# James51332/OceanSimulation

Hardware: AMD Instinct MI355X
Metric: height-field points/sec (N² iFFT) at 1/2/4/8 MI355X; % HBM roofline (higher is better)
Workload: dtype f32

## Files before the change

include/oceanfft.h:

```cpp
#ifndef OCEANFFT_H
#define OCEANFFT_H

#include <stddef.h>
#include <stdint.h>

#ifdef __cplusplus
extern "C" {
#endif

#define OCEAN_OK 0
#define OCEAN_ERR_INVALID 1
#define OCEAN_ERR_HIP 2
#define OCEAN_ERR_NO_DEVICE 3
#define OCEAN_ERR_OOM 4

#define OCEAN_MAX_CASCADES 64

typedef struct ocean_settings
{
  int32_t seed[2];
  float U_10;
  float theta_0;
  float F;
  float g;
  float swell;
  float h;
  float displacement;
  float time;
  float planeSize;
  float scale;
  float spread;
  int32_t boundWavelength;
  float wavelengthMin;
  float wavelengthMax;
} ocean_settings;

typedef struct ocean_fft ocean_fft;
typedef struct ocean_generator ocean_generator;

const char* ocean_last_error(void);
const char* ocean_version(void);
void ocean_default_settings(ocean_settings* s);
int ocean_device_count(void);

int ocean_fft_create(ocean_fft** out, size_t texture_size, void* hip_stream);
int ocean_fft_destroy(ocean_fft* fft);
size_t ocean_fft_texture_resolution(const ocean_fft* fft);
int ocean_fft_encode_ifft(ocean_fft* fft, float* image);
int ocean_fft_encode_ifft_batch(ocean_fft* fft, float* images, int n_images);
int ocean_fft_synchronize(ocean_fft* fft);
int ocean_fft_device_cus(const ocean_fft* fft);
int ocean_fft_set_cu_budget(ocean_fft* fft, int cus);

int ocean_generator_create(ocean_generator** out, ocean_fft* fft, int cascades);
int ocean_generator_destroy(ocean_generator* gen);
int ocean_generator_cascades(const ocean_generator* gen);
ocean_settings* ocean_generator_settings(ocean_generator* gen, int cascade);
int ocean_generator_calculate(ocean_generator* gen, float timestep, int update_spectrum);
int ocean_generator_generate_spectrum(ocean_generator* gen);
float* ocean_generator_height_map(ocean_generator* gen, int cascade);
float* ocean_generator_displacement_map(ocean_generator* gen, int cascade);
float* ocean_generator_jacobian_map(ocean_generator* gen, int cascade);
float* ocean_generator_initial_spectrum(ocean_generator* gen, int cascade);
int ocean_generator_spectrum_block(const ocean_generator* gen);

int ocean_generator_set_half_spectrum(ocean_generator* gen, int enable);
int ocean_generator_set_four_step(ocean_generator* gen, int enable);
int ocean_generator_set_h0_memo(ocean_generator* gen, int enable);
int ocean_generator_set_frame_overlap(ocean_generator* gen, int enable);
int ocean_generator_frame_bytes(const ocean_generator* gen, double per_point[2]);

int ocean_generator_create_slab(ocean_generator** out, ocean_fft* fft, int rank, int ranks);
size_t ocean_generator_exchange_bytes(const ocean_generator* gen);
int ocean_generator_slab_columns(ocean_generator* gen, float timestep, int update_spectrum, float* send);
int ocean_generator_slab_rows(ocean_generator* gen, const float* recv);
int ocean_generator_slab_info(const ocean_generator* gen, int* rank, int* ranks, int* row0, int* rows);
int ocean_slab_layout(size_t texture_size, int rank, int ranks, int half, int64_t out[6]);

#define OCEAN_COMM_ID_BYTES 128
typedef struct ocean_comm ocean_comm;
int ocean_comm_unique_id(unsigned char id[OCEAN_COMM_ID_BYTES]);
int ocean_comm_create(ocean_comm** out, const unsigned char id[OCEAN_COMM_ID_BYTES], int nranks, int rank);
int ocean_comm_wrap(ocean_comm** out, void* nccl_comm, int nranks, int rank);
int ocean_comm_destroy(ocean_comm* comm);
int ocean_comm_all_to_all(ocean_comm* comm, const void* send, void* recv, size_t bytes, void* hip_stream);
int ocean_generator_slab_frame(ocean_generator* gen, ocean_comm* comm, float timestep, int update_spectrum);
int ocean_generator_slab_frame_pipelined(ocean_generator* gen, ocean_comm* comm, float timestep, int update_spectrum);
int ocean_generator_slab_flush(ocean_generator* gen);

#define OCEAN_ERR_TIMEOUT 5
#define OCEAN_PEER_HANDLE_BYTES 256
typedef struct ocean_peers ocean_peers;
int ocean_peers_create(ocean_peers** out, ocean_generator* gen);
int ocean_peers_destroy(ocean_peers* peers);
int ocean_peers_handle(const ocean_peers* peers, unsigned char handle[OCEAN_PEER_HANDLE_BYTES]);
int ocean_peers_connect(ocean_peers* peers, const unsigned char* handles);
int ocean_peers_connect_local(ocean_peers* const* all, int ranks);
int ocean_peers_set_timeout(ocean_peers* peers, int ms);
int ocean_peers_set_put_cus(ocean_peers* peers, int cus);
int ocean_peers_set_streams(ocean_peers* peers, void* column_stream, void* put_stream, void* row_stream);
int ocean_peers_set_row_cus(ocean_peers* peers, int cus);
int ocean_peers_set_put_cu_mask(ocean_peers* peers, int cus_per_xcd);
int ocean_generator_slab_frame_put(ocean_generator* gen, ocean_peers* peers, float timestep, int update_spectrum);
int ocean_generator_slab_frame_put_pipelined(ocean_generator* gen, ocean_peers* peers, float timestep,
                                             int update_spectrum);
int ocean_peers_flush(ocean_peers* peers);
int ocean_generator_slab_put_columns(ocean_generator* gen, ocean_peers* peers, float timestep, int update_spectrum);
int ocean_generator_slab_put_rows(ocean_generator* gen, ocean_peers* peers);
int ocean_peers_synchronize(ocean_peers* peers);

int ocean_peers_debug_slot(const ocean_peers* peers, int slot, void** ptr, size_t* bytes);

int ocean_frame_plan(size_t texture_size, int cascades, int32_t out[8]);

int ocean_generator_set_profiling(ocean_generator* gen, int enable);
int ocean_generator_kernel_times(ocean_generator* gen, double ms_total[3], int64_t launches[3]);
int ocean_generator_kernel_times4(ocean_generator* gen, double ms_total[4], int64_t launches[4]);

int ocean_debug_hash(const uint32_t* xy, int count, uint32_t* raw, float* uv, void* hip_stream);
int ocean_debug_copy(void* dst, const void* src, size_t bytes, int workgroups, void* hip_stream);
int ocean_debug_fft_work_limit(ocean_fft* fft, size_t bytes);

int ocean_surface_sample(ocean_generator* const* gens, const int* cascades, int count, const float* xz,
                         int64_t points, float* out);
int ocean_surface_sample_plane(ocean_generator* const* gens, const int* cascades, int count, const float camera[5],
                               int res, float* out);
int ocean_surface_query(ocean_generator* const* gens, const int* cascades, int count, const float* xz,
                        int64_t points, int iterations, float tolerance, float* out);

int ocean_generator_mip_levels(const ocean_generator* gen);
int ocean_generator_build_mips(ocean_generator* gen);
float* ocean_generator_height_mip(ocean_generator* gen, int cascade, int level);
float* ocean_generator_displacement_mip(ocean_generator* gen, int cascade, int level);
float* ocean_generator_jacobian_mip(ocean_generator* gen, int cascade, int level);
int ocean_surface_sample_lod(ocean_generator* const* gens, const int* cascades, int count, const float* xzf,
                             int64_t points, float* out);
int ocean_surface_sample_plane_lod(ocean_generator* const* gens, const int* cascades, int count,
                                   const float camera[5], int res, float* out);

int ocean_generator_calculate_rates(ocean_generator* gen);
float* ocean_generator_height_rate_map(ocean_generator* gen, int cascade);
float* ocean_generator_displacement_rate_map(ocean_generator* gen, int cascade);
int ocean_surface_velocity(ocean_generator* const* gens, const int* cascades, int count, const float* xz,
                           int64_t points, float* out);

int ocean_generator_set_depth_layers(ocean_generator* gen, const float* depths, int layers);
int ocean_generator_depth_layers(const ocean_generator* gen, float out[8]);
int ocean_generator_calculate_kinematics(ocean_generator* gen);
float* ocean_generator_kinematics_map(ocean_generator* gen, int cascade, int layer, int image);
int ocean_water_kinematics(ocean_generator* const* gens, const int* cascades, int count, const float* xyz,
                           int64_t points, int iterations, float tolerance, float* out);

int ocean_generator_build_bounds(ocean_generator* gen);
int ocean_generator_bounds(ocean_generator* gen, int cascade, float out[18]);
const float* ocean_generator_bounds_device(ocean_generator* gen);
int ocean_surface_raycast(ocean_generator* const* gens, const int* cascades, int count, const float* rays,
                          int64_t n_rays, float step, int max_steps, int refine, int iterations, float tolerance,
                          float slope, float pad, float* out);

typedef struct ocean_camera
{
  float position[3];
  float right[3], up[3], forward[3];
  float tan_half_fov_y, near_plane, far_plane;
  float lod_scale;
} ocean_camera;
typedef struct ocean_shading
{
  float wave_color[3], scatter_color[3], sky_color[3], light_color[3], light_direction[3];
  float sun_view_angle, sun_falloff_angle, fog_begin, fog_density;
} ocean_shading;
typedef struct ocean_march
{
  float step;
  int max_steps, refine, iterations;
  float tolerance, slope, pad;
} ocean_march;
void ocean_default_camera(ocean_camera* camera);
void ocean_default_shading(ocean_shading* shading);
void ocean_default_march(ocean_march* march);
int ocean_camera_rays(const ocean_camera* camera, int width, int height, float* rays, void* hip_stream);
int ocean_camera_render(ocean_generator* const* gens, const int* cascades, int count, const ocean_camera* camera,
                        const ocean_shading* shading, const ocean_march* march, int width, int height, float* image,
                        float* aux, uint8_t* image8);

typedef struct ocean_camera_layers
{
  float foam_color[3];
  float foam_lo, foam_hi;
  float foam_opacity;
  float spray_color[3];
  float spray_radius;
  int32_t spray_max_half;
  float spray_opacity;
} ocean_camera_layers;
void ocean_default_camera_layers(ocean_camera_layers* layers);
size_t ocean_camera_layers_scratch_bytes(int width, int height);
int ocean_camera_render_layers(ocean_generator* const* gens, const int* cascades, int count,
                               const ocean_camera* camera, const ocean_shading* shading, const ocean_march* march,
                               const ocean_camera_layers* layers, int width, int height, const float* records,
                               const int64_t* count_device, int64_t max_records, void* scratch, float* image,
                               float* aux, float* aux2, uint8_t* image8);

typedef struct ocean_hulls ocean_hulls;
int ocean_hulls_create(ocean_hulls** out, ocean_fft* fft, const float* points, int64_t n_points,
                       const int32_t* ranges, int bodies);
int ocean_hulls_destroy(ocean_hulls* hulls);
int ocean_hulls_bodies(const ocean_hulls* hulls);
int64_t ocean_hulls_instance_points(const ocean_hulls* hulls);
int ocean_hulls_loads(ocean_hulls* hulls, ocean_generator* const* gens, const int* cascades, int count,
                      const float* poses, float rho_g, int iterations, float tolerance, int water_velocity,
                      float* loads, float* point_out);

int ocean_hulls_set_bodies(ocean_hulls* hulls, const float* props);

typedef struct ocean_hull_step_settings {
  float dt; int32_t substeps;
  float gravity[3];
  float rho_g; int32_t iterations; float tolerance; int32_t water_velocity;
} ocean_hull_step_settings;
void ocean_default_hull_step_settings(ocean_hull_step_settings* settings);

int ocean_hulls_step(ocean_hulls* hulls, ocean_generator* const* gens, const int* cascades, int count,
                     const ocean_hull_step_settings* settings, float* poses, const float* wrench_ext,
                     float* loads, float* point_out);

int ocean_debug_hulls_packing(int enable);

typedef struct ocean_foam_settings {
  float bias;
  float gain;
  float decay;
  float level;
} ocean_foam_settings;
void ocean_default_foam_settings(ocean_foam_settings* out);
ocean_foam_settings* ocean_generator_foam_settings(ocean_generator* gen, int cascade);
int ocean_generator_advance_foam(ocean_generator* gen, float dt);
int ocean_generator_reset_foam(ocean_generator* gen);
float* ocean_generator_foam_map(ocean_generator* gen, int cascade);
int ocean_generator_foam_counts(ocean_generator* gen, int cascade, int64_t out[3]);
const int64_t* ocean_generator_foam_counts_device(ocean_generator* gen);
int ocean_surface_sample_foam(ocean_generator* const* gens, const int* cascades, int count, const float* xz,
                              int64_t points, float* out);
int ocean_surface_sample_plane_foam(ocean_generator* const* gens, const int* cascades, int count,
                                    const float camera[5], int res, float* out);

typedef struct ocean_foam_deposit_settings {
  float amount;
  float per_speed;
} ocean_foam_deposit_settings;
void ocean_default_foam_deposit_settings(ocean_foam_deposit_settings* out);
int ocean_foam_deposit(ocean_generator* const* gens, const int* cascades, int count,
                       const ocean_foam_deposit_settings* settings, const float* records,
                       const int64_t* count_device, int64_t max_records);
int ocean_foam_deposit_counts(ocean_generator* gen0, int64_t out[50]);
const int64_t* ocean_foam_deposit_counts_device(ocean_generator* gen0);
int ocean_debug_foam_deposit_merge(int enable);

typedef struct ocean_spray_settings {
  float threshold;
  float rate;
  uint32_t seed;
} ocean_spray_settings;
void ocean_default_spray_settings(ocean_spray_settings* out);
typedef struct ocean_spray ocean_spray;
int ocean_spray_create(ocean_spray** out, ocean_fft* fft);
int ocean_spray_destroy(ocean_spray* spray);
int ocean_spray_emit(ocean_spray* spray, ocean_generator* const* gens, const int* cascades, int count,
                     const ocean_spray_settings* settings, const int32_t* tiles, float dt, uint32_t step,
                     int velocity, int64_t capacity, float* out);
int ocean_spray_counts(ocean_spray* spray, int64_t out[18]);
const int64_t* ocean_spray_counts_device(ocean_spray* spray);

typedef struct ocean_particle_settings {
  float gravity;
  float drag;
  float wind[3];
  float lifetime;
  float gain;
  float lift;
  int32_t iterations;
  float tolerance;
} ocean_particle_settings;
void ocean_default_particle_settings(ocean_particle_settings* out);
typedef struct ocean_particles ocean_particles;
int ocean_particles_create(ocean_particles** out, ocean_fft* fft, int64_t capacity);
int ocean_particles_destroy(ocean_particles* pool);
int ocean_particles_step(ocean_particles* pool, ocean_generator* const* gens, const int* cascades, int count,
                         const ocean_particle_settings* settings, float dt, const float* emit_records,
                         const int64_t* emit_counts_device, int64_t landed_capacity, float* landed_out);
int ocean_particles_load(ocean_particles* pool, const float* device_records, int64_t count);
int ocean_particles_clear(ocean_particles* pool);
const float* ocean_particles_records(ocean_particles* pool);
int ocean_particles_counts(ocean_particles* pool, int64_t out[8]);
const int64_t* ocean_particles_counts_device(ocean_particles* pool);

#ifdef __cplusplus
}
#endif

#endif
```

oceansimulation_amd/capi.py:

```python
from __future__ import annotations

import ctypes
import os

_HERE = os.path.dirname(os.path.abspath(__file__))
LIB_PATH = os.path.join(_HERE, "liboceanfft.so")

OCEAN_OK = 0
OCEAN_ERR_INVALID = 1
OCEAN_ERR_HIP = 2
OCEAN_ERR_NO_DEVICE = 3
OCEAN_ERR_OOM = 4
OCEAN_ERR_TIMEOUT = 5
OCEAN_MAX_CASCADES = 64
OCEAN_COMM_ID_BYTES = 128
OCEAN_PEER_HANDLE_BYTES = 256


class OceanSettings(ctypes.Structure):

    _fields_ = [
        ("seed", ctypes.c_int32 * 2),
        ("U_10", ctypes.c_float),
        ("theta_0", ctypes.c_float),
        ("F", ctypes.c_float),
        ("g", ctypes.c_float),
        ("swell", ctypes.c_float),
        ("h", ctypes.c_float),
        ("displacement", ctypes.c_float),
        ("time", ctypes.c_float),
        ("planeSize", ctypes.c_float),
        ("scale", ctypes.c_float),
        ("spread", ctypes.c_float),
        ("boundWavelength", ctypes.c_int32),
        ("wavelengthMin", ctypes.c_float),
        ("wavelengthMax", ctypes.c_float),
    ]


assert ctypes.sizeof(OceanSettings) == 64


class OceanFoamSettings(ctypes.Structure):

    _fields_ = [
        ("bias", ctypes.c_float),
        ("gain", ctypes.c_float),
        ("decay", ctypes.c_float),
        ("level", ctypes.c_float),
    ]


assert ctypes.sizeof(OceanFoamSettings) == 16


class OceanFoamDepositSettings(ctypes.Structure):

    _fields_ = [
        ("amount", ctypes.c_float),
        ("per_speed", ctypes.c_float),
    ]


assert ctypes.sizeof(OceanFoamDepositSettings) == 8


class OceanSpraySettings(ctypes.Structure):

    _fields_ = [
        ("threshold", ctypes.c_float),
        ("rate", ctypes.c_float),
        ("seed", ctypes.c_uint32),
    ]


assert ctypes.sizeof(OceanSpraySettings) == 12


class OceanParticleSettings(ctypes.Structure):

    _fields_ = [
        ("gravity", ctypes.c_float),
        ("drag", ctypes.c_float),
        ("wind", ctypes.c_float * 3),
        ("lifetime", ctypes.c_float),
        ("gain", ctypes.c_float),
        ("lift", ctypes.c_float),
        ("iterations", ctypes.c_int32),
        ("tolerance", ctypes.c_float),
    ]


assert ctypes.sizeof(OceanParticleSettings) == 40


class OceanHullStepSettings(ctypes.Structure):

    _fields_ = [
        ("dt", ctypes.c_float),
        ("substeps", ctypes.c_int32),
        ("gravity", ctypes.c_float * 3),
        ("rho_g", ctypes.c_float),
        ("iterations", ctypes.c_int32),
        ("tolerance", ctypes.c_float),
        ("water_velocity", ctypes.c_int32),
    ]


assert ctypes.sizeof(OceanHullStepSettings) == 36


class OceanCamera(ctypes.Structure):

    _fields_ = [
        ("position", ctypes.c_float * 3),
        ("right", ctypes.c_float * 3),
        ("up", ctypes.c_float * 3),
        ("forward", ctypes.c_float * 3),
        ("tan_half_fov_y", ctypes.c_float),
        ("near_plane", ctypes.c_float),
        ("far_plane", ctypes.c_float),
        ("lod_scale", ctypes.c_float),
    ]


class OceanShading(ctypes.Structure):

    _fields_ = [
        ("wave_color", ctypes.c_float * 3),
        ("scatter_color", ctypes.c_float * 3),
        ("sky_color", ctypes.c_float * 3),
        ("light_color", ctypes.c_float * 3),
        ("light_direction", ctypes.c_float * 3),
        ("sun_view_angle", ctypes.c_float),
        ("sun_falloff_angle", ctypes.c_float),
        ("fog_begin", ctypes.c_float),
        ("fog_density", ctypes.c_float),
    ]


class OceanMarch(ctypes.Structure):

    _fields_ = [
        ("step", ctypes.c_float),
        ("max_steps", ctypes.c_int),
        ("refine", ctypes.c_int),
        ("iterations", ctypes.c_int),
        ("tolerance", ctypes.c_float),
        ("slope", ctypes.c_float),
        ("pad", ctypes.c_float),
    ]


assert ctypes.sizeof(OceanCamera) == 64 and ctypes.sizeof(OceanShading) == 76 and ctypes.sizeof(OceanMarch) == 28


class OceanCameraLayers(ctypes.Structure):

    _fields_ = [
        ("foam_color", ctypes.c_float * 3),
        ("foam_lo", ctypes.c_float),
        ("foam_hi", ctypes.c_float),
        ("foam_opacity", ctypes.c_float),
        ("spray_color", ctypes.c_float * 3),
        ("spray_radius", ctypes.c_float),
        ("spray_max_half", ctypes.c_int32),
        ("spray_opacity", ctypes.c_float),
    ]


assert ctypes.sizeof(OceanCameraLayers) == 48

_vp = ctypes.c_void_p
_i = ctypes.c_int
_f = ctypes.c_float
_sz = ctypes.c_size_t
_fp = ctypes.POINTER(ctypes.c_float)
_sp = ctypes.POINTER(OceanSettings)
_fsp = ctypes.POINTER(OceanFoamSettings)

SIGNATURES = {
    "ocean_last_error": (ctypes.c_char_p, []),
    "ocean_version": (ctypes.c_char_p, []),
    "ocean_default_settings": (None, [_sp]),
    "ocean_device_count": (_i, []),
    "ocean_fft_create": (_i, [ctypes.POINTER(_vp), _sz, _vp]),
    "ocean_fft_destroy": (_i, [_vp]),
    "ocean_fft_texture_resolution": (_sz, [_vp]),
    "ocean_fft_encode_ifft": (_i, [_vp, _vp]),
    "ocean_fft_encode_ifft_batch": (_i, [_vp, _vp, _i]),
    "ocean_fft_synchronize": (_i, [_vp]),
    "ocean_fft_device_cus": (_i, [_vp]),
    "ocean_fft_set_cu_budget": (_i, [_vp, _i]),
    "ocean_generator_create": (_i, [ctypes.POINTER(_vp), _vp, _i]),
    "ocean_generator_destroy": (_i, [_vp]),
    "ocean_generator_cascades": (_i, [_vp]),
    "ocean_generator_settings": (_sp, [_vp, _i]),
    "ocean_generator_calculate": (_i, [_vp, _f, _i]),
    "ocean_generator_generate_spectrum": (_i, [_vp]),
    "ocean_generator_height_map": (_vp, [_vp, _i]),
    "ocean_generator_displacement_map": (_vp, [_vp, _i]),
    "ocean_generator_jacobian_map": (_vp, [_vp, _i]),
    "ocean_generator_initial_spectrum": (_vp, [_vp, _i]),
    "ocean_generator_spectrum_block": (_i, [_vp]),
    "ocean_generator_create_slab": (_i, [ctypes.POINTER(_vp), _vp, _i, _i]),
    "ocean_generator_exchange_bytes": (_sz, [_vp]),
    "ocean_generator_slab_columns": (_i, [_vp, _f, _i, _vp]),
    "ocean_generator_slab_rows": (_i, [_vp, _vp]),
    "ocean_generator_slab_info": (_i, [_vp, ctypes.POINTER(_i), ctypes.POINTER(_i), ctypes.POINTER(_i), ctypes.POINTER(_i)]),
    "ocean_generator_set_profiling": (_i, [_vp, _i]),
    "ocean_generator_kernel_times": (_i, [_vp, ctypes.POINTER(ctypes.c_double), ctypes.POINTER(ctypes.c_int64)]),
    "ocean_debug_hash": (_i, [_vp, _i, _vp, _vp, _vp]),
    "ocean_debug_copy": (_i, [_vp, _vp, _sz, _i, _vp]),
    "ocean_debug_fft_work_limit": (_i, [_vp, _sz]),
    "ocean_surface_sample": (_i, [_vp, _vp, _i, _vp, ctypes.c_int64, _vp]),
    "ocean_surface_sample_plane": (_i, [_vp, _vp, _i, _vp, _i, _vp]),
    "ocean_surface_query": (_i, [_vp, _vp, _i, _vp, ctypes.c_int64, _i, ctypes.c_float, _vp]),
    "ocean_generator_mip_levels": (_i, [_vp]),
    "ocean_generator_build_mips": (_i, [_vp]),
    "ocean_generator_height_mip": (_vp, [_vp, _i, _i]),
    "ocean_generator_displacement_mip": (_vp, [_vp, _i, _i]),
    "ocean_generator_jacobian_mip": (_vp, [_vp, _i, _i]),
    "ocean_surface_sample_lod": (_i, [_vp, _vp, _i, _vp, ctypes.c_int64, _vp]),
    "ocean_surface_sample_plane_lod": (_i, [_vp, _vp, _i, _vp, _i, _vp]),
    "ocean_generator_calculate_rates": (_i, [_vp]),
    "ocean_generator_height_rate_map": (_vp, [_vp, _i]),
    "ocean_generator_displacement_rate_map": (_vp, [_vp, _i]),
    "ocean_surface_velocity": (_i, [_vp, _vp, _i, _vp, ctypes.c_int64, _vp]),
    "ocean_generator_set_depth_layers": (_i, [_vp, _fp, _i]),
    "ocean_generator_depth_layers": (_i, [_vp, _fp]),
    "ocean_generator_calculate_kinematics": (_i, [_vp]),
    "ocean_generator_kinematics_map": (_vp, [_vp, _i, _i, _i]),
    "ocean_water_kinematics": (_i, [_vp, _vp, _i, _vp, ctypes.c_int64, _i, ctypes.c_float, _vp]),
    "ocean_generator_build_bounds": (_i, [_vp]),
    "ocean_generator_bounds": (_i, [_vp, _i, _fp]),
    "ocean_generator_bounds_device": (_vp, [_vp]),
    "ocean_surface_raycast": (_i, [_vp, _vp, _i, _vp, ctypes.c_int64, _f, _i, _i, _i, _f, _f, _f, _vp]),
    "ocean_default_camera": (None, [ctypes.POINTER(OceanCamera)]),
    "ocean_default_shading": (None, [ctypes.POINTER(OceanShading)]),
    "ocean_default_march": (None, [ctypes.POINTER(OceanMarch)]),
    "ocean_camera_rays": (_i, [ctypes.POINTER(OceanCamera), _i, _i, _vp, _vp]),
    "ocean_camera_render": (_i, [_vp, _vp, _i, ctypes.POINTER(OceanCamera), ctypes.POINTER(OceanShading),
                                 ctypes.POINTER(OceanMarch), _i, _i, _vp, _vp, _vp]),
    "ocean_default_camera_layers": (None, [ctypes.POINTER(OceanCameraLayers)]),
    "ocean_camera_layers_scratch_bytes": (_sz, [_i, _i]),
    "ocean_camera_render_layers": (_i, [_vp, _vp, _i, ctypes.POINTER(OceanCamera), ctypes.POINTER(OceanShading),
                                        ctypes.POINTER(OceanMarch), ctypes.POINTER(OceanCameraLayers), _i, _i, _vp, _vp,
                                        ctypes.c_int64, _vp, _vp, _vp, _vp, _vp]),
    "ocean_default_foam_settings": (None, [_fsp]),
    "ocean_generator_foam_settings": (_fsp, [_vp, _i]),
    "ocean_generator_advance_foam": (_i, [_vp, _f]),
    "ocean_generator_reset_foam": (_i, [_vp]),
    "ocean_generator_foam_map": (_vp, [_vp, _i]),
    "ocean_generator_foam_counts": (_i, [_vp, _i, ctypes.POINTER(ctypes.c_int64)]),
    "ocean_generator_foam_counts_device": (_vp, [_vp]),
    "ocean_surface_sample_foam": (_i, [_vp, _vp, _i, _vp, ctypes.c_int64, _vp]),
    "ocean_surface_sample_plane_foam": (_i, [_vp, _vp, _i, _vp, _i, _vp]),
    "ocean_default_foam_deposit_settings": (None, [ctypes.POINTER(OceanFoamDepositSettings)]),
    "ocean_foam_deposit": (_i, [_vp, _vp, _i, ctypes.POINTER(OceanFoamDepositSettings), _vp, _vp, ctypes.c_int64]),
    "ocean_foam_deposit_counts": (_i, [_vp, ctypes.POINTER(ctypes.c_int64)]),
    "ocean_foam_deposit_counts_device": (_vp, [_vp]),
    "ocean_debug_foam_deposit_merge": (_i, [_i]),
    "ocean_hulls_create":(_i, [ctypes.POINTER(_vp), _vp, _vp, ctypes.c_int64, _vp, _i]),
    "ocean_hulls_destroy": (_i, [_vp]),
    "ocean_hulls_bodies": (_i, [_vp]),
    "ocean_hulls_instance_points": (ctypes.c_int64, [_vp]),
    "ocean_debug_hulls_packing": (_i, [_i]),
    "ocean_hulls_loads": (_i, [_vp, _vp, _vp, _i, _vp, _f, _i, _f, _i, _vp, _vp]),
    "ocean_hulls_set_bodies": (_i, [_vp, _vp]),
    "ocean_default_hull_step_settings": (None, [ctypes.POINTER(OceanHullStepSettings)]),
    "ocean_hulls_step": (_i, [_vp, _vp, _vp, _i, ctypes.POINTER(OceanHullStepSettings), _vp, _vp, _vp, _vp]),
    "ocean_default_spray_settings": (None, [ctypes.POINTER(OceanSpraySettings)]),
    "ocean_spray_create": (_i, [ctypes.POINTER(_vp), _vp]),
    "ocean_spray_destroy": (_i, [_vp]),
    "ocean_spray_emit": (_i, [_vp, _vp, _vp, _i, ctypes.POINTER(OceanSpraySettings), _vp, _f, ctypes.c_uint32, _i,
                              ctypes.c_int64, _vp]),
    "ocean_spray_counts": (_i, [_vp, ctypes.POINTER(ctypes.c_int64)]),
    "ocean_spray_counts_device": (_vp, [_vp]),
    "ocean_default_particle_settings": (None, [ctypes.POINTER(OceanParticleSettings)]),
    "ocean_particles_create": (_i, [ctypes.POINTER(_vp), _vp, ctypes.c_int64]),
    "ocean_particles_destroy": (_i, [_vp]),
    "ocean_particles_step": (_i, [_vp, _vp, _vp, _i, ctypes.POINTER(OceanParticleSettings), _f, _vp, _vp,
                                  ctypes.c_int64, _vp]),
    "ocean_particles_load": (_i, [_vp, _vp, ctypes.c_int64]),
    "ocean_particles_clear": (_i, [_vp]),
    "ocean_particles_records": (_vp, [_vp]),
    "ocean_particles_counts": (_i, [_vp, ctypes.POINTER(ctypes.c_int64)]),
    "ocean_particles_counts_device": (_vp, [_vp]),
    "ocean_generator_set_half_spectrum": (_i, [_vp, _i]),
    "ocean_generator_set_four_step": (_i, [_vp, _i]),
    "ocean_generator_set_h0_memo": (_i, [_vp, _i]),
    "ocean_generator_set_frame_overlap": (_i, [_vp, _i]),
    "ocean_generator_frame_bytes": (_i, [_vp, _vp]),
    "ocean_slab_layout": (_i, [_sz, _i, _i, _i, ctypes.POINTER(ctypes.c_int64)]),
    "ocean_comm_unique_id": (_i, [_vp]),
    "ocean_comm_create": (_i, [ctypes.POINTER(_vp), _vp, _i, _i]),
    "ocean_comm_wrap": (_i, [ctypes.POINTER(_vp), _vp, _i, _i]),
    "ocean_comm_destroy": (_i, [_vp]),
    "ocean_comm_all_to_all": (_i, [_vp, _vp, _vp, _sz, _vp]),
    "ocean_generator_slab_frame": (_i, [_vp, _vp, _f, _i]),
    "ocean_generator_slab_frame_pipelined": (_i, [_vp, _vp, _f, _i]),
    "ocean_generator_slab_flush": (_i, [_vp]),
    "ocean_peers_create": (_i, [ctypes.POINTER(_vp), _vp]),
    "ocean_peers_destroy": (_i, [_vp]),
    "ocean_peers_handle": (_i, [_vp, _vp]),
    "ocean_peers_connect": (_i, [_vp, _vp]),
    "ocean_peers_connect_local": (_i, [ctypes.POINTER(_vp), _i]),
    "ocean_peers_set_timeout": (_i, [_vp, _i]),
    "ocean_peers_set_put_cus": (_i, [_vp, _i]),
    "ocean_peers_set_streams": (_i, [_vp, _vp, _vp, _vp]),
    "ocean_peers_set_row_cus": (_i, [_vp, _i]),
    "ocean_peers_set_put_cu_mask": (_i, [_vp, _i]),
    "ocean_generator_kernel_times4": (_i, [_vp, ctypes.POINTER(ctypes.c_double), ctypes.POINTER(ctypes.c_int64)]),
    "ocean_generator_slab_frame_put": (_i, [_vp, _vp, _f, _i]),
    "ocean_generator_slab_frame_put_pipelined": (_i, [_vp, _vp, _f, _i]),
    "ocean_peers_flush": (_i, [_vp]),
    "ocean_frame_plan": (_i, [_sz, _i, ctypes.POINTER(ctypes.c_int32)]),
    "ocean_peers_debug_slot": (_i, [_vp, _i, ctypes.POINTER(ctypes.c_void_p), ctypes.POINTER(_sz)]),
    "ocean_generator_slab_put_columns": (_i, [_vp, _vp, _f, _i]),
    "ocean_generator_slab_put_rows": (_i, [_vp, _vp]),
    "ocean_peers_synchronize": (_i, [_vp]),
}

_lib = None


class OceanError(RuntimeError):
    def __init__(self, code: int, where: str):
        msg = lib().ocean_last_error().decode(errors="replace")
        super().__init__(f"{where} failed with status {code}: {msg}")
        self.code = code


def lib():
    global _lib
    if _lib is None:
        if not os.path.exists(LIB_PATH):
            raise ImportError(f"{LIB_PATH} is missing — run `make` (or __graft_entry__.build()) first; "
                              "there is no CPU fallback for the ocean hot path")
        L = ctypes.CDLL(LIB_PATH)
        for name, (res, args) in SIGNATURES.items():
            fn = getattr(L, name)
            fn.restype = res
            fn.argtypes = args
        _lib = L
    return _lib


def check(code: int, where: str) -> None:
    if code != OCEAN_OK:
        raise OceanError(code, where)
```

oceansimulation_amd/csrc/device/k_half_cols.h:

```cpp
#pragma once

#include <hip/hip_runtime.h>

#include <cstdint>

#include "ocean_internal.h"
#include "launch_common.h"
#include "device/evolve.h"
#include "device/fft.h"
#include "device/grid.h"
#include "device/memory.h"
#include "device/spectrum.h"

namespace oceanfft
{


template <int LOGN>
struct HalfCfg
{
  static constexpr int N = 1 << LOGN;
  static constexpr int B = ColFirstCfg<LOGN>::B;
  static constexpr int STRIPS = N / (2 * B) + 1;
  static constexpr bool SUPPORTED = B == 4 && ColFirstCfg<LOGN>::SPW == 1;
  static constexpr bool SLAB_SUPPORTED = ColFirstCfg<LOGN>::SPW == 1;
};

constexpr int kHalfRG = 2, kHalfRGC = 4;
constexpr int kHalfRG2 = 4, kHalfRGC2 = 8;
constexpr int kHalfHL = 1, kHalfHK = 4, kHalfHKSeed = 2;
template <int LOGN, int RG, int FB = 4>
__device__ __forceinline__ int half_group_offset(int y, int strip, int b = 0)
{
  constexpr int N = HalfCfg<LOGN>::N, FS = HalfCfg<LOGN>::STRIPS * HalfCfg<LOGN>::B / FB;
  return RG == 1 ? (strip * N + y) * FB + b : (((y / RG) * FS + strip) * RG + (y % RG)) * FB + b;
}


template <int LOGN_, bool SEED_>
struct ColsWhole
{
  static constexpr int LOGN = LOGN_, LA = SEED_ ? 0 : kStream;
  static constexpr bool SLAB = false, SEED = SEED_, PUT = false, NYQ = true;
  static constexpr int RG = kHalfRG, RGC = kHalfRGC, FB = 4;
  static constexpr int CPI = ColFirstCfg<LOGN_>::B, HB = ColFirstCfg<LOGN_>::B;
  static constexpr int HL = kHalfHL, HK = SEED_ ? kHalfHKSeed : LOGN_ == 12 ? kHalfHK : 2;
};

template <int LOGN_, bool SEED_, int HB_>
struct ColsHalfStrip
{
  static constexpr int LOGN = LOGN_, LA = SEED_ ? 0 : kStream;
  static constexpr bool SLAB = false, SEED = SEED_, PUT = false, NYQ = true;
  static constexpr int RG = kHalfRG2, RGC = kHalfRGC2, FB = 2;
  static constexpr int CPI = 2, HB = HB_;
  static constexpr int HL = kHalfHL, HK = SEED_ ? kHalfHKSeed : LOGN_ == 12 ? kHalfHK : 2;
};

template <int LOGN_, bool PUT_>
struct ColsSlab
{
  static constexpr int LOGN = LOGN_, LA = kStream;
  static constexpr bool SLAB = true, SEED = false, PUT = PUT_, NYQ = false;
  static constexpr int RG = 1, RGC = 1, FB = 4;
  static constexpr int CPI = ColFirstCfg<LOGN_>::B, HB = ColFirstCfg<LOGN_>::B;
  static constexpr int HL = kHalfHL, HK = LOGN_ == 13 ? 1 : kHalfHK - 1;
};

template <typename Sh>
struct ColsLaunch
{
  using S = FftShape<Sh::LOGN>;
  static constexpr int WG = S::T * Sh::CPI;
  static constexpr int LDS = ((S::TW_ENTRIES * 8 + 15) / 16) * 16 + Sh::CPI * S::PADDED * 8 + Sh::HL * WG * 16;
  static constexpr int items(int cascades, int nstrips) { return cascades * nstrips * (ColFirstCfg<Sh::LOGN>::B / Sh::CPI); }
  static constexpr int max_grid(int hs_blocks) { return Sh::SLAB ? hs_blocks : hs_blocks * (1024 / WG); }
};

template <typename Sh>
__global__ __launch_bounds__(ColsLaunch<Sh>::WG, Sh::CPI < ColFirstCfg<Sh::LOGN>::B ? 4 : 1) void k_cols_half(
    FrameParams fp, const float4* __restrict__ h0, float4* __restrict__ gab, float4* __restrict__ gde,
    float2* __restrict__ gc, const float2* __restrict__ tw_glob, float2* __restrict__ hs, HalfSlab hsl,
    unsigned char* __restrict__ send, int h0_full, const SpectrumConsts* __restrict__ seed)
{
  constexpr int LOGN = Sh::LOGN, LA = Sh::LA, RG = Sh::RG, RGC = Sh::RGC, CPI = Sh::CPI, HL = Sh::HL, HK = Sh::HK,
                FB = Sh::FB, HB = Sh::HB;
  constexpr bool SLAB = Sh::SLAB, SEED = Sh::SEED, PUT = Sh::PUT, NYQ = Sh::NYQ;
  using S = FftShape<LOGN>;
  using K = ColFirstCfg<LOGN>;
  using HC = HalfCfg<LOGN>;
  constexpr int N = S::N, T = S::T, B = K::B, STRIPS = HC::STRIPS, WG = T * CPI, HALVES = B / CPI;
  static_assert(SLAB ? HC::SLAB_SUPPORTED : HC::SUPPORTED, "half-spectrum path: one strip per item (B = 4 unless SLAB)");
  static_assert(CPI * HALVES == B && HALVES <= 2 && (HALVES == 1 || !SLAB), "whole or half strips");
  static_assert(HL >= 0 && HK >= 0 && HL + HK <= 8, "H pairs outside the scratch");
  static_assert(FB == 4 || (FB == CPI && HALVES == 2 && !SLAB && RG > 1 && RGC > 1), "FB: half-strip fields");
  static_assert(!PUT || SLAB, "PUT: the strip-dealt slab stores");
  static_assert(HB == B || (HB == CPI && HALVES == 2 && !SLAB), "HB: half strips over 2-column h0 strips");
  static_assert(!NYQ || !SLAB, "NYQ: whole grids (send is the spec output)");
  constexpr int XB = CPI * S::PADDED * 8;
  extern __shared__ __attribute__((aligned(16))) unsigned char smem[];
  float2* tw = reinterpret_cast<float2*>(smem);
  void* xch = smem + ((S::TW_ENTRIES * 8 + 15) / 16) * 16;
  float4* hlds = reinterpret_cast<float4*>(static_cast<unsigned char*>(xch) + XB);
  load_twiddles<LOGN>(tw, tw_glob);

  const int nstrips = SLAB ? hsl.nstrips : STRIPS;
  const int total = fp.cascades * nstrips * HALVES;
  const float dim = (float)N;
  for (int item = HALVES > 1 ? xcd_pair_slot(blockIdx.x, gridDim.x) : (int)blockIdx.x; item < total; item += gridDim.x)
  {
    const int hh = HALVES > 1 ? item % HALVES : 0, si = HALVES > 1 ? item / HALVES : item;
    const int c = si / nstrips, s = si - c * nstrips;
    const int sg = SLAB ? hsl.strip0 + s : s;
    if (HALVES > 1 && sg == STRIPS - 1 && hh != 0)
      continue;
    const int b = opaque((int)threadIdx.x) % CPI + hh * CPI;
    const int xb = sg == STRIPS - 1 ? 0 : N / (2 * B) + sg;
    const CascadeFrame f = fp.c[c];
    const float4* src = HB != B                  ? h0 + ((size_t)c * (N / HB) + xb * (B / HB) + hh) * N * HB
                        : (!SLAB || h0_full) ? h0 + ((size_t)c * (N / B) + xb) * N * B
                                             : h0 + ((size_t)c * nstrips + s) * N * B;
    const int fs = FB == 4 ? s : 2 * s + hh;
    const size_t gbase = RG == 1 ? ((size_t)c * STRIPS + s) * N * B
                                 : (size_t)c * STRIPS * N * B + half_group_offset<LOGN, RG, FB>(0, fs);
    const size_t cgbase = RGC == 1 ? ((size_t)c * STRIPS + s) * N * B
                                   : (size_t)c * STRIPS * N * B + half_group_offset<LOGN, RGC, FB>(0, fs);
    const int bf = FB == 4 ? b : b - hh * CPI;
    const int x = xb * B + b;
    float4 hk[HK > 0 ? HK : 1];
    auto run_round = [&](int round) __attribute__((always_inline)) {
      const int i = (opaque((int)threadIdx.x) / CPI) % T;
      const int voff = (i * B + b) * 16;
      CPair v[16];
      auto pack = [&](int m, float2 H, const KVec& q) __attribute__((always_inline)) {
        if (round == 0)
          v[m] = CPair{f2v{H.x, q.kz * H.x}, f2v{H.y, q.kz * H.y}};
        else if (round == 1)
        {
          const float e = q.kz * q.dirz;
          v[m] = CPair{f2v{q.dirz * H.x, e * H.x}, f2v{q.dirz * H.y, e * H.y}};
        }
        else
          v[m] = CPair{f2v{q.inv * H.x, 0.0f}, f2v{q.inv * H.y, 0.0f}};
      };
      if (SEED && round == 0)
      {
        float2* hsb = hs + (size_t)blockIdx.x * 16 * WG;
        const int hoff = opaque((int)threadIdx.x) * 8;
        const SpectrumConsts q = seed[c];
#pragma unroll 1
        for (int m = 0; m < 16; m++)
        {
          const int y = i + ((m + 8) & 15) * T;
          const float2 H = evolve(seed_texel(q, x, y, dim), make_kvec(x, y, dim, f.dk).k, f);
          if ((m >> 1) < HL)
            reinterpret_cast<float2*>(hlds)[((m >> 1) * WG + threadIdx.x) * 2 + (m & 1)] = H;
          else
            st2s<0>(hsb, hoff * 2 + (m & 1) * 8, (m >> 1) * WG * 16, H);
        }
        __threadfence_block();
#pragma unroll
        for (int m = 0; m < 16; m += 2)
        {
          const int y = i + ((m + 8) & 15) * T, p = m >> 1;
          const float4 pp = p < HL ? hlds[p * WG + threadIdx.x] : ld4s<kStream>(hsb, hoff * 2, p * WG * 16);
          if (p >= HL && p < HL + HK)
            hk[p < HL + HK && p >= HL ? p - HL : 0] = pp;
          pack(m, make_float2(pp.x, pp.y), make_kvec(x, y, dim, f.dk));
          pack(m + 1, make_float2(pp.z, pp.w), make_kvec(x, y + T, dim, f.dk));
        }
      }
      else if (round == 0)
      {
        float2* hsb = hs + (size_t)blockIdx.x * 16 * WG;
        const int hoff = opaque((int)threadIdx.x) * 8;
        float4 a[16];
        float2 hprev = make_float2(0.0f, 0.0f);
        const int loff = HB == B ? voff : (i * HB + (b - hh * CPI)) * 16;
#pragma unroll
        for (int m = 0; m < 16; m++)
          a[m] = ld4s<LA>(src, loff, ((m + 8) & 15) * T * HB * 16);
#pragma unroll
        for (int m = 0; m < 16; m++)
        {
          const int y = i + ((m + 8) & 15) * T;
          const KVec q = make_kvec(x, y, dim, f.dk);
          const float2 H = evolve(a[m], q.k, f);
          const int p = m >> 1;
          if ((m & 1) && p < HL)
            hlds[p * WG + threadIdx.x] = make_float4(hprev.x, hprev.y, H.x, H.y);
          else if ((m & 1) && p < HL + HK)
            hk[p - HL] = make_float4(hprev.x, hprev.y, H.x, H.y);
          else if (m & 1)
            st4s<0>(hsb, hoff * 2, p * WG * 16, make_float4(hprev.x, hprev.y, H.x, H.y));
          else
            hprev = H;
          pack(m, H, q);
        }
      }
      else
      {
        const float2* hsb = hs + (size_t)blockIdx.x * 16 * WG;
        const int hoff = opaque((int)threadIdx.x) * 8;
#pragma unroll
        for (int m = 0; m < 16; m += 2)
        {
          const int y = i + ((m + 8) & 15) * T, pi = m >> 1;
          const float4 p = pi < HL        ? hlds[pi * WG + threadIdx.x]
                           : pi < HL + HK ? hk[pi < HL + HK ? pi - HL : 0]
                                          : ld4s<kStream>(hsb, hoff * 2, pi * WG * 16);
          pack(m, make_float2(p.x, p.y), make_kvec(x, y, dim, f.dk));
          pack(m + 1, make_float2(p.z, p.w), make_kvec(x, y + T, dim, f.dk));
        }
      }
      const int reg = HALVES > 1 ? opaque((int)threadIdx.x) % CPI : b;
      fft_run<LOGN, CPI, true>(v, i, reg, xch, tw);
      const int vo = (i * B + b) * 16;
#pragma unroll
      for (int m = 0; m < 16; m++)
      {
        if constexpr (SLAB)
        {
          const size_t part = (size_t)fp.cascades * hsl.S * hsl.w * B;
          const int q = (m * T) / hsl.w, yl0 = (m * T) % hsl.w;
          const size_t el = (((size_t)c * hsl.S + s) * hsl.w + yl0) * B;
          unsigned char* blk =
              PUT ? reinterpret_cast<unsigned char*>(sopaque((size_t)reinterpret_cast<const uint64_t*>(send)[q]))
                  : send + sopaque((size_t)q * (part * 40 + (size_t)fp.cascades * 2 * N * 16));
          if (round == 0)
            st4<kStream>(blk + el * 16, vo, pair_raw(v[m]));
          else if (round == 1)
            st4<kStream>(blk + part * 16 + el * 16, vo, pair_raw(v[m]));
          else
            st2<kStream>(blk + part * 32 + el * 8, (i * B + b) * 8, make_float2(v[m].re.x, v[m].im.x));
        }
        else if constexpr (RG == 1 && RGC == 1)
        {
          if (round == 0)
            st4s<kStream>(gab + gbase, vo, m * T * B * 16, pair_raw(v[m]));
          else if (round == 1)
            st4s<kStream>(gde + gbase, vo, m * T * B * 16, pair_raw(v[m]));
          else
            st2s<kStream>(gc + gbase, (i * B + b) * 8, m * T * B * 8, make_float2(v[m].re.x, v[m].im.x));
        }
        else if (round == 0)
          st4s<kStream>(gab + gbase, half_group_offset<LOGN, RG, FB>(i, 0, bf) * 16, half_group_offset<LOGN, RG, FB>(m * T, 0) * 16,
                        pair_raw(v[m]));
        else if (round == 1)
          st4s<kStream>(gde + gbase, half_group_offset<LOGN, RG, FB>(i, 0, bf) * 16, half_group_offset<LOGN, RG, FB>(m * T, 0) * 16,
                        pair_raw(v[m]));
        else
          st2s<kStream>(gc + cgbase, half_group_offset<LOGN, RGC, FB>(i, 0, bf) * 8, half_group_offset<LOGN, RGC, FB>(m * T, 0) * 8,
                        make_float2(v[m].re.x, v[m].im.x));
      }
    };
#pragma unroll
    for (int round = 0; round < 3; round++)
      run_round(round);
  }
  if constexpr (NYQ)
    if ((HALVES > 1 ? xcd_pair_slot(blockIdx.x, gridDim.x) : (int)blockIdx.x) == (int)gridDim.x - 1)
      for (int idx = threadIdx.x; idx < fp.cascades * N; idx += WG)
        half_nyquist_texel(fp, N, HB, h0, reinterpret_cast<float4*>(send), nullptr, 1, 0, seed, nullptr, 0, idx);
}

template <typename Sh>
hipError_t launch_cols_half(const FrameParams& fp, int nstrips, const float4* h0, float4* gab, float4* gde, float2* gc,
                            const float2* tw, float2* hs, int hs_blocks, const HalfSlab& hsl, unsigned char* send,
                            int h0_full, const SpectrumConsts* seed, hipStream_t stream, int cus)
{
  using G = ColsLaunch<Sh>;
  auto kern = k_cols_half<Sh>;
  int grid = persistent_grid(kern, G::WG, G::LDS, G::items(fp.cascades, nstrips), cus);
  if (grid > G::max_grid(hs_blocks))
    grid = G::max_grid(hs_blocks);
  if (grid < 1)
    return hipErrorInvalidValue;
  hipLaunchKernelGGL(kern, dim3(grid), dim3(G::WG), G::LDS, stream, fp, h0, gab, gde, gc, tw, hs, hsl, send, h0_full, seed);
  return hipGetLastError();
}

}
```

oceansimulation_amd/csrc/device/k_half_rows.h:

```cpp
#pragma once

#include <hip/hip_runtime.h>

#include <cstdint>

#include "ocean_internal.h"
#include "device/evolve.h"
#include "device/fft.h"
#include "device/grid.h"
#include "device/memory.h"
#include "device/spectrum.h"
#include "device/k_half_cols.h"

namespace oceanfft
{

template <int LOGN, int LA, bool RM, int RG = 1, int RGC = 1, int FB = 4>
__global__ __launch_bounds__(FftShape<LOGN>::T * 2) void k_rows_half(
    FrameParams fp, const float4* __restrict__ gab, const float4* __restrict__ gde, const float2* __restrict__ gc,
    const float4* __restrict__ spec, float4* __restrict__ maps, float* __restrict__ jac, FoamParams foam,
    const float2* __restrict__ tw_glob, int rows, RowSrc rs)
{
  using S = FftShape<LOGN>;
  using K = ColFirstCfg<LOGN>;
  using HC = HalfCfg<LOGN>;
  constexpr int N = S::N, T = S::T, B = K::B, RPW = 2, STRIPS = HC::STRIPS, WG = T * RPW;
  static_assert(WG <= 1024, "two rows per workgroup: N <= 8192");
  static_assert(WG * 8 * 16 <= lds_row_slots<LOGN>(RPW) * 8, "mirror exchange fits the transform's LDS");
  extern __shared__ __attribute__((aligned(16))) unsigned char smem[];
  float2* tw = reinterpret_cast<float2*>(smem);
  void* xch = smem + ((S::TW_ENTRIES * 8 + 15) / 16) * 16;
  CPair* mir = reinterpret_cast<CPair*>(xch);
  load_twiddles<LOGN>(tw, tw_glob);

  const int blocks = (RM ? rows : N) / RPW;
  const int b0 = threadIdx.x % B, r0 = (threadIdx.x / B) % RPW, ihi0 = threadIdx.x / (B * RPW);
  constexpr int CI = T >= 128 ? 2 : 0;
  const int i20 = CI ? (threadIdx.x / RPW) % T : threadIdx.x % T, r20 = CI ? threadIdx.x % RPW : threadIdx.x / T;
  const int total = fp.cascades * blocks;
  const float dim = (float)N;
  for (int item = xcd_pair_slot(blockIdx.x, gridDim.x); item < total; item += gridDim.x)
  {
    const int c = item / blocks, y0 = (item - c * blocks) * RPW;
    float2 ckeep[8];
    float2 cnyq;
#pragma unroll
    for (int img = 0; img < 2; img++)
    {
    const int cimg = c * 2 + img;
    const int b = opaque(b0), ihi = opaque(ihi0), r = opaque(r0);
    const int i = ihi * B + b;
    const float dk = fp.c[c].dk;
    const size_t base = RM ? ((size_t)c * rows + y0) * rs.lp : (size_t)c * STRIPS * N * B;
    const int y = y0 + r;
    const float sgy = (y & 1) ? -1.0f : 1.0f;
    const float4* sp = spec + (size_t)cimg * N;
    const int tid = opaque((int)threadIdx.x);
    CPair v[16];
#pragma unroll
    for (int m = 0; m < 8; m++)
    {
      const int u = m * T + i;
      const int src = RM ? __builtin_amdgcn_readfirstlane(u >> (31 - __builtin_clz(rs.cpr))) : 0;
      const int off = RM ? r * rs.lp + (u & (rs.cpr - 1)) : half_group_offset<LOGN, RG, FB>(y, u / FB, u % FB);
      const int offc = RM ? off : half_group_offset<LOGN, RGC, FB>(y, u / FB, u % FB);
      const float4* fab = RM ? reinterpret_cast<const float4*>(rs.ab + src * rs.src_stride) + base : gab + base;
      const float4* fde = RM ? reinterpret_cast<const float4*>(rs.de + src * rs.src_stride) + base : gde + base;
      const float2* fc = RM ? reinterpret_cast<const float2*>(rs.c + src * rs.src_stride) + base : gc + base;
      const float kx = (float)u * dk;
      const float4 s4 = ld4<0>(sp, (N / 2 - u) * 16);
      CPair own, neg;
      if (img == 0)
      {
        const CPair p = raw_pair(ld4<LA>(fab, off * 16));
        const float2 cc = ld2<LA>(fc, offc * 8);
        ckeep[m] = cc;
        const float Ar = p.re.x, Ai = p.im.x, Br = p.re.y, Bi = p.im.y, Cr = cc.x, Ci = cc.y;
        own = CPair{f2v{(1.0f - kx) * Ar, -Bi - kx * Cr}, f2v{(1.0f - kx) * Ai, Br - kx * Ci}};
        neg = CPair{f2v{(1.0f + kx) * Ar + sgy * s4.x, -Bi + kx * Cr + sgy * s4.z},
                    f2v{-(1.0f + kx) * Ai + sgy * s4.y, -Br - kx * Ci + sgy * s4.w}};
      }
      else
      {
        const CPair q = raw_pair(ld4<LA>(fde, off * 16));
        const float2 cc = ckeep[m];
        const float Cr = cc.x, Ci = cc.y, Dr = q.re.x, Di = q.im.x, Er = q.re.y, Ei = q.im.y;
        const float kx2 = kx * kx;
        own = CPair{f2v{-(Di - kx2 * Ci), -Er + kx * Di}, f2v{Dr - kx2 * Cr, -Ei - kx * Dr}};
        neg = CPair{f2v{-(Di + kx2 * Ci) + sgy * s4.x, -Er - kx * Di + sgy * s4.z},
                    f2v{-Dr - kx2 * Cr + sgy * s4.y, Ei - kx * Dr + sgy * s4.w}};
      }
      v[m] = own;
      mir[m * WG + tid] = neg;
    }
    __syncthreads();
    const int tp = i == 0 ? tid : tid + (((T - i) / B - ihi) * B * RPW) + ((T - i) % B - b);
#pragma unroll
    for (int m = 8; m < 16; m++)
    {
      if (i == 0 && m == 8)
      {
        const int off = RM ? r * rs.lp + rs.cpr : half_group_offset<LOGN, RG, FB>(y, N / 2 / FB);
        const int offc = RM ? off : half_group_offset<LOGN, RGC, FB>(y, N / 2 / FB);
        const size_t ns = RM ? (size_t)rs.nyq_src * rs.src_stride : 0;
        const float4* fab = RM ? reinterpret_cast<const float4*>(rs.ab + ns) + base : gab + base;
        const float4* fde = RM ? reinterpret_cast<const float4*>(rs.de + ns) + base : gde + base;
        const float2* fc = RM ? reinterpret_cast<const float2*>(rs.c + ns) + base : gc + base;
        const float kx = -(dim / 2.0f) * dk;
        float2 cc;
        if (img == 1)
          cc = cnyq;
        else
          cc = ld2<LA>(fc, offc * 8);
        if (img == 0)
          cnyq = cc;
        if (img == 0)
        {
          const CPair p = raw_pair(ld4<LA>(fab, off * 16));
          v[m] = CPair{f2v{(1.0f - kx) * p.re.x, -p.im.y - kx * cc.x},
                       f2v{(1.0f - kx) * p.im.x, p.re.y - kx * cc.y}};
        }
        else
        {
          const CPair q = raw_pair(ld4<LA>(fde, off * 16));
          const float kx2 = kx * kx;
          v[m] = CPair{f2v{-(q.im.x - kx2 * cc.y), -q.re.y + kx * q.im.x},
                       f2v{q.re.x - kx2 * cc.x, -q.im.y - kx * q.re.x}};
        }
      }
      else
        v[m] = mir[(i == 0 ? 16 - m : 15 - m) * WG + tp];
    }
    __syncthreads();
    const int i2 = opaque(i20), r2 = opaque(r20);
    fft_run<LOGN, CI, true>(v, i, r, i2, r2, xch, tw);
    float4* dst = maps + ((size_t)cimg * (RM ? rows : N) + y0) * N;
    const int woff = ((r2 << LOGN) + i2) * 16;
#pragma unroll
    for (int m = 0; m < 16; m++)
      st4<kStream>(dst + m * T, woff, from_pair(v[m]));
    if (img & 1)
    {
      const float lam = foam.displacement[c];
      float* jb = jac + ((size_t)c * (RM ? rows : N) + y0) * N;
      const int joff = ((r2 << LOGN) + i2) * 4;
#pragma unroll
      for (int m = 0; m < 16; m++)
        st1<kStream>(jb + m * T, joff,
                (1.0f + lam * v[m].im.x) * (1.0f + lam * v[m].re.y) - lam * lam * v[m].im.y * v[m].im.y);
    }
    }
  }
}

}
```

oceansimulation_amd/csrc/device/k_rows_hp.h:

```cpp
#pragma once

#include <hip/hip_runtime.h>

#include <cstdint>

#include "ocean_internal.h"
#include "device/fft.h"
#include "device/grid.h"
#include "device/k_half_cols.h"
#include "device/lane_xchg.h"
#include "device/memory.h"

namespace oceanfft
{

struct HpCfg
{
  static constexpr int LOGN = 12, RS = 264;
  static constexpr int TW = ((FftShape<LOGN>::TW_ENTRIES * 8 + 15) / 16) * 16;
  static constexpr int LDS = TW + 16 * RS * 8;
};

__device__ __forceinline__ int hp_swz(int n1) { return ((n1 >> 1) & 7) ^ (((n1 >> 1) & 1) << 2); }
__device__ __forceinline__ int hp_slot(int n1, int j) { return n1 * HpCfg::RS + (j ^ hp_swz(n1)); }

template <int RG, int RGC, bool RM = false, int FB = 4, int GRP = 4, int EARLY = 0, int MINB = 4>
__global__ __launch_bounds__(256, MINB) void k_rows_hp(FrameParams fp, const float4* __restrict__ gab,
                                                 const float4* __restrict__ gde, const float2* __restrict__ gc,
                                                 const float4* __restrict__ spec, float4* __restrict__ maps,
                                                 float* __restrict__ jac, FoamParams foam,
                                                 const float2* __restrict__ tw_glob, int rows, RowSrc rs)
{
  constexpr int LOGN = HpCfg::LOGN, RS = HpCfg::RS;
  using S = FftShape<LOGN>;
  using HC = HalfCfg<LOGN>;
  constexpr int N = S::N, T = S::T, B = 4, STRIPS = HC::STRIPS;
  static_assert(T == 256, "one 4-wave row per workgroup");
  extern __shared__ __attribute__((aligned(16))) unsigned char smem[];
  float2* tw = reinterpret_cast<float2*>(smem);
  float2* xs = reinterpret_cast<float2*>(smem + HpCfg::TW);
  load_twiddles<LOGN>(tw, tw_glob);

  const int nrows = RM ? rows : N;
  const int total = fp.cascades * nrows;
  const float dim = (float)N;
  constexpr int LA = RM ? kStream : 0;
  const int lcpr = RM ? 31 - __builtin_clz(rs.cpr) : 0, cmask = RM ? rs.cpr - 1 : 0;
  const int wave0 = __builtin_amdgcn_readfirstlane((int)threadIdx.x & ~63);
  static_assert(EARLY == 0 || (EARLY == 1 && !RM), "EARLY: whole-grid layouts");
  float4 fpre[EARLY > 0 ? 8 : 1];
  auto issue = [&](int item, float4* f) __attribute__((always_inline)) {
    const int c = item / nrows, y = item - c * nrows;
    const size_t base = (size_t)c * STRIPS * N * B;
    const int i = opaque((int)threadIdx.x);
#pragma unroll
    for (int m = 0; m < 8; m++)
    {
      const int u = m * T + i;
      f[m] = ld4<LA>(gde + base, half_group_offset<LOGN, RG, FB>(y, u / FB, u % FB) * 16);
    }
  };
  for (int item = RM ? (int)blockIdx.x : xcd_group_slot<GRP>(blockIdx.x, gridDim.x); item < total; item += gridDim.x)
  {
    const int c = item / nrows, y = item - c * nrows;
    const float dk = fp.c[c].dk;
    const size_t base = RM ? ((size_t)c * rows + y) * rs.lp : (size_t)c * STRIPS * N * B;
    const float sgy = (y & 1) ? -1.0f : 1.0f;
    float2 ckeep[8], cnyq;
#pragma unroll
    for (int img = 0; img < 2; img++)
    {
      const int cimg = c * 2 + img;
      const float4* sp = spec + (size_t)cimg * N;
      const int tid = opaque((int)threadIdx.x), i = tid;
      CPair v[16];
#pragma unroll
      for (int m = 0; m < 8; m++)
      {
        const int u = m * T + i;
        const int src = RM ? (m * T + sopaque(wave0)) >> lcpr : 0;
        const int off = RM ? (u & cmask) : half_group_offset<LOGN, RG, FB>(y, u / FB, u % FB);
        const int offc = RM ? off : half_group_offset<LOGN, RGC, FB>(y, u / FB, u % FB);
        const float4* fab = RM ? reinterpret_cast<const float4*>(rs.ab + (size_t)src * rs.src_stride) : gab;
        const float4* fde = RM ? reinterpret_cast<const float4*>(rs.de + (size_t)src * rs.src_stride) : gde;
        const float2* fc = RM ? reinterpret_cast<const float2*>(rs.c + (size_t)src * rs.src_stride) : gc;
        const float kx = (float)u * dk;
        const float4 s4 = ld4<0>(sp, (N / 2 - u) * 16);
        if (img == 0)
        {
          const CPair p = raw_pair(ld4<LA>(fab + base, off * 16));
          const float2 cc = ld2<0>(fc + base, offc * 8);
          if constexpr (!RM)
            ckeep[m] = cc;
          const float Ar = p.re.x, Ai = p.im.x, Br = p.re.y, Bi = p.im.y, Cr = cc.x, Ci = cc.y;
          v[m] = CPair{f2v{(1.0f - kx) * Ar, -Bi - kx * Cr}, f2v{(1.0f - kx) * Ai, Br - kx * Ci}};
          v[m + 8] = CPair{f2v{(1.0f + kx) * Ar + sgy * s4.x, -Bi + kx * Cr + sgy * s4.z},
                           f2v{-(1.0f + kx) * Ai + sgy * s4.y, -Br - kx * Ci + sgy * s4.w}};
        }
        else
        {
          const CPair q = raw_pair(EARLY > 0 ? fpre[m] : ld4<LA>(fde + base, off * 16));
          float2 cc;
          if constexpr (RM)
            cc = ld2<0>(fc + base, offc * 8);
          else
            cc = ckeep[m];
          const float Cr = cc.x, Ci = cc.y, Dr = q.re.x, Di = q.im.x, Er = q.re.y, Ei = q.im.y;
          const float kx2 = kx * kx;
          v[m] = CPair{f2v{-(Di - kx2 * Ci), -Er + kx * Di}, f2v{Dr - kx2 * Cr, -Ei - kx * Dr}};
          v[m + 8] = CPair{f2v{-(Di + kx2 * Ci) + sgy * s4.x, -Er - kx * Di + sgy * s4.z},
                           f2v{-Dr - kx2 * Cr + sgy * s4.y, Ei - kx * Dr + sgy * s4.w}};
        }
      }
      if (i == 0)
      {
        const int off = RM ? rs.cpr : half_group_offset<LOGN, RG, FB>(y, N / 2 / FB);
        const int offc = RM ? off : half_group_offset<LOGN, RGC, FB>(y, N / 2 / FB);
        const size_t ns = RM ? (size_t)rs.nyq_src * rs.src_stride : 0;
        const float4* fab = RM ? reinterpret_cast<const float4*>(rs.ab + ns) : gab;
        const float4* fde = RM ? reinterpret_cast<const float4*>(rs.de + ns) : gde;
        const float2* fc = RM ? reinterpret_cast<const float2*>(rs.c + ns) : gc;
        const float kx = -(dim / 2.0f) * dk;
        if (RM || img == 0)
          cnyq = ld2<0>(fc + base, offc * 8);
        const float2 cc = cnyq;
        if (img == 0)
        {
          const CPair p = raw_pair(ld4<LA>(fab + base, off * 16));
          v[8] = CPair{f2v{(1.0f - kx) * p.re.x, -p.im.y - kx * cc.x}, f2v{(1.0f - kx) * p.im.x, p.re.y - kx * cc.y}};
        }
        else
        {
          const CPair q = raw_pair(ld4<LA>(fde + base, off * 16));
          const float kx2 = kx * kx;
          v[8] = CPair{f2v{-(q.im.x - kx2 * cc.y), -q.re.y + kx * q.im.x}, f2v{q.re.x - kx2 * cc.x, -q.im.y - kx * q.re.x}};
        }
      }
      const int w = tid >> 6, l = tid & 63, s = l & 3, p = l >> 2;
      const int n1r = 4 * w + s;
      const int rd = n1r * RS + (p ^ hp_swz(n1r));
      const int wo = hp_slot(i & 15, i >> 4);
      const int nm = N - i;
      const int wm = hp_slot(nm & 15, nm >> 4);
      const int wm0 = i == 0 ? hp_slot(0, (N / 2) >> 4) : wm;
      __syncthreads();
#pragma unroll
      for (int h = 0; h < 2; h++)
      {
        if (h)
          __syncthreads();
#pragma unroll
        for (int m = 0; m < 8; m++)
        {
          xs[wo + 16 * m] = half_of(v[m], h);
          xs[(m == 0 ? wm0 : wm) - 16 * m] = half_of(v[m + 8], h);
        }
        __syncthreads();
#pragma unroll
        for (int m = 0; m < 16; m++)
          set_half(v[m], h, xs[rd + 16 * m]);
      }
      idft16(v);
      apply_stage_twiddles<LOGN>(v, 16 * p, tw);
      transpose_reg_lanes_2_5(v);
      idft16(v);
      const float2 base_w = twiddle<LOGN>(n1r * p, tw);
#pragma unroll
      for (int m = 0; m < 16; m++)
        v[m] = cmul(v[m], base_w);
      apply_stage_twiddles<LOGN>(v, 16 * n1r, tw);
#pragma unroll
      for (int h = 0; h < 2; h++)
      {
        if (h)
          __syncthreads();
#pragma unroll
        for (int m = 0; m < 16; m++)
          xs[rd + 16 * m] = half_of(v[m], h);
        __syncthreads();
#pragma unroll
        for (int n1 = 0; n1 < 16; n1++)
          set_half(v[n1], h, xs[n1 * RS + (tid ^ hp_swz(n1))]);
      }
      idft16(v);
      if constexpr (EARLY > 0)
        if (img == 0)
          issue(item, fpre);
      float4* dst = maps + ((size_t)cimg * nrows + y) * N;
#pragma unroll
      for (int m = 0; m < 16; m++)
        st4<kStream>(dst + m * T, tid * 16, from_pair(v[m]));
      if (img == 1)
      {
        const float lam = foam.displacement[c];
        float* jb = jac + ((size_t)c * nrows + y) * N;
#pragma unroll
        for (int m = 0; m < 16; m++)
          st1<kStream>(jb + m * T, tid * 4,
                       (1.0f + lam * v[m].im.x) * (1.0f + lam * v[m].re.y) - lam * lam * v[m].im.y * v[m].im.y);
      }
    }
  }
}

}
```

oceansimulation_amd/csrc/launch_half.hip:

```cpp
#include <hip/hip_runtime.h>

#include <cstdint>

#include "oceanfft.h"
#include "ocean_internal.h"
#include "launch_common.h"
#include "device/grid.h"
#include "device/k_half_cols.h"
#include "device/k_half_rows.h"
#include "device/k_rows_hp.h"
#include "device/spectrum.h"

namespace oceanfft
{

bool half_spectrum_supported(int logn) { return logn >= 10 && logn <= 12; }

constexpr bool half_strip_launch(int logn, int cascades) { return (logn == 12 || logn == 11) && cascades <= 2; }

template <int LOGN, typename V>
hipError_t select_half_cols(int cascades, bool seed, int h0_blk, V&& visit)
{
  constexpr int B = ColFirstCfg<LOGN>::B;
  if constexpr (LOGN == 12 || LOGN == 11)
    if (half_strip_launch(LOGN, cascades))
    {
      if (h0_blk != 0 && h0_blk != 2 && h0_blk != B)
        return hipErrorInvalidValue;
      if (seed)
        return visit(ColsHalfStrip<LOGN, true, B>{});
      return h0_blk == B ? visit(ColsHalfStrip<LOGN, false, B>{}) : visit(ColsHalfStrip<LOGN, false, 2>{});
    }
  if (h0_blk != 0 && h0_blk != B)
    return hipErrorInvalidValue;
  return seed ? visit(ColsWhole<LOGN, true>{}) : visit(ColsWhole<LOGN, false>{});
}

template <int FB_, int RG_, int RGC_, int GRP_, int EARLY_, int MINB_>
struct RowsHp
{
  static constexpr bool HP = true;
  static constexpr int FB = FB_, RG = RG_, RGC = RGC_, GRP = GRP_, EARLY = EARLY_, MINB = MINB_;
};
template <int FB_, int RG_, int RGC_>
struct RowsHalf
{
  static constexpr bool HP = false;
  static constexpr int FB = FB_, RG = RG_, RGC = RGC_;
};

template <int LOGN, typename V>
hipError_t select_half_rows(int cascades, V&& visit)
{
  const bool hs = half_strip_launch(LOGN, cascades);
  if constexpr (LOGN == 12)
    return hs ? visit(RowsHp<2, kHalfRG2, kHalfRGC2, kHalfRGC2, 0, 4>{}) : visit(RowsHp<4, kHalfRG, kHalfRGC, 4, 1, 3>{});
  else if constexpr (LOGN == 11)
    return hs ? visit(RowsHalf<2, kHalfRG2, kHalfRGC2>{}) : visit(RowsHalf<4, kHalfRG, kHalfRGC>{});
  else
    return visit(RowsHalf<4, kHalfRG, kHalfRGC>{});
}

int half_h0_block(int logn, int cascades)
{
  int hb = spectrum_block(logn);
  (void)with_logn(logn, [&](auto L) -> hipError_t {
    constexpr int LOGN = decltype(L)::value;
    if constexpr (HalfCfg<LOGN>::SUPPORTED)
      return select_half_cols<LOGN>(cascades, false, 0, [&](auto sh) {
        hb = decltype(sh)::HB;
        return hipSuccess;
      });
    else
      return hipSuccess;
  });
  return hb;
}

size_t half_field_texels(int logn)
{
  const size_t n = (size_t)1 << logn;
  return (n / 8 + 1) * n * 4;
}

size_t half_hs_bytes(int logn, int blocks)
{
  return half_slab_supported(logn) ? (size_t)blocks * 16 * 1024 * sizeof(float2) : 0;
}

hipError_t launch_half_columns(int logn, const FrameParams& fp, const float4* h0, float4* gab, float4* gcd, float2* ge,
                               float4* spec, const float2* tw, hipStream_t stream, int cus, float2* hs, int hs_blocks,
                               const void* seed_consts, int h0_blk)
{
  if (!hs)
    return hipErrorInvalidValue;
  const SpectrumConsts* seed = static_cast<const SpectrumConsts*>(seed_consts);
  return with_logn(logn, [&](auto L) -> hipError_t {
    constexpr int LOGN = decltype(L)::value;
    if constexpr (!HalfCfg<LOGN>::SUPPORTED)
      return hipErrorInvalidValue;
    else
      return select_half_cols<LOGN>(fp.cascades, seed != nullptr, h0_blk > 0 ? h0_blk : ColFirstCfg<LOGN>::B, [&](auto sh) {
        return launch_cols_half<decltype(sh)>(fp, HalfCfg<LOGN>::STRIPS, h0, gab, gcd, ge, tw, hs, hs_blocks, HalfSlab{},
                                              reinterpret_cast<unsigned char*>(spec), 1, seed, stream, cus);
      });
  });
}

hipError_t launch_half_rows(int logn, const FrameParams& fp, const float4* gab, const float4* gcd, const float2* ge,
                            const float4* rcorr, float4* maps, float* jac, const FoamParams& foam, const float2* tw,
                            hipStream_t stream, int cus)
{
  return with_logn(logn, [&](auto L) -> hipError_t {
    constexpr int LOGN = decltype(L)::value;
    if constexpr (!HalfCfg<LOGN>::SUPPORTED)
      return hipErrorInvalidValue;
    else
      return select_half_rows<LOGN>(fp.cascades, [&](auto sh) {
        using R = decltype(sh);
        using S = FftShape<LOGN>;
        if constexpr (R::HP)
        {
          auto kern = k_rows_hp<R::RG, R::RGC, false, R::FB, R::GRP, R::EARLY, R::MINB>;
          const int grid = persistent_grid(kern, 256, HpCfg::LDS, fp.cascades * S::N, cus);
          hipLaunchKernelGGL(kern, dim3(grid), dim3(256), HpCfg::LDS, stream, fp, gab, gcd, ge, rcorr, maps, jac, foam, tw, 0,
                             RowSrc{});
        }
        else
        {
          auto kern = k_rows_half<LOGN, 0, false, R::RG, R::RGC, R::FB>;
          const int lds = ((S::TW_ENTRIES * 8 + 15) / 16) * 16 + lds_row_slots<LOGN>(2) * 8;
          const int grid = persistent_grid(kern, S::T * 2, lds, fp.cascades * (S::N / 2), cus);
          hipLaunchKernelGGL(kern, dim3(grid), dim3(S::T * 2), lds, stream, fp, gab, gcd, ge, rcorr, maps, jac, foam, tw, S::N,
                             RowSrc{});
        }
        return hipGetLastError();
      });
  });
}

}

extern "C" int ocean_frame_plan(size_t texture_size, int cascades, int32_t out[8])
{
  using namespace oceanfft;
  int logn = 0;
  while (logn < 15 && ((size_t)1 << logn) < texture_size)
    logn++;
  if (!out || ((size_t)1 << logn) != texture_size || !half_spectrum_supported(logn) || cascades < 1 ||
      cascades > kMaxCascades)
    return OCEAN_ERR_INVALID;
  const hipError_t e = with_logn(logn, [&](auto L) -> hipError_t {
    constexpr int LOGN = decltype(L)::value;
    if constexpr (!HalfCfg<LOGN>::SUPPORTED)
      return hipErrorInvalidValue;
    else
    {
      const hipError_t ec = select_half_cols<LOGN>(cascades, false, 0, [&](auto sh) {
        using C = decltype(sh);
        out[0] = C::FB, out[1] = C::RG, out[2] = C::RGC, out[3] = C::HB;
        return hipSuccess;
      });
      const hipError_t er = select_half_rows<LOGN>(cascades, [&](auto sh) {
        using R = decltype(sh);
        out[4] = R::FB, out[5] = R::RG, out[6] = R::RGC;
        return hipSuccess;
      });
      return ec != hipSuccess ? ec : er;
    }
  });
  if (e != hipSuccess)
    return OCEAN_ERR_INVALID;
  out[7] = half_h0_block(logn, cascades);
  return OCEAN_OK;
}
```

oceansimulation_amd/csrc/ocean_capi.cpp:

```cpp
#include "oceanfft.h"

#include <hip/hip_runtime.h>

#include <algorithm>
#include <cmath>
#include <cstdio>
#include <cstring>
#include <string>
#include <vector>

#include "ocean_capi_internal.h"
#include "ocean_internal.h"

static_assert(sizeof(ocean_settings) == sizeof(OceanSettings), "settings layout");

namespace
{
int log2_exact(size_t n)
{
  int l = 0;
  while (((size_t)1 << l) < n)
    l++;
  return ((size_t)1 << l) == n ? l : -1;
}

std::vector<float2> twiddle_tables(int logn, size_t& tw2_at, size_t& twm_at)
{
  std::vector<float2> tab;
  const double two_pi = 6.283185307179586476925286766559;
  auto append_table = [&](int lg) {
    const int lb = lg / 2, tb = 1 << lb, ta = 1 << (lg - lb);
    const double len = (double)(1 << lg);
    for (int e2 = 0; e2 < tb; e2++)
    {
      double a = two_pi * e2 / len;
      tab.push_back(make_float2((float)std::cos(a), (float)std::sin(a)));
    }
    for (int e2 = 0; e2 < ta; e2++)
    {
      double a = two_pi * ((double)e2 * tb) / len;
      tab.push_back(make_float2((float)std::cos(a), (float)std::sin(a)));
    }
  };
  append_table(logn);
  tw2_at = tab.size();
  if (fourstep_table(logn))
    append_table(logn - 4);
  twm_at = tab.size();
  if (ifft_pre_supported(logn))
    append_table(12);
  return tab;
}

void grow_work(ocean_fft* fft, size_t texels, int images)
{
  float4* w = nullptr;
  if (texels * sizeof(float4) > fft->work_limit)
    return;
  if (hipMalloc(&w, texels * sizeof(float4)) != hipSuccess)
  {
    (void)hipGetLastError();
    return;
  }
  if (fft->work)
    (void)hipFree(fft->work);
  fft->work = w;
  fft->work_images = images;
  fft->work_texels = texels;
}
}

constexpr int kFourStepSlab = 2048;

extern "C" {

const char* ocean_last_error(void) { return g_err.c_str(); }

const char* ocean_version(void) { return "oceanfft 0.1 (gfx950)"; }

void ocean_default_settings(ocean_settings* s)
{
  std::memset(s, 0, sizeof(*s));
  s->seed[0] = 12342;
  s->seed[1] = 8934;
  s->U_10 = 40.0f;
  s->theta_0 = 25.0f;
  s->F = 800000.0f;
  s->g = 9.8f;
  s->swell = 0.5f;
  s->h = 100.0f;
  s->displacement = 0.4f;
  s->time = 0.0f;
  s->planeSize = 40.0f;
  s->scale = 1.0f;
  s->spread = 0.2f;
  s->boundWavelength = 0;
  s->wavelengthMin = 0.0f;
  s->wavelengthMax = 0.0f;
}

int ocean_device_count(void)
{
  int n = 0;
  if (hipGetDeviceCount(&n) != hipSuccess)
    return 0;
  return n;
}

int ocean_fft_create(ocean_fft** out, size_t texture_size, void* hip_stream)
{
  if (!out)
    return fail(OCEAN_ERR_INVALID, "ocean_fft_create: out is null");
  *out = nullptr;
  int logn = log2_exact(texture_size);
  if (logn < 4 || logn > 14)
    return fail(OCEAN_ERR_INVALID, "ocean_fft_create: texture_size must be a power of two in [16, 16384], got " +
                                       std::to_string(texture_size));
  int ndev = 0;
  if (hipGetDeviceCount(&ndev) != hipSuccess || ndev == 0)
    return fail(OCEAN_ERR_NO_DEVICE, "ocean_fft_create: no HIP device visible");

  auto* f = new ocean_fft();
  f->n = (int)texture_size;
  f->logn = logn;
  f->stream = (hipStream_t)hip_stream;
  hipError_t e = hipGetDevice(&f->device);
  if (e == hipSuccess)
    e = hipDeviceGetAttribute(&f->device_cus, hipDeviceAttributeMultiprocessorCount, f->device);
  f->cus = f->device_cus;
  if (e != hipSuccess)
  {
    delete f;
    return hip_fail(e, "ocean_fft_create: device query");
  }

  size_t tw2_at = 0, twm_at = 0;
  const std::vector<float2> tab = twiddle_tables(logn, tw2_at, twm_at);
  e = hipMalloc(&f->twiddles, tab.size() * sizeof(float2));
  if (e == hipSuccess)
    e = hipMemcpy(f->twiddles, tab.data(), tab.size() * sizeof(float2), hipMemcpyHostToDevice);
  if (e != hipSuccess)
  {
    if (f->twiddles)
      (void)hipFree(f->twiddles);
    delete f;
    return hip_fail(e, "ocean_fft_create: twiddle table");
  }
  if (fourstep_table(logn))
    f->tw2 = f->twiddles + tw2_at;
  if (ifft_pre_supported(logn))
    f->twm = f->twiddles + twm_at;
  *out = f;
  return OCEAN_OK;
}

int ocean_fft_destroy(ocean_fft* fft)
{
  if (!fft)
    return OCEAN_OK;
  if (fft->twiddles)
    (void)hipFree(fft->twiddles);
  if (fft->work)
    (void)hipFree(fft->work);
  if (fft->surf_atlas)
    (void)hipFree(fft->surf_atlas);
  delete fft;
  return OCEAN_OK;
}

size_t ocean_fft_texture_resolution(const ocean_fft* fft) { return fft ? (size_t)fft->n : 0; }

int ocean_fft_device_cus(const ocean_fft* fft) { return fft ? fft->device_cus : 0; }

int ocean_fft_set_cu_budget(ocean_fft* fft, int cus)
{
  if (!fft)
    return fail(OCEAN_ERR_INVALID, "ocean_fft_set_cu_budget: null plan");
  if (cus < 0 || cus > fft->device_cus)
    return fail(OCEAN_ERR_INVALID, "ocean_fft_set_cu_budget: budget outside [0, device CUs]");
  fft->cus = cus == 0 ? fft->device_cus : cus;
  return OCEAN_OK;
}

int ocean_debug_fft_work_limit(ocean_fft* fft, size_t bytes)
{
  if (!fft)
    return fail(OCEAN_ERR_INVALID, "ocean_debug_fft_work_limit: null plan");
  fft->work_limit = bytes;
  if (fft->work && fft->work_texels * sizeof(float4) > bytes)
  {
    HIP_TRY(hipStreamSynchronize(fft->stream), "hipStreamSynchronize");
    (void)hipFree(fft->work);
    fft->work = nullptr;
    fft->work_images = 0;
    fft->work_texels = 0;
  }
  return OCEAN_OK;
}

int ocean_fft_encode_ifft_batch(ocean_fft* fft, float* images, int n_images)
{
  if (!fft || !images || n_images < 1)
    return fail(OCEAN_ERR_INVALID, "ocean_fft_encode_ifft_batch: null plan/image or n_images < 1");
  auto* img = reinterpret_cast<float4*>(images);
  const bool pre = fft->logn == 13 && fft->twm != nullptr;
  if (ifft_colfirst_supported(fft->logn) || pre)
  {
    const int chunk = std::max(1, (int)(((size_t)2 << 30) / ((size_t)fft->n * fft->n * sizeof(float4))));
    const int want = n_images < chunk ? n_images : chunk;
    if (fft->work_images < want)
      grow_work(fft, (size_t)want * fft->n * fft->n, want);
    if (fft->work)
    {
      for (int first = 0; first < n_images; first += fft->work_images)
      {
        const int count = n_images - first < fft->work_images ? n_images - first : fft->work_images;
        float4* first_img = img + (size_t)first * fft->n * fft->n;
        if (pre)
          HIP_TRY(launch_ifft_pre(fft->logn, count, first_img, fft->work, fft->twiddles, fft->twm, fft->stream, fft->cus),
                  "pre-stage EncodeIFFT");
        else
          HIP_TRY(launch_ifft_colfirst(fft->logn, count, first_img, fft->work, fft->twiddles, fft->stream, fft->cus),
                  "column-first EncodeIFFT");
      }
      return OCEAN_OK;
    }
  }
  if (ifft_fourstep_supported(fft->logn) && fft->logn == 14)
  {
    const size_t want = ifft_fourstep_work_texels(fft->logn, kFourStepSlab);
    if (fft->work_texels < want)
      grow_work(fft, want, 0);
    if (fft->work_texels >= want)
    {
      HIP_TRY(launch_ifft_fourstep(fft->logn, n_images, img, fft->work, kFourStepSlab, fft->twiddles, fft->tw2,
                                   fft->stream, fft->cus),
              "four-step EncodeIFFT");
      return OCEAN_OK;
    }
  }
  HIP_TRY(launch_rows_ifft(fft->logn, n_images, img, fft->twiddles, fft->stream, fft->cus), "row pass");
  HIP_TRY(launch_cols(fft->logn, n_images, img, fft->twiddles, fft->stream, fft->cus), "column pass");
  return OCEAN_OK;
}

int ocean_fft_encode_ifft(ocean_fft* fft, float* image) { return ocean_fft_encode_ifft_batch(fft, image, 1); }

int ocean_fft_synchronize(ocean_fft* fft)
{
  if (!fft)
    return fail(OCEAN_ERR_INVALID, "ocean_fft_synchronize: null plan");
  HIP_TRY(hipStreamSynchronize(fft->stream), "hipStreamSynchronize");
  return OCEAN_OK;
}

}

namespace
{
hipEvent_t take_event(ocean_generator* g)
{
  if (!g->pool.empty())
  {
    hipEvent_t e = g->pool.back();
    g->pool.pop_back();
    return e;
  }
  hipEvent_t e = nullptr;
  (void)hipEventCreate(&e);
  return e;
}

template <typename F>
hipError_t timed(ocean_generator* g, int kind, F&& launch, hipStream_t stream = nullptr)
{
  if (!g->profiling)
    return launch();
  if (!stream)
    stream = g->fft->stream;
  EventPair p{kind, take_event(g), take_event(g)};
  hipError_t e = hipEventRecord(p.a, stream);
  if (e != hipSuccess)
    return e;
  e = launch();
  if (e != hipSuccess)
    return e;
  e = hipEventRecord(p.b, stream);
  g->pending.push_back(p);
  return e;
}

hipError_t half_fields(ocean_generator* g, int slot)
{
  const size_t t = half_field_texels(g->fft->logn) * g->cascades;
  HalfFields& f = g->fields[slot];
  hipError_t e = alloc_if_null(f.gab, t * sizeof(float4));
  e = alloc_if_null(f.gde, t * sizeof(float4), e);
  e = alloc_if_null(f.gc, t * sizeof(float2), e);
  return alloc_if_null(f.spec, (size_t)g->cascades * 2 * g->fft->n * sizeof(float4), e);
}

hipError_t half_buffers(ocean_generator* g)
{
  return alloc_if_null(g->hs, half_hs_bytes(g->fft->logn, g->fft->device_cus), half_fields(g, 0));
}

HalfSlab half_slab_geom(int logn, int rank, int ranks)
{
  const int strips = half_strips(logn);
  HalfSlab h{};
  h.S = (strips + ranks - 1) / ranks;
  h.strip0 = rank * h.S;
  h.nstrips = std::max(0, std::min(h.S, strips - h.strip0));
  h.w = (1 << logn) / ranks;
  return h;
}

int h0_block(const ocean_generator* g)
{
  switch (frame_path(g))
  {
    case FramePath::FourStep:
      return gen4_h0_block();
    case FramePath::HalfBlocked:
      return half_h0_block(g->fft->logn, g->cascades);
    default:
      return spectrum_block(g->fft->logn);
  }
}

size_t h0_texels(const ocean_generator* g)
{
  const size_t full = (size_t)g->fft->n * g->geom.w;
  if (g->ranks == 1)
    return full;
  const size_t strips = (size_t)g->hsl.nstrips * spectrum_block(g->fft->logn) * g->fft->n;
  size_t t = std::max(full, strips);
  if (gen4_supported(g->fft->logn))
    t = std::max(t, g->g4.h0_cstride);
  return t;
}

hipError_t full_buffers(ocean_generator* g)
{
  const size_t slab = (size_t)g->fft->n * g->geom.w * g->cascades;
  hipError_t e = alloc_if_null(g->inter, slab * 2 * sizeof(float4));
  return rows_need_transpose(g->fft->logn) ? alloc_if_null(g->scratch, slab * 2 * sizeof(float4), e) : e;
}

hipError_t path_buffers(ocean_generator* g)
{
  switch (frame_path(g))
  {
    case FramePath::Full:
      return full_buffers(g);
    case FramePath::HalfBlocked:
      return half_buffers(g);
    default:
      return hslab_buffers(g);
  }
}
}

size_t hslab_xbuf_bytes(const ocean_generator* g)
{
  if (frame_path(g) == FramePath::FourStep)
    return (size_t)g->ranks * g->g4.blk_bytes;
  return (size_t)g->ranks * half_slab_block_bytes(g->fft->logn, g->cascades, g->hsl);
}

hipError_t hslab_buffers(ocean_generator* g)
{
  const int logn = g->fft->logn, C = g->cascades;
  hipError_t e = hipSuccess;
  if (frame_path(g) == FramePath::FourStep)
    e = alloc_if_null(g->parts, gen4_parts_bytes(logn, C, g->g4));
  else
  {
    const size_t rt = half_slab_row_texels(logn, C, g->hsl.w);
    e = alloc_if_null(g->rm_ab, rt * sizeof(float4));
    e = alloc_if_null(g->rm_de, rt * sizeof(float4), e);
    e = alloc_if_null(g->rm_c, rt * sizeof(float2), e);
    e = alloc_if_null(g->hs, half_hs_bytes(logn, g->fft->device_cus), e);
  }
  const size_t xb = hslab_xbuf_bytes(g);
  if (e == hipSuccess && g->xbuf_bytes < xb)
  {
    if (g->xbuf)
      (void)hipFree(g->xbuf);
    g->xbuf = nullptr;
    g->xbuf_bytes = 0;
    e = hipMalloc(&g->xbuf, xb);
    if (e == hipSuccess)
      g->xbuf_bytes = xb;
  }
  if (g->ranks > 1)
    e = alloc_if_null(g->h0row, (size_t)C * g->fft->n * sizeof(float4), e);
  return e;
}

namespace
{
int generator_alloc(ocean_generator** out, ocean_fft* fft, int cascades, int rank, int ranks, bool is_slab)
{
  auto* g = new ocean_generator();
  g->fft = fft;
  g->cascades = cascades;
  g->rank = rank;
  g->ranks = ranks;
  g->geom.w = fft->n / ranks;
  g->geom.x0 = rank * g->geom.w;
  g->settings.resize(cascades);
  for (auto& s : g->settings)
    ocean_default_settings(&s);
  g->foam_settings.resize(cascades);
  for (auto& s : g->foam_settings)
    ocean_default_foam_settings(&s);
  const size_t slab = (size_t)fft->n * g->geom.w;
  g->slab = is_slab;
  g->half_kind = half_kind_of(fft->logn, is_slab);
  g->half_on = g->half_kind != HalfKind::None;
  g->hsl = half_slab_geom(fft->logn, rank, ranks);
  if (gen4_supported(fft->logn))
  {
    g->g4 = gen4_geom(fft->logn, cascades, rank, ranks, ranks == 1);
    g->g4.h0_cstride = h0_texels(g);
  }
  if (is_slab && cascades != 1)
  {
    delete g;
    return fail(OCEAN_ERR_INVALID, "generator allocation: a slab generator holds exactly one cascade");
  }
  const size_t h0_bytes = h0_texels(g) * cascades * sizeof(float4);
  hipError_t e = alloc_if_null(g->h0, h0_bytes);
  if (e == hipSuccess)
    e = path_buffers(g);
  e = alloc_if_null(g->maps, slab * cascades * 2 * sizeof(float4), e);
  e = alloc_if_null(g->jac, slab * cascades * sizeof(float), e);
  if (e == hipSuccess)
    e = hipMemsetAsync(g->h0, 0, h0_bytes, fft->stream);
  if (e == hipSuccess)
    e = hipMemsetAsync(g->maps, 0, slab * cascades * 2 * sizeof(float4), fft->stream);
  if (e == hipSuccess)
    e = hipMemsetAsync(g->jac, 0, slab * cascades * sizeof(float), fft->stream);
  if (e != hipSuccess)
  {
    ocean_generator_destroy(g);
    return alloc_fail(e, "generator allocation");
  }
  *out = g;
  return OCEAN_OK;
}

int wait_h0_readers(ocean_generator* g)
{
  if (g->cols_ev_valid)
    HIP_TRY(hipStreamWaitEvent(g->fft->stream, g->h0r_ev, 0), "h0 write: wait for the last column pass");
  return OCEAN_OK;
}

struct H0Piece
{
  size_t at;
  int x0, cols, block;
};

struct H0Pieces
{
  H0Piece piece[2];
  int count = 0;
  bool row0 = false;
};

H0Pieces h0_pieces(const ocean_generator* g)
{
  const int n = g->fft->n;
  const FramePath path = frame_path(g);
  H0Pieces p;
  if (g->ranks > 1 && path == FramePath::FourStep)
  {
    const Gen4Geom& q = g->g4;
    const int B = gen4_h0_block();
    p.piece[p.count++] = {q.h0_reg, n / 2 + q.u0, q.cols, B};
    if (q.nyq)
      p.piece[p.count++] = {q.h0_nyq, 0, B, B};
    p.row0 = true;
  }
  else if (g->ranks > 1 && path == FramePath::StripDealt)
  {
    const int B = spectrum_block(g->fft->logn), strips = half_strips(g->fft->logn);
    const HalfSlab& h = g->hsl;
    const int nreg = std::max(0, std::min(h.nstrips, strips - 1 - h.strip0));
    if (nreg > 0)
      p.piece[p.count++] = {0, n / 2 + h.strip0 * B, nreg * B, 0};
    if (nreg < h.nstrips)
      p.piece[p.count++] = {(size_t)nreg * n * B, 0, B, 0};
    p.row0 = true;
  }
  else
    p.piece[p.count++] = {0, g->geom.x0, g->geom.w, h0_block(g)};
  return p;
}

int generate_spectrum_with(ocean_generator* g, const std::vector<ocean_settings>& settings)
{
  TRY(wait_h0_readers(g));
  g->h0_dirty = true;
  g->h0_stale = false;
  g->h0_block = h0_block(g);
  g->h0_settings = settings;
  g->seeded = settings;
  ocean_fft* f = g->fft;
  const H0Pieces pieces = h0_pieces(g);
  for (int c = 0; c < g->cascades; c++)
  {
    OceanSettings s;
    std::memcpy(&s, &settings[c], sizeof(s));
    float4* base = g->h0 + h0_texels(g) * c;
    HIP_TRY(timed(g, 0, [&] {
              hipError_t e = hipSuccess;
              for (int i = 0; i < pieces.count && e == hipSuccess; i++)
              {
                const H0Piece& p = pieces.piece[i];
                e = launch_generate_spectrum(s, f->n, base + p.at, f->stream, f->cus, p.x0, p.cols, p.block);
              }
              if (e == hipSuccess && pieces.row0)
                e = launch_generate_spectrum_row(s, f->n, g->h0row + (size_t)c * f->n, f->stream);
              return e;
            }),
            "generateSpectrum");
  }
  return OCEAN_OK;
}

bool same_h0_inputs(const std::vector<ocean_settings>& a, const std::vector<ocean_settings>& b)
{
  if (a.size() != b.size())
    return false;
  for (size_t i = 0; i < a.size(); i++)
  {
    ocean_settings x = a[i], y = b[i];
    x.time = y.time = 0.0f;
    if (std::memcmp(&x, &y, sizeof(x)) != 0)
      return false;
  }
  return true;
}

int fused_reseed(ocean_generator* g, const void*& seed)
{
  ocean_fft* f = g->fft;
  std::vector<unsigned char> host((size_t)g->cascades * seed_consts_bytes());
  for (int c = 0; c < g->cascades; c++)
  {
    OceanSettings os;
    std::memcpy(&os, &g->settings[c], sizeof(os));
    seed_consts(os, f->n, host.data() + (size_t)c * seed_consts_bytes());
  }
  if (!g->seedc)
    HIP_TRY(hipMalloc(&g->seedc, (size_t)kMaxCascades * seed_consts_bytes()), "seed constants");
  if (host != g->seedc_host)
  {
    TRY(wait_h0_readers(g));
    HIP_TRY(hipMemcpyAsync(g->seedc, host.data(), host.size(), hipMemcpyHostToDevice, f->stream), "seed constants");
    g->seedc_host.swap(host);
  }
  seed = g->seedc;
  g->h0_dirty = true;
  g->h0_stale = true;
  g->seed_settings = g->settings;
  g->seeded = g->settings;
  return OCEAN_OK;
}

int seed_h0(ocean_generator* g, int update_spectrum, const void*& seed)
{
  if (update_spectrum && !g->update_spectrum && g->memo_h0 && same_h0_inputs(g->settings, g->seeded))
    update_spectrum = 0;
  if (g->update_spectrum || update_spectrum)
  {
    const bool fused = update_spectrum && !g->update_spectrum && frame_path(g) == FramePath::HalfBlocked && g->hs;
    g->update_spectrum = false;
    return fused ? fused_reseed(g, seed) : ocean_generator_generate_spectrum(g);
  }
  TRY(materialise_h0(g));
  if (g->h0_block != h0_block(g))
    TRY(generate_spectrum_with(g, g->h0_settings));
  return OCEAN_OK;
}

FrameParams frame_params(const ocean_generator* g)
{
  FrameParams fp{};
  fp.cascades = g->cascades;
  for (int c = 0; c < g->cascades; c++)
  {
    const ocean_settings& s = g->settings[c];
    fp.c[c].dk = 2.0f * 3.14159265358f / s.planeSize;
    fp.c[c].time = s.time;
    fp.c[c].g = s.g;
    fp.c[c].h = s.h;
  }
  return fp;
}

int half_slab_columns(ocean_generator* g, const FrameParams& fp, float4* out, const Gen4Put* put,
                      hipStream_t col_stream)
{
  ocean_fft* f = g->fft;
  const hipError_t eb = hslab_buffers(g);
  if (eb != hipSuccess)
    return alloc_fail(eb, "column pass buffers");
  hipStream_t cs = col_stream ? col_stream : f->stream;
  if (g->cols_ev_valid)
    HIP_TRY(hipStreamWaitEvent(cs, g->cols_ev, 0), "column pass: after the last column pass");
  if (cs != f->stream && g->h0_dirty)
  {
    if (!g->put_h0)
      HIP_TRY(hipEventCreateWithFlags(&g->put_h0, hipEventDisableTiming), "column pass: event");
    HIP_TRY(hipEventRecord(g->put_h0, f->stream), "column pass: stream event");
    HIP_TRY(hipStreamWaitEvent(cs, g->put_h0, 0), "column pass: stream order");
    g->h0_dirty = false;
  }
  Gen4Put timed_put = put ? *put : Gen4Put{};
  EventPair pp{3, nullptr, nullptr};
  if (put && g->profiling)
  {
    pp.a = take_event(g);
    pp.b = take_event(g);
    timed_put.start = pp.a;
  }
  if (frame_path(g) == FramePath::FourStep)
    HIP_TRY(timed(g, 1, [&] {
              return launch_gen4_columns(f->logn, fp, g->g4, g->h0, g->ranks > 1 ? g->h0row : nullptr,
                                         put && put->parts ? put->parts : g->parts, out ? (void*)out : (void*)g->xbuf,
                                         f->twiddles, f->tw2, cs, f->cus, put ? &timed_put : nullptr);
            }, cs),
            "column pass (half spectrum, four-step)");
  else
    HIP_TRY(timed(g, 1, [&] {
              return launch_half_slab_columns(f->logn, fp, g->hsl, g->ranks, g->h0, g->ranks == 1, g->h0row,
                                              out ? (void*)out : (void*)g->xbuf, f->twiddles, cs, f->cus, g->hs,
                                              f->device_cus, put ? &timed_put : nullptr);
            }, cs),
            "column pass (half spectrum, strip-dealt)");
  if (pp.a)
  {
    HIP_TRY(hipEventRecord(pp.b, put && put->stream ? put->stream : cs), "column pass: put event");
    g->pending.push_back(pp);
  }
  for (hipEvent_t* ev : {&g->cols_ev, &g->h0r_ev})
    if (!*ev)
      HIP_TRY(hipEventCreateWithFlags(ev, hipEventDisableTiming), "column pass: event");
  HIP_TRY(hipEventRecord(g->cols_ev, cs), "column pass: end event");
  HIP_TRY(hipEventRecord(g->h0r_ev, put && put->stream ? put->stream : cs), "column pass: end event");
  g->cols_ev_valid = true;
  return OCEAN_OK;
}

int overlapped_columns(ocean_generator* g, const FrameParams& fp, const void* seed)
{
  ocean_fft* f = g->fft;
  const int s = g->oslot;
  if (g->h0_dirty)
  {
    HIP_TRY(hipEventRecord(g->oh0, f->stream), "overlap: h0 event");
    HIP_TRY(hipStreamWaitEvent(g->side, g->oh0, 0), "overlap: h0 wait");
    g->h0_dirty = false;
  }
  if (g->orows_valid[s])
    HIP_TRY(hipStreamWaitEvent(g->side, g->orows[s], 0), "overlap: slot wait");
  const HalfFields& fl = g->fields[s];
  HIP_TRY(timed(g, 1, [&] {
            return launch_half_columns(f->logn, fp, g->h0, fl.gab, fl.gde, fl.gc, fl.spec, f->twiddles, g->side, f->cus,
                                       g->hs, f->device_cus, seed, g->h0_block);
          }, g->side),
          "column pass (half spectrum, overlapped)");
  HIP_TRY(hipEventRecord(g->ocols[s], g->side), "overlap: column event");
  return OCEAN_OK;
}

float4* own_exchange(const ocean_generator* g) { return half_slab_path(g) ? nullptr : g->inter; }

int land_frames_in_flight(ocean_generator* g)
{
  if (peers_pending(g->peers))
    TRY(ocean_peers_flush(g->peers));
  return ocean_generator_slab_flush(g);
}
}

int generator_columns(ocean_generator* g, float timestep, int update_spectrum, float4* out, const Gen4Put* put,
                      hipStream_t col_stream)
{
  ocean_fft* f = g->fft;
  g->rates_fresh = false;
  g->kin_fresh = false;
  for (auto& s : g->settings)
    s.time += timestep;
  const void* seed = nullptr;
  TRY(seed_h0(g, update_spectrum, seed));
  const FrameParams fp = frame_params(g);
  if (put && !half_slab_path(g))
    return fail(OCEAN_ERR_INVALID, "column pass: the one-sided exchange needs a half-spectrum slab path (N >= 1024)");
  switch (frame_path(g))
  {
    case FramePath::FourStep:
    case FramePath::StripDealt:
      TRY(half_slab_columns(g, fp, out, put, col_stream));
      break;
    case FramePath::HalfBlocked:
      if (g->overlap)
        TRY(overlapped_columns(g, fp, seed));
      else
        HIP_TRY(timed(g, 1, [&] {
                  const HalfFields& fl = g->fields[0];
                  return launch_half_columns(f->logn, fp, g->h0, fl.gab, fl.gde, fl.gc, fl.spec, f->twiddles, f->stream,
                                             f->cus, g->hs, f->device_cus, seed, g->h0_block);
                }),
                "column pass (half spectrum)");
      break;
    case FramePath::Full:
      HIP_TRY(timed(g, 1, [&] {
                return launch_cols_evolve(f->logn, fp, g->geom, g->h0, out, f->twiddles, f->stream, f->cus,
                                          default_keep(f->logn));
              }),
              "column pass");
      break;
  }
  g->frame = fp;
  return OCEAN_OK;
}

FrameState current_frame(const ocean_generator* g)
{
  FrameState fs{g->frame, FoamParams{}};
  for (int c = 0; c < g->cascades; c++)
    fs.foam.displacement[c] = g->settings[c].displacement;
  return fs;
}

int generator_rows(ocean_generator* g, const float4* in, const FrameState& fs, hipStream_t row_stream, int row_cus)
{
  ocean_fft* f = g->fft;
  g->mips_fresh = false;
  g->bounds_fresh = false;
  const int rcus = row_cus > 0 && row_cus < f->cus ? row_cus : f->cus;
  if (row_stream && !half_slab_path(g))
    return fail(OCEAN_ERR_INVALID, "row pass: a row stream needs a half-spectrum slab path");
  hipStream_t rs = row_stream ? row_stream : f->stream;
  switch (frame_path(g))
  {
    case FramePath::FourStep:
      HIP_TRY(timed(g, 2, [&] {
                return launch_gen4_rows(f->logn, fs.frame, g->g4, in ? (const void*)in : (const void*)g->xbuf, g->maps,
                                        g->jac, fs.foam, f->twiddles, f->tw2, rs, rcus);
              }, rs),
              "row pass (half spectrum, four-step)");
      break;
    case FramePath::StripDealt:
      HIP_TRY(timed(g, 2, [&] {
                return launch_half_slab_rows(f->logn, fs.frame, g->hsl, in ? (const void*)in : (const void*)g->xbuf,
                                             g->rm_ab, g->rm_de, g->rm_c, g->maps, g->jac, fs.foam, f->twiddles,
                                             f->tw2, rs, rcus);
              }, rs),
              "row pass (half spectrum, strip-dealt)");
      break;
    case FramePath::HalfBlocked:
    {
      const int s = g->overlap ? g->oslot : 0;
      const HalfFields& fl = g->fields[s];
      if (g->overlap)
        HIP_TRY(hipStreamWaitEvent(f->stream, g->ocols[s], 0), "overlap: column wait");
      HIP_TRY(timed(g, 2, [&] {
                return launch_half_rows(f->logn, fs.frame, fl.gab, fl.gde, fl.gc, fl.spec, g->maps, g->jac, fs.foam,
                                        f->twiddles, f->stream, f->cus);
              }),
              g->overlap ? "row pass (half spectrum, overlapped)" : "row pass (half spectrum)");
      if (g->overlap)
      {
        HIP_TRY(hipEventRecord(g->orows[s], f->stream), "overlap: row event");
        g->orows_valid[s] = true;
        g->oslot = s ^ 1;
      }
      break;
    }
    case FramePath::Full:
      HIP_TRY(timed(g, 2, [&] {
                return launch_rows_final(f->logn, g->cascades, g->geom, in, g->scratch, g->maps, g->jac, fs.foam,
                                         f->twiddles, f->stream, f->cus);
              }),
              "row pass");
      break;
  }
  return OCEAN_OK;
}

int materialise_h0(ocean_generator* g)
{
  return g->h0_stale ? generate_spectrum_with(g, g->seed_settings) : OCEAN_OK;
}

extern "C" {

int ocean_generator_create(ocean_generator** out, ocean_fft* fft, int cascades)
{
  if (!out || !fft)
    return fail(OCEAN_ERR_INVALID, "ocean_generator_create: null argument");
  *out = nullptr;
  if (cascades < 1 || cascades > OCEAN_MAX_CASCADES)
    return fail(OCEAN_ERR_INVALID, "ocean_generator_create: cascades must be in [1, 64]");
  return generator_alloc(out, fft, cascades, 0, 1, false);
}

int ocean_generator_create_slab(ocean_generator** out, ocean_fft* fft, int rank, int ranks)
{
  if (!out || !fft)
    return fail(OCEAN_ERR_INVALID, "ocean_generator_create_slab: null argument");
  *out = nullptr;
  const int blk = spectrum_block(fft->logn);
  if (ranks < 1 || ranks > 16 || (ranks & (ranks - 1)) != 0 || rank < 0 || rank >= ranks)
    return fail(OCEAN_ERR_INVALID, "ocean_generator_create_slab: ranks must be a power of two in [1, 16], 0 <= rank < ranks");
  const int w = fft->n / ranks;
  if (w % blk != 0 || w < fft->n / 16 || w < slab_min_width(fft->logn))
    return fail(OCEAN_ERR_INVALID, "ocean_generator_create_slab: N / ranks = " + std::to_string(w) +
                                       " is below this size's minimum slab width " +
                                       std::to_string(slab_min_width(fft->logn)));
  return generator_alloc(out, fft, 1, rank, ranks, true);
}

int ocean_generator_destroy(ocean_generator* g)
{
  if (!g)
    return OCEAN_OK;
  if (g->comm_stream)
    (void)hipStreamSynchronize(g->comm_stream);
  if (g->peers)
    peers_detach(g->peers);
  if (g->fft)
    (void)hipStreamSynchronize(g->fft->stream);
  if (g->side)
    (void)hipStreamSynchronize(g->side);
  for (hipStream_t st : {g->comm_stream, g->side})
    if (st)
      (void)hipStreamDestroy(st);
  for (auto& p : g->pending)
    for (hipEvent_t ev : {p.a, p.b})
      g->pool.push_back(ev);
  for (hipEvent_t ev : g->pool)
    (void)hipEventDestroy(ev);
  for (hipEvent_t ev : {g->cols_done[0], g->cols_done[1], g->xchg_done[0], g->xchg_done[1], g->rows_done[0],
                        g->rows_done[1], g->put_h0, g->cols_ev, g->h0r_ev, g->ocols[0], g->ocols[1], g->orows[0],
                        g->orows[1], g->oh0})
    if (ev)
      (void)hipEventDestroy(ev);
  const HalfFields &f0 = g->fields[0], &f1 = g->fields[1];
  for (void* p : {(void*)g->h0, (void*)g->inter, (void*)g->scratch, (void*)g->maps, (void*)g->jac, (void*)g->xsend[0],
                  (void*)g->xsend[1], (void*)g->xrecv[0], (void*)g->xrecv[1], (void*)f0.gab, (void*)f0.gde, (void*)f0.gc,
                  (void*)f0.spec, (void*)f1.gab, (void*)f1.gde, (void*)f1.gc, (void*)f1.spec, (void*)g->hs,
                  (void*)g->h0row, g->seedc, (void*)g->rm_ab, (void*)g->rm_de, (void*)g->rm_c, (void*)g->parts,
                  (void*)g->xbuf, (void*)g->mips, (void*)g->rates, (void*)g->kin, (void*)g->bounds, (void*)g->foam, g->foam_counts,
                  (void*)g->deposit_acc, g->deposit_counts})
    if (p)
      (void)hipFree(p);
  delete g;
  return OCEAN_OK;
}

int ocean_generator_cascades(const ocean_generator* g) { return g ? g->cascades : 0; }

ocean_settings* ocean_generator_settings(ocean_generator* g, int c)
{
  if (!g || c < 0 || c >= g->cascades)
  {
    fail(OCEAN_ERR_INVALID, "ocean_generator_settings: cascade out of range");
    return nullptr;
  }
  return &g->settings[c];
}

int ocean_generator_generate_spectrum(ocean_generator* g)
{
  if (!g)
    return fail(OCEAN_ERR_INVALID, "ocean_generator_generate_spectrum: null generator");
  return generate_spectrum_with(g, g->settings);
}

int ocean_generator_set_half_spectrum(ocean_generator* g, int enable)
{
  if (!g)
    return fail(OCEAN_ERR_INVALID, "ocean_generator_set_half_spectrum: null generator");
  TRY(land_frames_in_flight(g));
  if (!enable && g->overlap)
    TRY(ocean_generator_set_frame_overlap(g, 0));
  if (enable && g->half_kind == HalfKind::None)
    return fail(OCEAN_ERR_INVALID, "ocean_generator_set_half_spectrum: N = 1024 .. 16384 only");
  const bool was_on = g->half_on, was_slab_path = half_slab_path(g);
  g->half_on = enable != 0;
  const hipError_t e = path_buffers(g);
  if (e != hipSuccess)
  {
    g->half_on = was_on;
    return alloc_fail(e, "ocean_generator_set_half_spectrum");
  }
  if ((was_slab_path && g->ranks > 1) != (half_slab_path(g) && g->ranks > 1))
    g->update_spectrum = true;
  return OCEAN_OK;
}

int ocean_generator_set_frame_overlap(ocean_generator* g, int enable)
{
  if (!g)
    return fail(OCEAN_ERR_INVALID, "ocean_generator_set_frame_overlap: null generator");
  if (enable && frame_path(g) != FramePath::HalfBlocked)
    return fail(OCEAN_ERR_INVALID, "ocean_generator_set_frame_overlap: whole grids of N = 1024 .. 4096 on the "
                                   "half-spectrum path only");
  ocean_fft* f = g->fft;
  if (enable && !g->overlap)
  {
    hipError_t e = hipSuccess;
    if (!g->side)
      e = hipStreamCreateWithFlags(&g->side, hipStreamNonBlocking);
    for (hipEvent_t* ev : {&g->ocols[0], &g->ocols[1], &g->orows[0], &g->orows[1], &g->oh0})
      if (e == hipSuccess && !*ev)
        e = hipEventCreateWithFlags(ev, hipEventDisableTiming);
    if (e == hipSuccess)
      e = half_fields(g, 1);
    if (e == hipSuccess)
      e = hipEventRecord(g->oh0, f->stream);
    if (e == hipSuccess)
      e = hipStreamWaitEvent(g->side, g->oh0, 0);
    if (e != hipSuccess)
      return alloc_fail(e, "ocean_generator_set_frame_overlap");
    g->orows_valid[0] = g->orows_valid[1] = false;
    g->oslot = 0;
    g->h0_dirty = false;
    g->overlap = true;
  }
  else if (!enable && g->overlap)
  {
    for (int s = 0; s < 2; s++)
      if (g->orows_valid[s])
        HIP_TRY(hipStreamWaitEvent(f->stream, g->orows[s], 0), "ocean_generator_set_frame_overlap");
    HIP_TRY(hipEventRecord(g->oh0, g->side), "ocean_generator_set_frame_overlap");
    HIP_TRY(hipStreamWaitEvent(f->stream, g->oh0, 0), "ocean_generator_set_frame_overlap");
    g->overlap = false;
  }
  return OCEAN_OK;
}

int ocean_generator_set_h0_memo(ocean_generator* g, int enable)
{
  if (!g)
    return fail(OCEAN_ERR_INVALID, "ocean_generator_set_h0_memo: null generator");
  g->memo_h0 = enable != 0;
  return OCEAN_OK;
}

int ocean_generator_set_four_step(ocean_generator* g, int enable)
{
  if (!g)
    return fail(OCEAN_ERR_INVALID, "ocean_generator_set_four_step: null generator");
  TRY(land_frames_in_flight(g));
  g->four_step = enable != 0;
  if (half_slab_path(g))
  {
    const hipError_t e = hslab_buffers(g);
    if (e != hipSuccess)
      return alloc_fail(e, "ocean_generator_set_four_step");
  }
  return OCEAN_OK;
}

int ocean_generator_frame_bytes(const ocean_generator* g, double per_point[2])
{
  if (!g || !per_point)
    return fail(OCEAN_ERR_INVALID, "ocean_generator_frame_bytes: null argument");
  const double n = g->fft->n;
  switch (const FramePath path = frame_path(g))
  {
    case FramePath::FourStep:
    {
      const double kept = (n / 2 + 1) / n;
      per_point[0] = (16.0 + 40.0 + 80.0) * kept;
      per_point[1] = 40.0 * kept + 36.0;
      break;
    }
    case FramePath::HalfBlocked:
    case FramePath::StripDealt:
    {
      const double kept = (n / 2 + spectrum_block(g->fft->logn)) / n;
      per_point[0] = 16.0 * kept + 40.0 * kept;
      per_point[1] = 40.0 * kept + 36.0 + (path == FramePath::StripDealt ? 80.0 * kept : 0.0);
      break;
    }
    case FramePath::Full:
      per_point[0] = 48.0;
      per_point[1] = 68.0 + (rows_need_transpose(g->fft->logn) ? 64.0 : 0.0);
      break;
  }
  return OCEAN_OK;
}

int ocean_generator_calculate(ocean_generator* g, float timestep, int update_spectrum)
{
  if (!g)
    return fail(OCEAN_ERR_INVALID, "ocean_generator_calculate: null generator");
  if (g->ranks != 1)
    return fail(OCEAN_ERR_INVALID, "ocean_generator_calculate: slab generators step with "
                                   "ocean_generator_slab_columns / exchange / ocean_generator_slab_rows");
  float4* buf = own_exchange(g);
  TRY(generator_columns(g, timestep, update_spectrum, buf));
  return generator_rows(g, buf, current_frame(g));
}

size_t ocean_generator_exchange_bytes(const ocean_generator* g)
{
  if (!g)
    return 0;
  if (half_slab_path(g))
    return hslab_xbuf_bytes(g);
  return (size_t)g->cascades * 2 * g->fft->n * g->geom.w * sizeof(float4);
}

int ocean_generator_slab_columns(ocean_generator* g, float timestep, int update_spectrum, float* send)
{
  if (!g)
    return fail(OCEAN_ERR_INVALID, "ocean_generator_slab_columns: null generator");
  return generator_columns(g, timestep, update_spectrum, send ? reinterpret_cast<float4*>(send) : own_exchange(g));
}

int ocean_generator_slab_rows(ocean_generator* g, const float* recv)
{
  if (!g)
    return fail(OCEAN_ERR_INVALID, "ocean_generator_slab_rows: null generator");
  return generator_rows(g, recv ? reinterpret_cast<const float4*>(recv) : own_exchange(g), current_frame(g));
}

int ocean_slab_layout(size_t texture_size, int rank, int ranks, int half, int64_t out[6])
{
  int logn = 0;
  while (logn < 15 && ((size_t)1 << logn) < texture_size)
    logn++;
  if (!out || ((size_t)1 << logn) != texture_size || logn < 4 || logn > 14 || ranks < 1 || ranks > 16 ||
      (ranks & (ranks - 1)) != 0 || rank < 0 || rank >= ranks)
    return fail(OCEAN_ERR_INVALID, "ocean_slab_layout: N a power of two in [16, 16384], ranks a power of two <= 16");
  if (half && !half_slab_supported(logn))
    return fail(OCEAN_ERR_INVALID, "ocean_slab_layout: the half-spectrum path needs N >= 1024");
  if (half == 2 && !gen4_supported(logn))
    return fail(OCEAN_ERR_INVALID, "ocean_slab_layout: the four-step path needs N = 8192 or 16384");
  const int n = 1 << logn, w = n / ranks;
  if (half == 2)
  {
    const Gen4Geom q = gen4_geom(logn, 1, rank, ranks, ranks == 1);
    const int64_t v[6] = {q.u0, q.cols, q.nyq, q.w, (int64_t)q.blk_bytes, (int64_t)q.blk_bytes * ranks};
    std::memcpy(out, v, sizeof(v));
  }
  else if (half)
  {
    const HalfSlab h = half_slab_geom(logn, rank, ranks);
    const int64_t blk = (int64_t)half_slab_block_bytes(logn, 1, h);
    const int64_t v[6] = {h.strip0, h.nstrips, h.S, h.w, blk, blk * ranks};
    std::memcpy(out, v, sizeof(v));
  }
  else
  {
    const int64_t blk = (int64_t)2 * w * w * sizeof(float4);
    const int64_t v[6] = {(int64_t)rank * w, w, 0, w, blk, blk * ranks};
    std::memcpy(out, v, sizeof(v));
  }
  return OCEAN_OK;
}

int ocean_generator_slab_info(const ocean_generator* g, int* rank, int* ranks, int* row0, int* rows)
{
  if (!g)
    return fail(OCEAN_ERR_INVALID, "ocean_generator_slab_info: null generator");
  if (rank)
    *rank = g->rank;
  if (ranks)
    *ranks = g->ranks;
  if (row0)
    *row0 = g->rank * g->geom.w;
  if (rows)
    *rows = g->geom.w;
  return OCEAN_OK;
}

float* ocean_generator_initial_spectrum(ocean_generator* g, int c)
{
  if (!g || c < 0 || c >= g->cascades)
    return nullptr;
  if (materialise_h0(g) != OCEAN_OK)
    return nullptr;
  g->seeded.clear();
  g->h0_dirty = true;
  return reinterpret_cast<float*>(g->h0 + h0_texels(g) * c);
}

int ocean_generator_spectrum_block(const ocean_generator* g)
{
  return g ? (g->h0_block > 0 ? g->h0_block : h0_block(g)) : 0;
}

int ocean_generator_set_profiling(ocean_generator* g, int enable)
{
  if (!g)
    return fail(OCEAN_ERR_INVALID, "ocean_generator_set_profiling: null generator");
  g->profiling = enable != 0;
  return OCEAN_OK;
}

int ocean_generator_kernel_times4(ocean_generator* g, double ms_total[4], int64_t launches[4])
{
  if (!g)
    return fail(OCEAN_ERR_INVALID, "ocean_generator_kernel_times: null generator");
  HIP_TRY(hipStreamSynchronize(g->fft->stream), "hipStreamSynchronize");
  for (auto& p : g->pending)
  {
    float ms = 0.0f;
    HIP_TRY(hipEventSynchronize(p.b), "hipEventSynchronize");
    HIP_TRY(hipEventElapsedTime(&ms, p.a, p.b), "hipEventElapsedTime");
    g->ms[p.kind] += ms;
    g->launches[p.kind] += 1;
    g->pool.push_back(p.a);
    g->pool.push_back(p.b);
  }
  g->pending.clear();
  for (int k = 0; k < 4; k++)
  {
    if (ms_total)
      ms_total[k] = g->ms[k];
    if (launches)
      launches[k] = g->launches[k];
    g->ms[k] = 0;
    g->launches[k] = 0;
  }
  return OCEAN_OK;
}

int ocean_generator_kernel_times(ocean_generator* g, double ms_total[3], int64_t launches[3])
{
  double m[4];
  int64_t l[4];
  const int rc = ocean_generator_kernel_times4(g, m, l);
  for (int k = 0; rc == OCEAN_OK && k < 3; k++)
  {
    if (ms_total)
      ms_total[k] = m[k];
    if (launches)
      launches[k] = l[k];
  }
  return rc;
}

int ocean_debug_copy(void* dst, const void* src, size_t bytes, int workgroups, void* hip_stream)
{
  if ((bytes > 0 && (!dst || !src)) || bytes % 16 != 0 || workgroups < 1 || workgroups > 65536 ||
      (reinterpret_cast<uintptr_t>(dst) | reinterpret_cast<uintptr_t>(src)) % 16 != 0)
    return fail(OCEAN_ERR_INVALID, "ocean_debug_copy: null or unaligned pointer, bytes not a multiple of 16, or "
                                   "workgroups outside [1, 65536]");
  if (bytes == 0)
    return OCEAN_OK;
  HIP_TRY(launch_debug_copy(dst, src, bytes, workgroups, (hipStream_t)hip_stream), "debug copy");
  return OCEAN_OK;
}

int ocean_debug_hash(const uint32_t* xy, int count, uint32_t* raw, float* uv, void* hip_stream)
{
  if (!xy || !raw || !uv || count < 0)
    return fail(OCEAN_ERR_INVALID, "ocean_debug_hash: null argument");
  if (count == 0)
    return OCEAN_OK;
  HIP_TRY(launch_hash(xy, count, raw, reinterpret_cast<float2*>(uv), (hipStream_t)hip_stream), "hash");
  return OCEAN_OK;
}

}
```

oceansimulation_amd/csrc/ocean_capi_internal.h:

```cpp
#pragma once

#include "oceanfft.h"

#include <hip/hip_runtime.h>

#include <string>
#include <vector>

#include "ocean_internal.h"

using namespace oceanfft;

struct __attribute__((visibility("hidden"))) EventPair
{
  int kind;
  hipEvent_t a, b;
};

struct FrameState
{
  FrameParams frame{};
  FoamParams foam{};
};

struct HalfFields
{
  float4* gab = nullptr;
  float4* gde = nullptr;
  float2* gc = nullptr;
  float4* spec = nullptr;
};

enum class HalfKind
{
  None,
  Blocked,
  Dealt
};

enum class FramePath
{
  Full,
  HalfBlocked,
  StripDealt,
  FourStep
};

struct ocean_fft
{
  int n = 0;
  int logn = 0;
  int device = 0;
  int device_cus = 0;
  int cus = 0;
  hipStream_t stream = nullptr;
  float2* twiddles = nullptr;
  float2* tw2 = nullptr;
  float2* twm = nullptr;
  float4* work = nullptr;
  int work_images = 0;
  size_t work_texels = 0;
  size_t work_limit = (size_t)-1;
  float4* surf_atlas = nullptr;
  size_t surf_atlas_texels = 0;
};

struct ocean_generator
{
  ocean_fft* fft = nullptr;
  int cascades = 0;
  int rank = 0, ranks = 1;
  SlabGeom geom{};
  std::vector<ocean_settings> settings;
  bool update_spectrum = true;
  float4* h0 = nullptr;
  float4* inter = nullptr;
  float4* scratch = nullptr;
  float4* maps = nullptr;
  float* jac = nullptr;
  HalfKind half_kind = HalfKind::None;
  bool half_on = false;
  bool four_step = true;
  FrameParams frame{};
  float2* hs = nullptr;
  HalfFields fields[2];
  bool slab = false;
  HalfSlab hsl{};
  Gen4Geom g4{};
  float4* h0row = nullptr;
  float4* rm_ab = nullptr;
  float4* rm_de = nullptr;
  float2* rm_c = nullptr;
  unsigned char* parts = nullptr;
  unsigned char* xbuf = nullptr;
  size_t xbuf_bytes = 0;
  void* seedc = nullptr;
  std::vector<unsigned char> seedc_host;
  bool h0_stale = false;
  std::vector<ocean_settings> seed_settings;
  int h0_block = 0;
  std::vector<ocean_settings> h0_settings;
  std::vector<ocean_settings> seeded;
  bool memo_h0 = true;
  unsigned char* xsend[2] = {nullptr, nullptr};
  unsigned char* xrecv[2] = {nullptr, nullptr};
  size_t xslot_bytes = 0;
  hipStream_t comm_stream = nullptr;
  hipEvent_t cols_done[2] = {nullptr, nullptr}, xchg_done[2] = {nullptr, nullptr}, rows_done[2] = {nullptr, nullptr};
  bool rows_recorded[2] = {false, false};
  int pending_slot = -1;
  FrameState slot_state[2];
  int64_t frames_issued = 0;
  ocean_peers* peers = nullptr;
  hipEvent_t put_h0 = nullptr;
  hipEvent_t cols_ev = nullptr, h0r_ev = nullptr;
  bool cols_ev_valid = false;
  bool overlap = false;
  hipStream_t side = nullptr;
  hipEvent_t ocols[2] = {nullptr, nullptr}, orows[2] = {nullptr, nullptr}, oh0 = nullptr;
  bool orows_valid[2] = {false, false};
  int oslot = 0;
  bool h0_dirty = false;
  float* mips = nullptr;
  bool mips_fresh = false;
  float4* rates = nullptr;
  bool rates_fresh = false;
  KinematicsDepths depths{};
  float4* kin = nullptr;
  bool kin_fresh = false;
  float* bounds = nullptr;
  bool bounds_fresh = false;
  std::vector<ocean_foam_settings> foam_settings;
  float* foam = nullptr;
  void* foam_counts = nullptr;
  unsigned long long* deposit_acc = nullptr;
  void* deposit_counts = nullptr;
  bool profiling = false;
  std::vector<EventPair> pending;
  std::vector<hipEvent_t> pool;
  double ms[4] = {0, 0, 0, 0};
  int64_t launches[4] = {0, 0, 0, 0};
};

#pragma GCC visibility push(hidden)

inline thread_local std::string g_err;

inline int fail(int code, const std::string& msg)
{
  g_err = msg;
  return code;
}

inline int hip_fail(hipError_t e, const char* what)
{
  return fail(OCEAN_ERR_HIP, std::string(what) + ": " + hipGetErrorString(e));
}

#define HIP_TRY(expr, what)                                                                        \
  do                                                                                               \
  {                                                                                                \
    hipError_t e_ = (expr);                                                                        \
    if (e_ != hipSuccess)                                                                          \
      return hip_fail(e_, what);                                                                   \
  } while (0)

#define TRY(expr)                                                                                  \
  do                                                                                               \
  {                                                                                                \
    const int rc_ = (expr);                                                                        \
    if (rc_ != OCEAN_OK)                                                                           \
      return rc_;                                                                                  \
  } while (0)

inline int alloc_fail(hipError_t e, const std::string& who)
{
  return fail(e == hipErrorOutOfMemory ? OCEAN_ERR_OOM : OCEAN_ERR_HIP, who + ": " + hipGetErrorString(e));
}

template <typename T>
hipError_t alloc_if_null(T*& ptr, size_t bytes, hipError_t e = hipSuccess)
{
  if (e != hipSuccess || ptr)
    return e;
  e = hipMalloc(&ptr, bytes);
  if (e != hipSuccess)
    ptr = nullptr;
  return e;
}

inline HalfKind half_kind_of(int logn, bool slab)
{
  if (!slab && half_spectrum_supported(logn))
    return HalfKind::Blocked;
  return half_slab_supported(logn) && (slab || logn > 12) ? HalfKind::Dealt : HalfKind::None;
}

inline FramePath frame_path(const ocean_generator* g)
{
  if (!g->half_on || g->half_kind == HalfKind::None)
    return FramePath::Full;
  if (g->half_kind == HalfKind::Blocked)
    return FramePath::HalfBlocked;
  return g->four_step && gen4_supported(g->fft->logn) ? FramePath::FourStep : FramePath::StripDealt;
}

inline bool half_slab_path(const ocean_generator* g)
{
  const FramePath p = frame_path(g);
  return p == FramePath::StripDealt || p == FramePath::FourStep;
}

int materialise_h0(ocean_generator* g);
hipError_t hslab_buffers(ocean_generator* g);
size_t hslab_xbuf_bytes(const ocean_generator* g);
int generator_columns(ocean_generator* g, float timestep, int update_spectrum, float4* out,
                      const Gen4Put* put = nullptr, hipStream_t col_stream = nullptr);
int generator_rows(ocean_generator* g, const float4* in, const FrameState& fs, hipStream_t row_stream = nullptr,
                   int row_cus = 0);
FrameState current_frame(const ocean_generator* g);

bool peers_pending(const ocean_peers* p);
void peers_detach(ocean_peers* p);

#pragma GCC visibility pop
```

oceansimulation_amd/csrc/ocean_internal.h:

```cpp
#pragma once

#include <hip/hip_runtime.h>

#include <cstdint>

namespace oceanfft
{

struct OceanSettings
{
  int32_t seed[2];
  float U_10;
  float theta_0;
  float F;
  float g;
  float swell;
  float h;
  float displacement;
  float time;
  float planeSize;
  float scale;
  float spread;
  int32_t boundWavelength;
  float wavelengthMin;
  float wavelengthMax;
};
static_assert(sizeof(OceanSettings) == 64, "GeneratorSettings is 64 bytes");

constexpr int kMaxCascades = 64;
constexpr int kMaxSurfaceCascades = 16;

struct SurfaceCascade
{
  const float4* height;
  const float4* disp;
  const float* jac;
  float plane;
  float scale;
  const float4* height_mip;
  const float4* disp_mip;
  const float* jac_mip;
};
struct SurfaceParams
{
  int count;
  int n;
  SurfaceCascade c[kMaxSurfaceCascades];
  float4* atlas;
};
struct SurfacePlane
{
  int res;
  float cam_x, cam_y, cam_z, fwd_x, fwd_z;
};

struct CascadeFrame
{
  float dk;
  float time;
  float g;
  float h;
};

struct FrameParams
{
  int cascades;
  int pad[3];
  CascadeFrame c[kMaxCascades];
};

struct FoamParams
{
  float displacement[kMaxCascades];
};

struct SlabGeom
{
  int x0;
  int w;
};

struct HalfSlab
{
  int strip0;
  int nstrips;
  int S;
  int w;
};

struct Gen4Geom
{
  int u0;
  int cols;
  int nyq;
  int lp;
  int w;
  int ranks;
  size_t h0_cstride;
  size_t h0_reg;
  size_t h0_nyq;
  size_t blk_bytes;
};

struct RowSrc
{
  const unsigned char* ab;
  const unsigned char* de;
  const unsigned char* c;
  size_t src_stride;
  int cpr;
  int lp;
  int nyq_src;
};

int spectrum_block(int logn);
hipError_t launch_generate_spectrum(const OceanSettings& s, int n, float4* h0, hipStream_t stream, int cus, int x0 = 0,
                                    int width = 0, int blk = 0);
bool half_spectrum_supported(int logn);
size_t half_field_texels(int logn);
size_t half_hs_bytes(int logn, int blocks);
int half_h0_block(int logn, int cascades);
hipError_t launch_half_columns(int logn, const FrameParams& fp, const float4* h0, float4* gab, float4* gcd, float2* ge,
                               float4* spec, const float2* tw, hipStream_t stream, int cus, float2* hs, int hs_blocks,
                               const void* seed_consts = nullptr, int h0_blk = 0);
size_t seed_consts_bytes();
void seed_consts(const OceanSettings& s, int n, void* out);
hipError_t launch_half_rows(int logn, const FrameParams& fp, const float4* gab, const float4* gcd, const float2* ge,
                            const float4* rcorr, float4* maps, float* jac, const FoamParams& foam, const float2* tw,
                            hipStream_t stream, int cus);
hipError_t launch_half_nyquist(const FrameParams& fp, int n, int blk, const float4* h0, float4* spec, const float4* h0row,
                               int copies, size_t copy_stride, const void* seed, hipStream_t stream, int cus,
                               const uint64_t* dst = nullptr, size_t dst_off = 0);
struct PeerWait
{
  const uint32_t* flags;
  int word0;
  int ranks;
  uint32_t target;
  long long deadline_ticks;
  uint32_t* err;
};
hipError_t launch_peer_wait(const PeerWait& w, hipStream_t stream);
hipError_t launch_peer_signal(uint32_t* const* flags, int ranks, int word, uint32_t value, hipStream_t stream);
hipError_t launch_peer_signal_release(uint32_t* const* flags, int ranks, int word, uint32_t value, uint32_t* counter,
                                      hipStream_t stream);
bool half_slab_supported(int logn);
int half_strips(int logn);
size_t half_slab_block_bytes(int logn, int cascades, const HalfSlab& h);
size_t half_slab_row_texels(int logn, int cascades, int w);
hipError_t launch_generate_spectrum_row(const OceanSettings& s, int n, float4* row, hipStream_t stream);
struct Gen4Put;
hipError_t launch_half_slab_columns(int logn, const FrameParams& fp, const HalfSlab& hsl, int ranks, const float4* h0,
                                    bool h0_full, const float4* h0row, void* send, const float2* tw,
                                    hipStream_t stream, int cus, float2* hs, int hs_blocks, const Gen4Put* put = nullptr);
hipError_t launch_half_slab_rows(int logn, const FrameParams& fp, const HalfSlab& hsl, const void* recv, float4* rm_ab,
                                 float4* rm_de, float2* rm_c, float4* maps, float* jac, const FoamParams& foam,
                                 const float2* tw, const float2* tw2, hipStream_t stream, int cus);
hipError_t launch_rows_ifft_rows(int logn, int rows, float4* data, const float2* tw, hipStream_t stream, int cus);
bool gen4_supported(int logn);
int gen4_h0_block();
Gen4Geom gen4_geom(int logn, int cascades, int rank, int ranks, bool whole_h0);
size_t gen4_parts_bytes(int logn, int cascades, const Gen4Geom& g);
struct Gen4Put
{
  const uint64_t* dst;
  const PeerWait* wait;
  int cus;
  hipEvent_t start = nullptr;
  hipStream_t stream = nullptr;
  hipEvent_t handoff = nullptr;
  void* parts = nullptr;
};
hipError_t launch_gen4_columns(int logn, const FrameParams& fp, const Gen4Geom& g, const float4* h0, const float4* h0row,
                               void* parts, void* send, const float2* tw, const float2* tw2, hipStream_t stream, int cus,
                               const Gen4Put* put = nullptr);
hipError_t launch_gen4_rows(int logn, const FrameParams& fp, const Gen4Geom& g, const void* recv, float4* maps, float* jac,
                            const FoamParams& foam, const float2* tw, const float2* tw2, hipStream_t stream, int cus);
bool fourstep_table(int logn);
bool ifft_fourstep_supported(int logn);
size_t ifft_fourstep_work_texels(int logn, int wc);
hipError_t launch_ifft_fourstep(int logn, int n_images, float4* images, float4* work, int wc, const float2* tw,
                                const float2* tw2, hipStream_t stream, int cus);
bool ifft_colfirst_supported(int logn);
hipError_t launch_ifft_colfirst(int logn, int n_images, float4* images, float4* work, const float2* tw,
                                hipStream_t stream, int cus);
bool ifft_pre_supported(int logn);
hipError_t launch_ifft_pre(int logn, int n_images, float4* images, float4* work, const float2* twn, const float2* twm,
                           hipStream_t stream, int cus);
hipError_t launch_surface(const SurfaceParams& p, const SurfacePlane& plane, const float2* xz, int64_t count,
                          float4* out, hipStream_t stream, int cus);
hipError_t launch_surface_query(const SurfaceParams& p, const float2* xz, int64_t count, int iterations,
                                float tolerance, float4* out, hipStream_t stream, int cus);
hipError_t launch_surface_lod(const SurfaceParams& p, const SurfacePlane& plane, const float* xzf, int64_t count,
                              float4* out, hipStream_t stream, int cus);
size_t mip_cascade_floats(int n);
hipError_t launch_build_mips(int n, int cascades, const float4* maps, const float* jac, float* mips,
                             hipStream_t stream);
hipError_t launch_rates_pack(int logn, const FrameParams& fp, int h0_blk, const float4* h0, float4* rates,
                             hipStream_t stream, int cus);
struct SurfaceRates
{
  const float4* height[kMaxSurfaceCascades];
  const float4* disp[kMaxSurfaceCascades];
};
hipError_t launch_surface_velocity(const SurfaceParams& p, const SurfaceRates& r, const float2* xz, int64_t count,
                                   float4* out, hipStream_t stream, int cus);
constexpr int kMaxDepthLayers = 8;
struct KinematicsDepths
{
  int layers;
  float d[kMaxDepthLayers];
};
hipError_t launch_kinematics_pack(int logn, const FrameParams& fp, const KinematicsDepths& kd, int h0_blk,
                                  const float4* h0, float4* out, hipStream_t stream, int cus);
struct WaterLayers
{
  const float4* map[kMaxSurfaceCascades];
  int layers;
  float d[kMaxDepthLayers];
};
hipError_t launch_water_kinematics(const SurfaceParams& p, const WaterLayers& w, const float* xyz, int64_t count,
                                   int iterations, float tolerance, float4* out, hipStream_t stream, int cus);
int bounds_tiles(int n);
size_t bounds_floats(int n, int cascades);
hipError_t launch_build_bounds(int n, int cascades, const float4* maps, const float* jac, float* bounds,
                               hipStream_t stream, int cus);
struct RaycastParams
{
  const float* bounds[kMaxSurfaceCascades];
  float step;
  int max_steps, refine, iterations;
  float tolerance, slope, pad;
};
hipError_t launch_surface_raycast(const SurfaceParams& p, const RaycastParams& rc, const float4* rays, int64_t n_rays,
                                  float4* out, hipStream_t stream, int cus);
struct CameraParams
{
  float pos[3], right[3], up[3], fwd[3];
  float tan_half, near_plane, far_plane, lod_scale;
  int width, height;
};
struct ShadingParams
{
  float wave[3], scatter[3], sky[3], light[3], L[3];
  float cthr, cfade, fog_begin, fog_density;
};
hipError_t launch_camera_rays(const CameraParams& cam, float4* rays, hipStream_t stream);
hipError_t launch_camera_render(const SurfaceParams& p, const RaycastParams& rc, const CameraParams& cam,
                                const ShadingParams& sh, float4* image, float4* aux, uint32_t* image8,
                                hipStream_t stream, int cus);
struct FoamCascade
{
  float a;
  float bias, gain, level, dt;
};
struct FoamStep
{
  const float* jac;
  float* foam;
  uint32_t* partial;
  int64_t* table;
  int nn;
  int tiles;
  int cascades;
  FoamCascade c[kMaxCascades];
};
int foam_tiles(int n);
size_t foam_counts_bytes(int n, int cascades);
hipError_t launch_foam_step(int n, int cascades, const float* jac, float* foam, void* counts, const FoamCascade* c,
                            hipStream_t stream, int cus);
struct SurfaceFoam
{
  const float* foam[kMaxSurfaceCascades];
};
hipError_t launch_surface_foam(const SurfaceParams& p, const SurfaceFoam& f, const SurfacePlane& plane, const float2* xz,
                               int64_t count, float4* out, hipStream_t stream, int cus);
struct CameraWaterLayers
{
  float foam_color[3];
  float foam_lo, foam_hi, foam_opacity;
  float4* aux2;
  unsigned long long* key;
  uint32_t* hits;
  float* foam;
};
struct CameraSpray
{
  const float* records;
  const int64_t* count_device;
  int64_t max_records;
  unsigned long long* key;
  uint32_t* hits;
  const float* foam;
  float4* base;
  const float4* aux;
  float color[3];
  float radius, opacity;
  int max_half;
};
size_t camera_layers_scratch_bytes(int width, int height);
void camera_layers_scratch(void* scratch, int width, int height, unsigned long long*& key, uint32_t*& hits,
                           float*& foam, float4*& image, float4*& aux);
hipError_t launch_camera_render_foam(const SurfaceParams& p, const RaycastParams& rc, const CameraParams& cam,
                                     const ShadingParams& sh, const SurfaceFoam& fm, const CameraWaterLayers& lw,
                                     float4* image, float4* aux, uint32_t* image8, hipStream_t stream, int cus);
hipError_t launch_camera_aux2_none(const CameraParams& cam, float4* aux2, hipStream_t stream, int cus);
hipError_t launch_camera_spray(const CameraParams& cam, const ShadingParams& sh, const CameraSpray& s, float4* image,
                               uint32_t* image8, float4* aux2, hipStream_t stream, int cus);
constexpr int kHullTilePoints = 64;
struct HullTile
{
  int64_t offset;
  int first, count, body, slot;
  int seg, pad;
};

struct HullBody
{
  int64_t offset;
  int first, count;
};

struct HullFold
{
  int body, slot, tiles, pad;
};

struct HullCall
{
  const float4* points;
  const HullTile* tiles;
  const HullBody* bodies;
  const float* poses;
  float4* loads;
  float4* partial;
  float4* point_out;
  int items;
  int iterations;
  float tolerance, rho_g;
};

hipError_t launch_hulls_loads(const SurfaceParams& p, const SurfaceRates& r, bool velocity, const HullCall& h,
                              const HullFold* folds, int n_folds, hipStream_t stream, int cus);
struct HullStep
{
  float* poses;
  const float4* props;
  const float4* ext;
  float h;
  float gx, gy, gz;
  int substeps;
  int last;
};

hipError_t launch_hulls_step(const SurfaceParams& p, const SurfaceRates& r, bool velocity, const HullCall& h,
                             HullStep st, int substeps, const HullFold* folds, int n_folds, hipStream_t stream,
                             int cus);
struct SprayPair
{
  const float* jac;
  float threshold, rate;
  uint32_t seed;
  int index;
};
struct SprayCall
{
  int64_t* table;
  int64_t* offset;
  uint32_t* partial;
  float* out;
  int64_t capacity;
  int n, logn, nn;
  int tiles;
  int pairs;
  float dt;
  uint32_t step;
  SprayPair c[kMaxSurfaceCascades];
};
struct SprayTiles
{
  int32_t t[kMaxSurfaceCascades][2];
};
size_t spray_scratch_bytes(int n);
void spray_scratch(void* scratch, int n, SprayCall& s);
hipError_t launch_spray_emit(const SprayCall& s, const SurfaceParams& p, const SurfaceRates& r, const SprayTiles& tiles,
                             bool velocity, hipStream_t stream, int cus);
constexpr int kParticleItem = 256;
constexpr int kParticleCounts = 8;
struct ParticleCall
{
  int64_t* table;
  int64_t* offset;
  uint32_t* partial;
  unsigned long long* ballots;
  float* cur;
  float* next;
  const float* emit;
  const int64_t* emit_counts;
  float* landed_out;
  int64_t landed_capacity;
  int64_t capacity;
  float dt, gravity, drag, wind[3], lifetime, gain, lift;
  int iterations;
  float tolerance;
};
int64_t particle_items(int64_t capacity);
size_t particle_scratch_bytes(int64_t capacity);
void particle_scratch(void* scratch, int64_t capacity, ParticleCall& c);
hipError_t launch_particles_step(const ParticleCall& c, const SurfaceParams& p, hipStream_t stream, int cus);
hipError_t launch_particles_reset(int64_t* table, int64_t alive, hipStream_t stream);
constexpr int kFoamDepositItem = 256;
constexpr int kFoamDepositCounts = 50;
constexpr int kFoamDepositMaxGrid = 4096;
struct FoamDepositPair
{
  float* foam;
  unsigned long long* acc;
  float plane, amount, per_speed;
  int pad;
};
struct FoamDepositCall
{
  const float* records;
  const int64_t* count_device;
  int64_t max_records;
  int64_t* table;
  uint32_t* taps;
  uint32_t* owned;
  int n;
  int pairs;
  int grid_add, grid_apply;
  FoamDepositPair c[kMaxSurfaceCascades];
};
size_t foam_deposit_scratch_bytes();
void foam_deposit_scratch(void* scratch, FoamDepositCall& c);
hipError_t launch_foam_deposit(FoamDepositCall c, bool merge, hipStream_t stream, int cus);
void launch_surface_atlas(const SurfaceParams& p, hipStream_t stream, int cus);
size_t surface_atlas_texels(const SurfaceParams& p);
bool surface_use_atlas(const SurfaceParams& p, int64_t points);
bool surface_query_use_atlas(const SurfaceParams& p, int64_t points, int iterations);
hipError_t launch_hash(const uint32_t* xy, int count, uint32_t* raw, float2* uv, hipStream_t stream);
hipError_t launch_debug_copy(void* dst, const void* src, size_t bytes, int workgroups, hipStream_t stream);
hipError_t launch_cols_evolve(int logn, const FrameParams& fp, const SlabGeom& g, const float4* h0, float4* inter,
                              const float2* tw, hipStream_t stream, int cus, int keep);
int default_keep(int logn);
int slab_min_width(int logn);
bool rows_need_transpose(int logn);
hipError_t launch_rows_final(int logn, int cascades, const SlabGeom& g, const float4* inter, float4* scratch,
                             float4* maps, float* jac, const FoamParams& foam, const float2* tw, hipStream_t stream,
                             int cus);
hipError_t launch_rows_ifft(int logn, int n_images, float4* images, const float2* tw, hipStream_t stream,
                            int cus);
hipError_t launch_cols(int logn, int n_images, float4* images, const float2* tw, hipStream_t stream, int cus);
int twiddle_entries(int logn);

}
```

oceansimulation_amd/waves.py:

```python
from __future__ import annotations

import ctypes

import numpy as np

from . import capi, hip
from .capi import (OceanFoamDepositSettings, OceanFoamSettings, OceanParticleSettings, OceanSettings, OceanSpraySettings,
                   check, lib)


def default_settings(**overrides) -> OceanSettings:
    s = OceanSettings()
    lib().ocean_default_settings(ctypes.byref(s))
    apply_settings(s, **overrides)
    return s


def apply_settings(s: OceanSettings, **overrides) -> OceanSettings:
    for k, v in overrides.items():
        if k == "seed":
            s.seed[0], s.seed[1] = int(v[0]), int(v[1])
        else:
            setattr(s, k, v)
    return s


def default_foam_settings(**overrides) -> OceanFoamSettings:
    s = OceanFoamSettings()
    lib().ocean_default_foam_settings(ctypes.byref(s))
    return apply_foam_settings(s, **overrides)


def apply_foam_settings(s: OceanFoamSettings, **overrides) -> OceanFoamSettings:
    for k, v in overrides.items():
        if k not in ("bias", "gain", "decay", "level"):
            raise AttributeError(f"ocean_foam_settings has no field {k!r}")
        setattr(s, k, v)
    return s


def default_foam_deposit_settings(**overrides) -> OceanFoamDepositSettings:
    s = OceanFoamDepositSettings()
    lib().ocean_default_foam_deposit_settings(ctypes.byref(s))
    return apply_foam_deposit_settings(s, **overrides)


def apply_foam_deposit_settings(s: OceanFoamDepositSettings, **overrides) -> OceanFoamDepositSettings:
    for k, v in overrides.items():
        if k not in ("amount", "per_speed"):
            raise AttributeError(f"ocean_foam_deposit_settings has no field {k!r}")
        setattr(s, k, v)
    return s


def default_spray_settings(**overrides) -> OceanSpraySettings:
    s = OceanSpraySettings()
    lib().ocean_default_spray_settings(ctypes.byref(s))
    return apply_spray_settings(s, **overrides)


def apply_spray_settings(s: OceanSpraySettings, **overrides) -> OceanSpraySettings:
    for k, v in overrides.items():
        if k not in ("threshold", "rate", "seed"):
            raise AttributeError(f"ocean_spray_settings has no field {k!r}")
        setattr(s, k, v)
    return s


def default_particle_settings(**overrides) -> OceanParticleSettings:
    s = OceanParticleSettings()
    lib().ocean_default_particle_settings(ctypes.byref(s))
    return apply_particle_settings(s, **overrides)


def apply_particle_settings(s: OceanParticleSettings, **overrides) -> OceanParticleSettings:
    names = [f[0] for f in OceanParticleSettings._fields_]
    for k, v in overrides.items():
        if k not in names:
            raise AttributeError(f"ocean_particle_settings has no field {k!r}")
        if k == "wind":
            s.wind[0], s.wind[1], s.wind[2] = float(v[0]), float(v[1]), float(v[2])
        else:
            setattr(s, k, v)
    return s


class FFTCalculator:

    def __init__(self, texture_size: int = 512, stream: int | None = None):
        h = ctypes.c_void_p()
        check(lib().ocean_fft_create(ctypes.byref(h), texture_size, ctypes.c_void_p(stream or 0)),
              "ocean_fft_create")
        self._h = h
        self.texture_size = texture_size

    def GetTextureResolution(self) -> int:
        return int(lib().ocean_fft_texture_resolution(self._h))

    get_texture_resolution = GetTextureResolution

    def EncodeIFFT(self, image_ptr: int) -> None:
        check(lib().ocean_fft_encode_ifft(self._h, ctypes.c_void_p(image_ptr)), "ocean_fft_encode_ifft")

    encode_ifft = EncodeIFFT

    def encode_ifft_batch(self, images_ptr: int, n_images: int) -> None:
        check(lib().ocean_fft_encode_ifft_batch(self._h, ctypes.c_void_p(images_ptr), n_images),
              "ocean_fft_encode_ifft_batch")

    def synchronize(self) -> None:
        check(lib().ocean_fft_synchronize(self._h), "ocean_fft_synchronize")

    @property
    def cus(self) -> int:
        return int(lib().ocean_fft_device_cus(self._h))

    def set_cu_budget(self, cus: int) -> None:
        check(lib().ocean_fft_set_cu_budget(self._h, int(cus)), "ocean_fft_set_cu_budget")

    def debug_work_limit(self, nbytes: int | None) -> None:
        cap = ctypes.c_size_t(-1).value if nbytes is None else int(nbytes)
        check(lib().ocean_debug_fft_work_limit(self._h, cap), "ocean_debug_fft_work_limit")

    @property
    def handle(self):
        return self._h

    def close(self) -> None:
        if self._h:
            lib().ocean_fft_destroy(self._h)
            self._h = ctypes.c_void_p()

    def __del__(self):
        try:
            self.close()
        except Exception:
            pass


class Generator:

    def __init__(self, fft: FFTCalculator, cascades: int = 1):
        h = ctypes.c_void_p()
        check(lib().ocean_generator_create(ctypes.byref(h), fft.handle, cascades), "ocean_generator_create")
        self._h = h
        self.fft = fft
        self.n = fft.GetTextureResolution()
        self.cascades = cascades

    @property
    def handle(self):
        return self._h

    def set_half_spectrum(self, enable: bool) -> None:
        check(lib().ocean_generator_set_half_spectrum(self._h, 1 if enable else 0), "ocean_generator_set_half_spectrum")

    def set_four_step(self, enable: bool) -> None:
        check(lib().ocean_generator_set_four_step(self._h, 1 if enable else 0), "ocean_generator_set_four_step")

    def set_h0_memo(self, enable: bool) -> None:
        check(lib().ocean_generator_set_h0_memo(self._h, 1 if enable else 0), "ocean_generator_set_h0_memo")

    def set_frame_overlap(self, enable: bool) -> None:
        check(lib().ocean_generator_set_frame_overlap(self._h, 1 if enable else 0),
              "ocean_generator_set_frame_overlap")

    def frame_bytes(self):
        out = (ctypes.c_double * 2)()
        check(lib().ocean_generator_frame_bytes(self._h, out), "ocean_generator_frame_bytes")
        return float(out[0]), float(out[1])

    def GetOceanSettings(self, cascade: int = 0) -> OceanSettings:
        p = lib().ocean_generator_settings(self._h, cascade)
        if not p:
            raise capi.OceanError(capi.OCEAN_ERR_INVALID, "ocean_generator_settings")
        return p.contents

    get_ocean_settings = GetOceanSettings

    def CalculateOcean(self, timestep: float, update_ocean: bool = False) -> None:
        check(lib().ocean_generator_calculate(self._h, ctypes.c_float(timestep), 1 if update_ocean else 0),
              "ocean_generator_calculate")

    calculate_ocean = CalculateOcean

    def GenerateSpectrum(self) -> None:
        check(lib().ocean_generator_generate_spectrum(self._h), "ocean_generator_generate_spectrum")

    def GetHeightMap(self, cascade: int = 0) -> int:
        return int(lib().ocean_generator_height_map(self._h, cascade))

    def GetDisplacementMap(self, cascade: int = 0) -> int:
        return int(lib().ocean_generator_displacement_map(self._h, cascade))

    def GetJacobianMap(self, cascade: int = 0) -> int:
        return int(lib().ocean_generator_jacobian_map(self._h, cascade))

    def GetInitialSpectrum(self, cascade: int = 0) -> int:
        return int(lib().ocean_generator_initial_spectrum(self._h, cascade))

    def height_map_host(self, cascade: int = 0) -> np.ndarray:
        self.fft.synchronize()
        return hip.to_host(self.GetHeightMap(cascade), (self.n, self.n, 4))

    def displacement_map_host(self, cascade: int = 0) -> np.ndarray:
        self.fft.synchronize()
        return hip.to_host(self.GetDisplacementMap(cascade), (self.n, self.n, 4))

    def jacobian_map_host(self, cascade: int = 0) -> np.ndarray:
        self.fft.synchronize()
        return hip.to_host(self.GetJacobianMap(cascade), (self.n, self.n))

    def initial_spectrum_host(self, cascade: int = 0) -> np.ndarray:
        self.fft.synchronize()
        b = int(lib().ocean_generator_spectrum_block(self._h))
        blocked = hip.to_host(self.GetInitialSpectrum(cascade), (self.n // b, self.n, b, 4))
        return np.ascontiguousarray(blocked.transpose(1, 0, 2, 3).reshape(self.n, self.n, 4))

    def build_mips(self) -> None:
        check(lib().ocean_generator_build_mips(self._h), "ocean_generator_build_mips")

    def mip_levels(self) -> int:
        return int(lib().ocean_generator_mip_levels(self._h))

    def _mip_host(self, getter: str, cascade: int, level: int, channels: int) -> np.ndarray:
        ptr = getattr(lib(), getter)(self._h, int(cascade), int(level))
        if not ptr:
            raise capi.OceanError(capi.OCEAN_ERR_INVALID, getter)
        self.fft.synchronize()
        side = self.n >> level
        return hip.to_host(int(ptr), (side, side, channels) if channels > 1 else (side, side))

    def height_mip_host(self, cascade: int, level: int) -> np.ndarray:
        return self._mip_host("ocean_generator_height_mip", cascade, level, 4)

    def displacement_mip_host(self, cascade: int, level: int) -> np.ndarray:
        return self._mip_host("ocean_generator_displacement_mip", cascade, level, 4)

    def jacobian_mip_host(self, cascade: int, level: int) -> np.ndarray:
        return self._mip_host("ocean_generator_jacobian_mip", cascade, level, 1)

    def calculate_rates(self) -> None:
        check(lib().ocean_generator_calculate_rates(self._h), "ocean_generator_calculate_rates")

    def _rate_host(self, getter: str, cascade: int) -> np.ndarray:
        ptr = getattr(lib(), getter)(self._h, int(cascade))
        if not ptr:
            raise capi.OceanError(capi.OCEAN_ERR_INVALID, getter)
        self.fft.synchronize()
        return hip.to_host(int(ptr), (self.n, self.n, 4))

    def height_rate_map_host(self, cascade: int = 0) -> np.ndarray:
        return self._rate_host("ocean_generator_height_rate_map", cascade)

    def displacement_rate_map_host(self, cascade: int = 0) -> np.ndarray:
        return self._rate_host("ocean_generator_displacement_rate_map", cascade)

    def set_depth_layers(self, depths) -> None:
        d = np.ascontiguousarray(depths, np.float32).reshape(-1)
        check(lib().ocean_generator_set_depth_layers(self._h, d.ctypes.data_as(ctypes.POINTER(ctypes.c_float)),
                                                     int(d.shape[0])), "ocean_generator_set_depth_layers")

    def depth_layers(self) -> np.ndarray:
        out = np.zeros(8, np.float32)
        count = int(lib().ocean_generator_depth_layers(self._h, out.ctypes.data_as(ctypes.POINTER(ctypes.c_float))))
        return out[:count]

    def calculate_kinematics(self) -> None:
        check(lib().ocean_generator_calculate_kinematics(self._h), "ocean_generator_calculate_kinematics")

    def GetKinematicsMap(self, cascade: int = 0, layer: int = 0, image: int = 0) -> int:
        ptr = lib().ocean_generator_kinematics_map(self._h, int(cascade), int(layer), int(image))
        if not ptr:
            raise capi.OceanError(capi.OCEAN_ERR_INVALID, "ocean_generator_kinematics_map")
        return int(ptr)

    def kinematics_map_host(self, cascade: int = 0, layer: int = 0, image: int = 0) -> np.ndarray:
        ptr = self.GetKinematicsMap(cascade, layer, image)
        self.fft.synchronize()
        return hip.to_host(ptr, (self.n, self.n, 4))

    def BuildBounds(self) -> None:
        check(lib().ocean_generator_build_bounds(self._h), "ocean_generator_build_bounds")

    build_bounds = BuildBounds

    def GetBounds(self, cascade: int = 0) -> np.ndarray:
        out = np.zeros(18, np.float32)
        check(lib().ocean_generator_bounds(self._h, int(cascade), out.ctypes.data_as(ctypes.POINTER(ctypes.c_float))),
              "ocean_generator_bounds")
        return out.reshape(9, 2)

    get_bounds = GetBounds

    def bounds_device(self) -> int:
        ptr = lib().ocean_generator_bounds_device(self._h)
        if not ptr:
            raise capi.OceanError(capi.OCEAN_ERR_INVALID, "ocean_generator_bounds_device")
        return int(ptr)

    def AdvanceFoam(self, dt: float) -> None:
        check(lib().ocean_generator_advance_foam(self._h, ctypes.c_float(dt)), "ocean_generator_advance_foam")

    advance_foam = AdvanceFoam

    def ResetFoam(self) -> None:
        check(lib().ocean_generator_reset_foam(self._h), "ocean_generator_reset_foam")

    reset_foam = ResetFoam

    def GetFoamSettings(self, cascade: int = 0) -> OceanFoamSettings:
        p = lib().ocean_generator_foam_settings(self._h, cascade)
        if not p:
            raise capi.OceanError(capi.OCEAN_ERR_INVALID, "ocean_generator_foam_settings")
        return p.contents

    get_foam_settings = GetFoamSettings

    def GetFoamMap(self, cascade: int = 0) -> int:
        ptr = lib().ocean_generator_foam_map(self._h, int(cascade))
        if not ptr:
            raise capi.OceanError(capi.OCEAN_ERR_INVALID, "ocean_generator_foam_map")
        return int(ptr)

    def foam_map_host(self, cascade: int = 0) -> np.ndarray:
        ptr = self.GetFoamMap(cascade)
        self.fft.synchronize()
        return hip.to_host(ptr, (self.n, self.n))

    def GetFoamCounts(self, cascade: int = 0) -> np.ndarray:
        out = np.zeros(3, np.int64)
        check(lib().ocean_generator_foam_counts(self._h, int(cascade), out.ctypes.data_as(ctypes.POINTER(ctypes.c_int64))),
              "ocean_generator_foam_counts")
        return out

    get_foam_counts = GetFoamCounts

    def foam_counts_device(self) -> int:
        ptr = lib().ocean_generator_foam_counts_device(self._h)
        if not ptr:
            raise capi.OceanError(capi.OCEAN_ERR_INVALID, "ocean_generator_foam_counts_device")
        return int(ptr)

    def set_profiling(self, enable: bool) -> None:
        check(lib().ocean_generator_set_profiling(self._h, 1 if enable else 0), "ocean_generator_set_profiling")

    def kernel_times(self):
        ms = (ctypes.c_double * 3)()
        cnt = (ctypes.c_int64 * 3)()
        check(lib().ocean_generator_kernel_times(self._h, ms, cnt), "ocean_generator_kernel_times")
        return list(ms), list(cnt)

    def close(self) -> None:
        if self._h:
            lib().ocean_generator_destroy(self._h)
            self._h = ctypes.c_void_p()

    def __del__(self):
        try:
            self.close()
        except Exception:
            pass


def debug_copy(dst_ptr: int, src_ptr: int, nbytes: int, workgroups: int, stream: int | None = None) -> None:
    check(lib().ocean_debug_copy(ctypes.c_void_p(dst_ptr), ctypes.c_void_p(src_ptr), nbytes, workgroups,
                                 ctypes.c_void_p(stream or 0)), "ocean_debug_copy")


def debug_hash(xy_dev_ptr: int, count: int, raw_dev_ptr: int, uv_dev_ptr: int, stream: int | None = None) -> None:
    check(lib().ocean_debug_hash(ctypes.c_void_p(xy_dev_ptr), count, ctypes.c_void_p(raw_dev_ptr),
                                 ctypes.c_void_p(uv_dev_ptr), ctypes.c_void_p(stream or 0)), "ocean_debug_hash")
```

Before: 62.29 billion.

## Compute Nyquist column in a separate ahead-of-time launch overlapped with main columns

Adds a 'nyquist ahead' mode in which the half-spectrum Nyquist strip (one extra column per cascade) is computed by a dedicated one-column-per-workgroup kernel into double-buffered side buffers, likely on a side stream. The main column pass then skips that last strip, and the row kernels read the Nyquist pair from the side buffers. This is meant to remove the straggler cost of the odd last strip from the main column grid. It costs extra buffers, events and cross-stream synchronisation. It is on by default only for N=2048 with 3 cascades.

After: 61.05 billion. 0.98x the previous value.

```diff
diff --git a/include/oceanfft.h b/include/oceanfft.h
--- a/include/oceanfft.h
+++ b/include/oceanfft.h
@@ -68,6 +68,9 @@
 int ocean_generator_set_four_step(ocean_generator* gen, int enable);
 int ocean_generator_set_h0_memo(ocean_generator* gen, int enable);
 int ocean_generator_set_frame_overlap(ocean_generator* gen, int enable);
+int ocean_generator_set_nyquist_ahead(ocean_generator* gen, int enable);
+int ocean_generator_nyquist_ahead(const ocean_generator* gen);
+int ocean_generator_nyquist_time(ocean_generator* gen, double* ms_total, int64_t* launches);
 int ocean_generator_frame_bytes(const ocean_generator* gen, double per_point[2]);
 
 int ocean_generator_create_slab(ocean_generator** out, ocean_fft* fft, int rank, int ranks);
diff --git a/oceansimulation_amd/capi.py b/oceansimulation_amd/capi.py
--- a/oceansimulation_amd/capi.py
+++ b/oceansimulation_amd/capi.py
@@ -291,6 +291,9 @@
     "ocean_generator_set_four_step": (_i, [_vp, _i]),
     "ocean_generator_set_h0_memo": (_i, [_vp, _i]),
     "ocean_generator_set_frame_overlap": (_i, [_vp, _i]),
+    "ocean_generator_set_nyquist_ahead": (_i, [_vp, _i]),
+    "ocean_generator_nyquist_ahead": (_i, [_vp]),
+    "ocean_generator_nyquist_time": (_i, [_vp, ctypes.POINTER(ctypes.c_double), ctypes.POINTER(ctypes.c_int64)]),
     "ocean_generator_frame_bytes": (_i, [_vp, _vp]),
     "ocean_slab_layout": (_i, [_sz, _i, _i, _i, ctypes.POINTER(ctypes.c_int64)]),
     "ocean_comm_unique_id": (_i, [_vp]),
diff --git a/oceansimulation_amd/csrc/device/k_half_cols.h b/oceansimulation_amd/csrc/device/k_half_cols.h
--- a/oceansimulation_amd/csrc/device/k_half_cols.h
+++ b/oceansimulation_amd/csrc/device/k_half_cols.h
@@ -37,21 +37,21 @@
 }
 
 
-template <int LOGN_, bool SEED_>
+template <int LOGN_, bool SEED_, bool NA_ = false>
 struct ColsWhole
 {
   static constexpr int LOGN = LOGN_, LA = SEED_ ? 0 : kStream;
-  static constexpr bool SLAB = false, SEED = SEED_, PUT = false, NYQ = true;
+  static constexpr bool SLAB = false, SEED = SEED_, PUT = false, NYQ = !NA_, NA = NA_, NCOL = false;
   static constexpr int RG = kHalfRG, RGC = kHalfRGC, FB = 4;
   static constexpr int CPI = ColFirstCfg<LOGN_>::B, HB = ColFirstCfg<LOGN_>::B;
   static constexpr int HL = kHalfHL, HK = SEED_ ? kHalfHKSeed : LOGN_ == 12 ? kHalfHK : 2;
 };
 
-template <int LOGN_, bool SEED_, int HB_>
+template <int LOGN_, bool SEED_, int HB_, bool NA_ = false>
 struct ColsHalfStrip
 {
   static constexpr int LOGN = LOGN_, LA = SEED_ ? 0 : kStream;
-  static constexpr bool SLAB = false, SEED = SEED_, PUT = false, NYQ = true;
+  static constexpr bool SLAB = false, SEED = SEED_, PUT = false, NYQ = !NA_, NA = NA_, NCOL = false;
   static constexpr int RG = kHalfRG2, RGC = kHalfRGC2, FB = 2;
   static constexpr int CPI = 2, HB = HB_;
   static constexpr int HL = kHalfHL, HK = SEED_ ? kHalfHKSeed : LOGN_ == 12 ? kHalfHK : 2;
@@ -61,41 +61,57 @@
 struct ColsSlab
 {
   static constexpr int LOGN = LOGN_, LA = kStream;
-  static constexpr bool SLAB = true, SEED = false, PUT = PUT_, NYQ = false;
+  static constexpr bool SLAB = true, SEED = false, PUT = PUT_, NYQ = false, NA = false, NCOL = false;
   static constexpr int RG = 1, RGC = 1, FB = 4;
   static constexpr int CPI = ColFirstCfg<LOGN_>::B, HB = ColFirstCfg<LOGN_>::B;
   static constexpr int HL = kHalfHL, HK = LOGN_ == 13 ? 1 : kHalfHK - 1;
 };
 
+template <int LOGN_, int HB_>
+struct ColsNyquist
+{
+  static constexpr int LOGN = LOGN_, LA = kStream;
+  static constexpr bool SLAB = false, SEED = false, PUT = false, NYQ = true, NA = false, NCOL = true;
+  static constexpr int RG = 1, RGC = 1, FB = 4;
+  static constexpr int CPI = 1, HB = HB_;
+  static constexpr int HL = 0, HK = 8;
+};
+
 template <typename Sh>
 struct ColsLaunch
 {
   using S = FftShape<Sh::LOGN>;
   static constexpr int WG = S::T * Sh::CPI;
   static constexpr int LDS = ((S::TW_ENTRIES * 8 + 15) / 16) * 16 + Sh::CPI * S::PADDED * 8 + Sh::HL * WG * 16;
-  static constexpr int items(int cascades, int nstrips) { return cascades * nstrips * (ColFirstCfg<Sh::LOGN>::B / Sh::CPI); }
+  static constexpr int items(int cascades, int nstrips)
+  {
+    return Sh::NCOL ? cascades : cascades * nstrips * (ColFirstCfg<Sh::LOGN>::B / Sh::CPI);
+  }
   static constexpr int max_grid(int hs_blocks) { return Sh::SLAB ? hs_blocks : hs_blocks * (1024 / WG); }
 };
 
 template <typename Sh>
-__global__ __launch_bounds__(ColsLaunch<Sh>::WG, Sh::CPI < ColFirstCfg<Sh::LOGN>::B ? 4 : 1) void k_cols_half(
+__global__ __launch_bounds__(ColsLaunch<Sh>::WG, Sh::NCOL ? 3 : Sh::CPI < ColFirstCfg<Sh::LOGN>::B ? 4 : 1) void k_cols_half(
     FrameParams fp, const float4* __restrict__ h0, float4* __restrict__ gab, float4* __restrict__ gde,
     float2* __restrict__ gc, const float2* __restrict__ tw_glob, float2* __restrict__ hs, HalfSlab hsl,
     unsigned char* __restrict__ send, int h0_full, const SpectrumConsts* __restrict__ seed)
 {
   constexpr int LOGN = Sh::LOGN, LA = Sh::LA, RG = Sh::RG, RGC = Sh::RGC, CPI = Sh::CPI, HL = Sh::HL, HK = Sh::HK,
                 FB = Sh::FB, HB = Sh::HB;
-  constexpr bool SLAB = Sh::SLAB, SEED = Sh::SEED, PUT = Sh::PUT, NYQ = Sh::NYQ;
+  constexpr bool SLAB = Sh::SLAB, SEED = Sh::SEED, PUT = Sh::PUT, NYQ = Sh::NYQ, NA = Sh::NA, NCOL = Sh::NCOL;
   using S = FftShape<LOGN>;
   using K = ColFirstCfg<LOGN>;
   using HC = HalfCfg<LOGN>;
-  constexpr int N = S::N, T = S::T, B = K::B, STRIPS = HC::STRIPS, WG = T * CPI, HALVES = B / CPI;
+  constexpr int N = S::N, T = S::T, B = K::B, STRIPS = HC::STRIPS, WG = T * CPI, HALVES = NCOL ? 1 : B / CPI;
   static_assert(SLAB ? HC::SLAB_SUPPORTED : HC::SUPPORTED, "half-spectrum path: one strip per item (B = 4 unless SLAB)");
-  static_assert(CPI * HALVES == B && HALVES <= 2 && (HALVES == 1 || !SLAB), "whole or half strips");
+  static_assert(NCOL || (CPI * HALVES == B && HALVES <= 2 && (HALVES == 1 || !SLAB)), "whole or half strips");
+  static_assert(!NCOL || (CPI == 1 && HL + HK == 8 && !SLAB && !SEED && !NA && RG == 1 && RGC == 1 && FB == 4),
+                "NCOL: one column per item, every H pair in VGPRs or LDS (no scratch slice)");
+  static_assert(!NA || (!SLAB && !NYQ), "NA: whole grids, the Nyquist work in a launch of its own");
   static_assert(HL >= 0 && HK >= 0 && HL + HK <= 8, "H pairs outside the scratch");
   static_assert(FB == 4 || (FB == CPI && HALVES == 2 && !SLAB && RG > 1 && RGC > 1), "FB: half-strip fields");
   static_assert(!PUT || SLAB, "PUT: the strip-dealt slab stores");
-  static_assert(HB == B || (HB == CPI && HALVES == 2 && !SLAB), "HB: half strips over 2-column h0 strips");
+  static_assert(HB == B || (HB == CPI && HALVES == 2 && !SLAB) || (NCOL && HB == 2), "HB: half strips over 2-column h0 strips");
   static_assert(!NYQ || !SLAB, "NYQ: whole grids (send is the spec output)");
   constexpr int XB = CPI * S::PADDED * 8;
   extern __shared__ __attribute__((aligned(16))) unsigned char smem[];
@@ -104,13 +120,13 @@
   float4* hlds = reinterpret_cast<float4*>(static_cast<unsigned char*>(xch) + XB);
   load_twiddles<LOGN>(tw, tw_glob);
 
-  const int nstrips = SLAB ? hsl.nstrips : STRIPS;
+  const int nstrips = SLAB ? hsl.nstrips : NCOL ? 1 : NA ? STRIPS - 1 : STRIPS;
   const int total = fp.cascades * nstrips * HALVES;
   const float dim = (float)N;
   for (int item = HALVES > 1 ? xcd_pair_slot(blockIdx.x, gridDim.x) : (int)blockIdx.x; item < total; item += gridDim.x)
   {
     const int hh = HALVES > 1 ? item % HALVES : 0, si = HALVES > 1 ? item / HALVES : item;
-    const int c = si / nstrips, s = si - c * nstrips;
+    const int c = si / nstrips, s = NCOL ? STRIPS - 1 : si - c * nstrips;
     const int sg = SLAB ? hsl.strip0 + s : s;
     if (HALVES > 1 && sg == STRIPS - 1 && hh != 0)
       continue;
@@ -219,7 +235,16 @@
 #pragma unroll
       for (int m = 0; m < 16; m++)
       {
-        if constexpr (SLAB)
+        if constexpr (NCOL)
+        {
+          if (round == 0)
+            st4s<kStream>(gab + (size_t)c * N, i * 16, m * T * 16, pair_raw(v[m]));
+          else if (round == 1)
+            st4s<kStream>(gde + (size_t)c * N, i * 16, m * T * 16, pair_raw(v[m]));
+          else
+            st2s<kStream>(gc + (size_t)c * N, i * 8, m * T * 8, make_float2(v[m].re.x, v[m].im.x));
+        }
+        else if constexpr (SLAB)
         {
           const size_t part = (size_t)fp.cascades * hsl.S * hsl.w * B;
           const int q = (m * T) / hsl.w, yl0 = (m * T) % hsl.w;
diff --git a/oceansimulation_amd/csrc/device/k_half_rows.h b/oceansimulation_amd/csrc/device/k_half_rows.h
--- a/oceansimulation_amd/csrc/device/k_half_rows.h
+++ b/oceansimulation_amd/csrc/device/k_half_rows.h
@@ -100,12 +100,14 @@
     {
       if (i == 0 && m == 8)
       {
-        const int off = RM ? r * rs.lp + rs.cpr : half_group_offset<LOGN, RG, FB>(y, N / 2 / FB);
-        const int offc = RM ? off : half_group_offset<LOGN, RGC, FB>(y, N / 2 / FB);
+        const bool ahead = !RM && rs.ab != nullptr;
+        const size_t nbase = ahead ? (size_t)c * N : base;
+        const int off = RM ? r * rs.lp + rs.cpr : ahead ? y : half_group_offset<LOGN, RG, FB>(y, N / 2 / FB);
+        const int offc = RM ? off : ahead ? y : half_group_offset<LOGN, RGC, FB>(y, N / 2 / FB);
         const size_t ns = RM ? (size_t)rs.nyq_src * rs.src_stride : 0;
-        const float4* fab = RM ? reinterpret_cast<const float4*>(rs.ab + ns) + base : gab + base;
-        const float4* fde = RM ? reinterpret_cast<const float4*>(rs.de + ns) + base : gde + base;
-        const float2* fc = RM ? reinterpret_cast<const float2*>(rs.c + ns) + base : gc + base;
+        const float4* fab = RM || ahead ? reinterpret_cast<const float4*>(rs.ab + ns) + nbase : gab + base;
+        const float4* fde = RM || ahead ? reinterpret_cast<const float4*>(rs.de + ns) + nbase : gde + base;
+        const float2* fc = RM || ahead ? reinterpret_cast<const float2*>(rs.c + ns) + nbase : gc + base;
         const float kx = -(dim / 2.0f) * dk;
         float2 cc;
         if (img == 1)
diff --git a/oceansimulation_amd/csrc/device/k_rows_hp.h b/oceansimulation_amd/csrc/device/k_rows_hp.h
--- a/oceansimulation_amd/csrc/device/k_rows_hp.h
+++ b/oceansimulation_amd/csrc/device/k_rows_hp.h
@@ -114,24 +114,26 @@
       }
       if (i == 0)
       {
-        const int off = RM ? rs.cpr : half_group_offset<LOGN, RG, FB>(y, N / 2 / FB);
-        const int offc = RM ? off : half_group_offset<LOGN, RGC, FB>(y, N / 2 / FB);
+        const bool ahead = !RM && rs.ab != nullptr;
+        const size_t nbase = ahead ? (size_t)c * N : base;
+        const int off = RM ? rs.cpr : ahead ? y : half_group_offset<LOGN, RG, FB>(y, N / 2 / FB);
+        const int offc = RM ? off : ahead ? y : half_group_offset<LOGN, RGC, FB>(y, N / 2 / FB);
         const size_t ns = RM ? (size_t)rs.nyq_src * rs.src_stride : 0;
-        const float4* fab = RM ? reinterpret_cast<const float4*>(rs.ab + ns) : gab;
-        const float4* fde = RM ? reinterpret_cast<const float4*>(rs.de + ns) : gde;
-        const float2* fc = RM ? reinterpret_cast<const float2*>(rs.c + ns) : gc;
+        const float4* fab = RM || ahead ? reinterpret_cast<const float4*>(rs.ab + ns) : gab;
+        const float4* fde = RM || ahead ? reinterpret_cast<const float4*>(rs.de + ns) : gde;
+        const float2* fc = RM || ahead ? reinterpret_cast<const float2*>(rs.c + ns) : gc;
         const float kx = -(dim / 2.0f) * dk;
         if (RM || img == 0)
-          cnyq = ld2<0>(fc + base, offc * 8);
+          cnyq = ld2<0>(fc + nbase, offc * 8);
         const float2 cc = cnyq;
         if (img == 0)
         {
-          const CPair p = raw_pair(ld4<LA>(fab + base, off * 16));
+          const CPair p = raw_pair(ld4<LA>(fab + nbase, off * 16));
           v[8] = CPair{f2v{(1.0f - kx) * p.re.x, -p.im.y - kx * cc.x}, f2v{(1.0f - kx) * p.im.x, p.re.y - kx * cc.y}};
         }
         else
         {
-          const CPair q = raw_pair(ld4<LA>(fde + base, off * 16));
+          const CPair q = raw_pair(ld4<LA>(fde + nbase, off * 16));
           const float kx2 = kx * kx;
           v[8] = CPair{f2v{-(q.im.x - kx2 * cc.y), -q.re.y + kx * q.im.x}, f2v{q.re.x - kx2 * cc.x, -q.im.y - kx * q.re.x}};
         }
diff --git a/oceansimulation_amd/csrc/launch_half.hip b/oceansimulation_amd/csrc/launch_half.hip
--- a/oceansimulation_amd/csrc/launch_half.hip
+++ b/oceansimulation_amd/csrc/launch_half.hip
@@ -18,10 +18,18 @@
 
 constexpr bool half_strip_launch(int logn, int cascades) { return (logn == 12 || logn == 11) && cascades <= 2; }
 
+constexpr bool nyquist_ahead_default(int logn, int cascades) { return logn == 11 && cascades == 3; }
+bool half_nyquist_ahead_default(int logn, int cascades)
+{
+  return half_spectrum_supported(logn) && nyquist_ahead_default(logn, cascades);
+}
+
 template <int LOGN, typename V>
-hipError_t select_half_cols(int cascades, bool seed, int h0_blk, V&& visit)
+hipError_t select_half_cols(int cascades, bool seed, int h0_blk, bool ahead, V&& visit)
 {
   constexpr int B = ColFirstCfg<LOGN>::B;
+  if (seed && ahead)
+    return hipErrorInvalidValue;
   if constexpr (LOGN == 12 || LOGN == 11)
     if (half_strip_launch(LOGN, cascades))
     {
@@ -29,10 +37,14 @@
         return hipErrorInvalidValue;
       if (seed)
         return visit(ColsHalfStrip<LOGN, true, B>{});
+      if (ahead)
+        return h0_blk == B ? visit(ColsHalfStrip<LOGN, false, B, true>{}) : visit(ColsHalfStrip<LOGN, false, 2, true>{});
       return h0_blk == B ? visit(ColsHalfStrip<LOGN, false, B>{}) : visit(ColsHalfStrip<LOGN, false, 2>{});
     }
   if (h0_blk != 0 && h0_blk != B)
     return hipErrorInvalidValue;
+  if (ahead)
+    return visit(ColsWhole<LOGN, false, true>{});
   return seed ? visit(ColsWhole<LOGN, true>{}) : visit(ColsWhole<LOGN, false>{});
 }
 
@@ -67,7 +79,7 @@
   (void)with_logn(logn, [&](auto L) -> hipError_t {
     constexpr int LOGN = decltype(L)::value;
     if constexpr (HalfCfg<LOGN>::SUPPORTED)
-      return select_half_cols<LOGN>(cascades, false, 0, [&](auto sh) {
+      return select_half_cols<LOGN>(cascades, false, 0, false, [&](auto sh) {
         hb = decltype(sh)::HB;
         return hipSuccess;
       });
@@ -90,7 +102,7 @@
 
 hipError_t launch_half_columns(int logn, const FrameParams& fp, const float4* h0, float4* gab, float4* gcd, float2* ge,
                                float4* spec, const float2* tw, hipStream_t stream, int cus, float2* hs, int hs_blocks,
-                               const void* seed_consts, int h0_blk)
+                               const void* seed_consts, int h0_blk, bool nyquist_ahead)
 {
   if (!hs)
     return hipErrorInvalidValue;
@@ -100,17 +112,65 @@
     if constexpr (!HalfCfg<LOGN>::SUPPORTED)
       return hipErrorInvalidValue;
     else
-      return select_half_cols<LOGN>(fp.cascades, seed != nullptr, h0_blk > 0 ? h0_blk : ColFirstCfg<LOGN>::B, [&](auto sh) {
-        return launch_cols_half<decltype(sh)>(fp, HalfCfg<LOGN>::STRIPS, h0, gab, gcd, ge, tw, hs, hs_blocks, HalfSlab{},
-                                              reinterpret_cast<unsigned char*>(spec), 1, seed, stream, cus);
-      });
+      return select_half_cols<LOGN>(fp.cascades, seed != nullptr, h0_blk > 0 ? h0_blk : ColFirstCfg<LOGN>::B,
+                                    nyquist_ahead, [&](auto sh) {
+        return launch_cols_half<decltype(sh)>(fp, HalfCfg<LOGN>::STRIPS - (nyquist_ahead ? 1 : 0), h0, gab, gcd, ge, tw,
+                                              hs, hs_blocks, HalfSlab{}, reinterpret_cast<unsigned char*>(spec), 1, seed,
+                                              stream, cus);
+      });
+  });
+}
+
+size_t half_nyquist_texels(int logn) { return (size_t)1 << logn; }
+
+hipError_t launch_half_nyquist_ahead(int logn, const FrameParams& fp, const float4* h0, const HalfNyquist& nq,
+                                     const float2* tw, hipStream_t stream, int cus, int h0_blk)
+{
+  if (!nq.ab || !nq.de || !nq.c || !nq.spec)
+    return hipErrorInvalidValue;
+  return with_logn(logn, [&](auto L) -> hipError_t {
+    constexpr int LOGN = decltype(L)::value;
+    if constexpr (!HalfCfg<LOGN>::SUPPORTED)
+      return hipErrorInvalidValue;
+    else
+    {
+      constexpr int B = ColFirstCfg<LOGN>::B;
+      auto go = [&](auto sh) -> hipError_t {
+        using Sh = decltype(sh);
+        using G = ColsLaunch<Sh>;
+        if constexpr (LOGN == 12)
+          static_assert(G::WG == 256 && G::LDS <= HpCfg::LDS + 1024, "ColsNyquist: a k_rows_hp workgroup's footprint");
+        auto kern = k_cols_half<Sh>;
+        (void)blocks_per_cu(kern, G::WG, G::LDS);
+        const int grid = fp.cascades < cus ? fp.cascades : cus;
+        if (grid < 1)
+          return hipErrorInvalidValue;
+        hipLaunchKernelGGL(kern, dim3(grid), dim3(G::WG), G::LDS, stream, fp, h0, nq.ab, nq.de, nq.c, tw,
+                           static_cast<float2*>(nullptr), HalfSlab{}, reinterpret_cast<unsigned char*>(nq.spec), 1,
+                           static_cast<const SpectrumConsts*>(nullptr));
+        return hipGetLastError();
+      };
+      const int hb = h0_blk > 0 ? h0_blk : B;
+      if (hb == B)
+        return go(ColsNyquist<LOGN, B>{});
+      if (hb == 2 && half_strip_launch(LOGN, fp.cascades))
+        return go(ColsNyquist<LOGN, 2>{});
+      return hipErrorInvalidValue;
+    }
   });
 }
 
 hipError_t launch_half_rows(int logn, const FrameParams& fp, const float4* gab, const float4* gcd, const float2* ge,
                             const float4* rcorr, float4* maps, float* jac, const FoamParams& foam, const float2* tw,
-                            hipStream_t stream, int cus)
-{
+                            hipStream_t stream, int cus, const HalfNyquist* nq)
+{
+  RowSrc nsrc{};
+  if (nq)
+  {
+    nsrc.ab = reinterpret_cast<const unsigned char*>(nq->ab);
+    nsrc.de = reinterpret_cast<const unsigned char*>(nq->de);
+    nsrc.c = reinterpret_cast<const unsigned char*>(nq->c);
+  }
   return with_logn(logn, [&](auto L) -> hipError_t {
     constexpr int LOGN = decltype(L)::value;
     if constexpr (!HalfCfg<LOGN>::SUPPORTED)
@@ -124,7 +184,7 @@
           auto kern = k_rows_hp<R::RG, R::RGC, false, R::FB, R::GRP, R::EARLY, R::MINB>;
           const int grid = persistent_grid(kern, 256, HpCfg::LDS, fp.cascades * S::N, cus);
           hipLaunchKernelGGL(kern, dim3(grid), dim3(256), HpCfg::LDS, stream, fp, gab, gcd, ge, rcorr, maps, jac, foam, tw, 0,
-                             RowSrc{});
+                             nsrc);
         }
         else
         {
@@ -132,7 +192,7 @@
           const int lds = ((S::TW_ENTRIES * 8 + 15) / 16) * 16 + lds_row_slots<LOGN>(2) * 8;
           const int grid = persistent_grid(kern, S::T * 2, lds, fp.cascades * (S::N / 2), cus);
           hipLaunchKernelGGL(kern, dim3(grid), dim3(S::T * 2), lds, stream, fp, gab, gcd, ge, rcorr, maps, jac, foam, tw, S::N,
-                             RowSrc{});
+                             nsrc);
         }
         return hipGetLastError();
       });
@@ -156,7 +216,7 @@
       return hipErrorInvalidValue;
     else
     {
-      const hipError_t ec = select_half_cols<LOGN>(cascades, false, 0, [&](auto sh) {
+      const hipError_t ec = select_half_cols<LOGN>(cascades, false, 0, false, [&](auto sh) {
         using C = decltype(sh);
         out[0] = C::FB, out[1] = C::RG, out[2] = C::RGC, out[3] = C::HB;
         return hipSuccess;
diff --git a/oceansimulation_amd/csrc/ocean_capi.cpp b/oceansimulation_amd/csrc/ocean_capi.cpp
--- a/oceansimulation_amd/csrc/ocean_capi.cpp
+++ b/oceansimulation_amd/csrc/ocean_capi.cpp
@@ -420,6 +420,7 @@
   g->slab = is_slab;
   g->half_kind = half_kind_of(fft->logn, is_slab);
   g->half_on = g->half_kind != HalfKind::None;
+  g->nyq_ahead = g->half_kind == HalfKind::Blocked && half_nyquist_ahead_default(fft->logn, cascades);
   g->hsl = half_slab_geom(fft->logn, rank, ranks);
   if (gen4_supported(fft->logn))
   {
@@ -680,6 +681,58 @@
   return OCEAN_OK;
 }
 
+hipError_t side_stream(ocean_generator* g, bool urgent)
+{
+  if (g->side)
+    return hipSuccess;
+  int least = 0, greatest = 0;
+  if (!urgent || hipDeviceGetStreamPriorityRange(&least, &greatest) != hipSuccess)
+    return hipStreamCreateWithFlags(&g->side, hipStreamNonBlocking);
+  return hipStreamCreateWithPriority(&g->side, hipStreamNonBlocking, greatest);
+}
+
+hipError_t nyquist_buffers(ocean_generator* g)
+{
+  hipError_t e = side_stream(g, true);
+  for (hipEvent_t* ev : {&g->nyq_done[0], &g->nyq_done[1], &g->nyq_read[0], &g->nyq_read[1], &g->oh0})
+    if (e == hipSuccess && !*ev)
+      e = hipEventCreateWithFlags(ev, hipEventDisableTiming);
+  const size_t t = half_nyquist_texels(g->fft->logn) * g->cascades;
+  for (HalfNyquist& q : g->nyq)
+  {
+    e = alloc_if_null(q.ab, t * sizeof(float4), e);
+    e = alloc_if_null(q.de, t * sizeof(float4), e);
+    e = alloc_if_null(q.c, t * sizeof(float2), e);
+    e = alloc_if_null(q.spec, (size_t)g->cascades * 2 * g->fft->n * sizeof(float4), e);
+  }
+  return e;
+}
+
+int nyquist_ahead_columns(ocean_generator* g, const FrameParams& fp)
+{
+  ocean_fft* f = g->fft;
+  const hipError_t eb = nyquist_buffers(g);
+  if (eb != hipSuccess)
+    return alloc_fail(eb, "column pass: Nyquist slots");
+  const int s = g->nyq_slot;
+  if (g->h0_dirty)
+  {
+    HIP_TRY(hipEventRecord(g->oh0, f->stream), "nyquist ahead: h0 event");
+    HIP_TRY(hipStreamWaitEvent(g->side, g->oh0, 0), "nyquist ahead: h0 wait");
+    g->h0_dirty = false;
+  }
+  if (g->nyq_read_valid[s])
+    HIP_TRY(hipStreamWaitEvent(g->side, g->nyq_read[s], 0), "nyquist ahead: slot wait");
+  HIP_TRY(timed(g, 4, [&] {
+            return launch_half_nyquist_ahead(f->logn, fp, g->h0, g->nyq[s], f->twiddles, g->side, f->cus, g->h0_block);
+          }, g->side),
+          "column pass (half spectrum, Nyquist ahead)");
+  HIP_TRY(hipEventRecord(g->nyq_done[s], g->side), "nyquist ahead: column event");
+  g->nyq_cur = s;
+  g->nyq_slot = s ^ 1;
+  return OCEAN_OK;
+}
+
 float4* own_exchange(const ocean_generator* g) { return half_slab_path(g) ? nullptr : g->inter; }
 
 int land_frames_in_flight(ocean_generator* g)
@@ -710,15 +763,20 @@
       TRY(half_slab_columns(g, fp, out, put, col_stream));
       break;
     case FramePath::HalfBlocked:
+      g->nyq_frame = g->nyq_ahead && !g->overlap && !seed;
       if (g->overlap)
         TRY(overlapped_columns(g, fp, seed));
       else
+      {
+        if (g->nyq_frame)
+          TRY(nyquist_ahead_columns(g, fp));
         HIP_TRY(timed(g, 1, [&] {
                   const HalfFields& fl = g->fields[0];
                   return launch_half_columns(f->logn, fp, g->h0, fl.gab, fl.gde, fl.gc, fl.spec, f->twiddles, f->stream,
-                                             f->cus, g->hs, f->device_cus, seed, g->h0_block);
+                                             f->cus, g->hs, f->device_cus, seed, g->h0_block, g->nyq_frame);
                 }),
                 "column pass (half spectrum)");
+      }
       break;
     case FramePath::Full:
       HIP_TRY(timed(g, 1, [&] {
@@ -772,11 +830,19 @@
       const HalfFields& fl = g->fields[s];
       if (g->overlap)
         HIP_TRY(hipStreamWaitEvent(f->stream, g->ocols[s], 0), "overlap: column wait");
+      const HalfNyquist* nq = g->nyq_frame && !g->overlap ? &g->nyq[g->nyq_cur] : nullptr;
+      if (nq)
+        HIP_TRY(hipStreamWaitEvent(f->stream, g->nyq_done[g->nyq_cur], 0), "nyquist ahead: column wait");
       HIP_TRY(timed(g, 2, [&] {
-                return launch_half_rows(f->logn, fs.frame, fl.gab, fl.gde, fl.gc, fl.spec, g->maps, g->jac, fs.foam,
-                                        f->twiddles, f->stream, f->cus);
+                return launch_half_rows(f->logn, fs.frame, fl.gab, fl.gde, fl.gc, nq ? nq->spec : fl.spec, g->maps,
+                                        g->jac, fs.foam, f->twiddles, f->stream, f->cus, nq);
               }),
               g->overlap ? "row pass (half spectrum, overlapped)" : "row pass (half spectrum)");
+      if (nq)
+      {
+        HIP_TRY(hipEventRecord(g->nyq_read[g->nyq_cur], f->stream), "nyquist ahead: row event");
+        g->nyq_read_valid[g->nyq_cur] = true;
+      }
       if (g->overlap)
       {
         HIP_TRY(hipEventRecord(g->orows[s], f->stream), "overlap: row event");
@@ -851,7 +917,7 @@
     (void)hipEventDestroy(ev);
   for (hipEvent_t ev : {g->cols_done[0], g->cols_done[1], g->xchg_done[0], g->xchg_done[1], g->rows_done[0],
                         g->rows_done[1], g->put_h0, g->cols_ev, g->h0r_ev, g->ocols[0], g->ocols[1], g->orows[0],
-                        g->orows[1], g->oh0})
+                        g->orows[1], g->oh0, g->nyq_done[0], g->nyq_done[1], g->nyq_read[0], g->nyq_read[1]})
     if (ev)
       (void)hipEventDestroy(ev);
   const HalfFields &f0 = g->fields[0], &f1 = g->fields[1];
@@ -860,7 +926,9 @@
                   (void*)f0.spec, (void*)f1.gab, (void*)f1.gde, (void*)f1.gc, (void*)f1.spec, (void*)g->hs,
                   (void*)g->h0row, g->seedc, (void*)g->rm_ab, (void*)g->rm_de, (void*)g->rm_c, (void*)g->parts,
                   (void*)g->xbuf, (void*)g->mips, (void*)g->rates, (void*)g->kin, (void*)g->bounds, (void*)g->foam, g->foam_counts,
-                  (void*)g->deposit_acc, g->deposit_counts})
+                  (void*)g->deposit_acc, g->deposit_counts, (void*)g->nyq[0].ab, (void*)g->nyq[0].de, (void*)g->nyq[0].c,
+                  (void*)g->nyq[0].spec, (void*)g->nyq[1].ab, (void*)g->nyq[1].de, (void*)g->nyq[1].c,
+                  (void*)g->nyq[1].spec})
     if (p)
       (void)hipFree(p);
   delete g;
@@ -893,6 +961,8 @@
   TRY(land_frames_in_flight(g));
   if (!enable && g->overlap)
     TRY(ocean_generator_set_frame_overlap(g, 0));
+  if (!enable && g->nyq_ahead)
+    TRY(ocean_generator_set_nyquist_ahead(g, 0));
   if (enable && g->half_kind == HalfKind::None)
     return fail(OCEAN_ERR_INVALID, "ocean_generator_set_half_spectrum: N = 1024 .. 16384 only");
   const bool was_on = g->half_on, was_slab_path = half_slab_path(g);
@@ -919,8 +989,7 @@
   if (enable && !g->overlap)
   {
     hipError_t e = hipSuccess;
-    if (!g->side)
-      e = hipStreamCreateWithFlags(&g->side, hipStreamNonBlocking);
+    e = side_stream(g, false);
     for (hipEvent_t* ev : {&g->ocols[0], &g->ocols[1], &g->orows[0], &g->orows[1], &g->oh0})
       if (e == hipSuccess && !*ev)
         e = hipEventCreateWithFlags(ev, hipEventDisableTiming);
@@ -946,6 +1015,47 @@
     HIP_TRY(hipStreamWaitEvent(f->stream, g->oh0, 0), "ocean_generator_set_frame_overlap");
     g->overlap = false;
   }
+  return OCEAN_OK;
+}
+
+int ocean_generator_set_nyquist_ahead(ocean_generator* g, int enable)
+{
+  if (!g)
+    return fail(OCEAN_ERR_INVALID, "ocean_generator_set_nyquist_ahead: null generator");
+  if (enable && frame_path(g) != FramePath::HalfBlocked)
+    return fail(OCEAN_ERR_INVALID, "ocean_generator_set_nyquist_ahead: whole grids of N = 1024 .. 4096 on the "
+                                   "half-spectrum path only");
+  if (enable && !g->nyq_ahead)
+  {
+    const hipError_t e = nyquist_buffers(g);
+    if (e != hipSuccess)
+      return alloc_fail(e, "ocean_generator_set_nyquist_ahead");
+    g->nyq_ahead = true;
+  }
+  else if (!enable && g->nyq_ahead)
+  {
+    if (g->side && g->oh0)
+    {
+      HIP_TRY(hipEventRecord(g->oh0, g->side), "ocean_generator_set_nyquist_ahead");
+      HIP_TRY(hipStreamWaitEvent(g->fft->stream, g->oh0, 0), "ocean_generator_set_nyquist_ahead");
+    }
+    g->nyq_ahead = false;
+  }
+  return OCEAN_OK;
+}
+
+int ocean_generator_nyquist_ahead(const ocean_generator* g) { return g && g->nyq_ahead ? 1 : 0; }
+
+int ocean_generator_nyquist_time(ocean_generator* g, double* ms_total, int64_t* launches)
+{
+  if (!g)
+    return fail(OCEAN_ERR_INVALID, "ocean_generator_nyquist_time: null generator");
+  if (ms_total)
+    *ms_total = g->nyq_ms;
+  if (launches)
+    *launches = g->nyq_launches;
+  g->nyq_ms = 0;
+  g->nyq_launches = 0;
   return OCEAN_OK;
 }
 
@@ -1121,8 +1231,16 @@
     float ms = 0.0f;
     HIP_TRY(hipEventSynchronize(p.b), "hipEventSynchronize");
     HIP_TRY(hipEventElapsedTime(&ms, p.a, p.b), "hipEventElapsedTime");
-    g->ms[p.kind] += ms;
-    g->launches[p.kind] += 1;
+    if (p.kind == 4)
+    {
+      g->nyq_ms += ms;
+      g->nyq_launches += 1;
+    }
+    else
+    {
+      g->ms[p.kind] += ms;
+      g->launches[p.kind] += 1;
+    }
     g->pool.push_back(p.a);
     g->pool.push_back(p.b);
   }
diff --git a/oceansimulation_amd/csrc/ocean_capi_internal.h b/oceansimulation_amd/csrc/ocean_capi_internal.h
--- a/oceansimulation_amd/csrc/ocean_capi_internal.h
+++ b/oceansimulation_amd/csrc/ocean_capi_internal.h
@@ -120,6 +120,14 @@
   hipEvent_t ocols[2] = {nullptr, nullptr}, orows[2] = {nullptr, nullptr}, oh0 = nullptr;
   bool orows_valid[2] = {false, false};
   int oslot = 0;
+  bool nyq_ahead = false;
+  HalfNyquist nyq[2];
+  hipEvent_t nyq_done[2] = {nullptr, nullptr}, nyq_read[2] = {nullptr, nullptr};
+  bool nyq_read_valid[2] = {false, false};
+  int nyq_slot = 0, nyq_cur = 0;
+  bool nyq_frame = false;
+  double nyq_ms = 0;
+  int64_t nyq_launches = 0;
   bool h0_dirty = false;
   float* mips = nullptr;
   bool mips_fresh = false;
diff --git a/oceansimulation_amd/csrc/ocean_internal.h b/oceansimulation_amd/csrc/ocean_internal.h
--- a/oceansimulation_amd/csrc/ocean_internal.h
+++ b/oceansimulation_amd/csrc/ocean_internal.h
@@ -122,12 +122,23 @@
 int half_h0_block(int logn, int cascades);
 hipError_t launch_half_columns(int logn, const FrameParams& fp, const float4* h0, float4* gab, float4* gcd, float2* ge,
                                float4* spec, const float2* tw, hipStream_t stream, int cus, float2* hs, int hs_blocks,
-                               const void* seed_consts = nullptr, int h0_blk = 0);
+                               const void* seed_consts = nullptr, int h0_blk = 0, bool nyquist_ahead = false);
+struct HalfNyquist
+{
+  float4* ab = nullptr;
+  float4* de = nullptr;
+  float2* c = nullptr;
+  float4* spec = nullptr;
+};
+size_t half_nyquist_texels(int logn);
+bool half_nyquist_ahead_default(int logn, int cascades);
+hipError_t launch_half_nyquist_ahead(int logn, const FrameParams& fp, const float4* h0, const HalfNyquist& nq,
+                                     const float2* tw, hipStream_t stream, int cus, int h0_blk = 0);
 size_t seed_consts_bytes();
 void seed_consts(const OceanSettings& s, int n, void* out);
 hipError_t launch_half_rows(int logn, const FrameParams& fp, const float4* gab, const float4* gcd, const float2* ge,
                             const float4* rcorr, float4* maps, float* jac, const FoamParams& foam, const float2* tw,
-                            hipStream_t stream, int cus);
+                            hipStream_t stream, int cus, const HalfNyquist* nq = nullptr);
 hipError_t launch_half_nyquist(const FrameParams& fp, int n, int blk, const float4* h0, float4* spec, const float4* h0row,
                                int copies, size_t copy_stride, const void* seed, hipStream_t stream, int cus,
                                const uint64_t* dst = nullptr, size_t dst_off = 0);
diff --git a/oceansimulation_amd/waves.py b/oceansimulation_amd/waves.py
--- a/oceansimulation_amd/waves.py
+++ b/oceansimulation_amd/waves.py
@@ -165,6 +165,19 @@
         check(lib().ocean_generator_set_frame_overlap(self._h, 1 if enable else 0),
               "ocean_generator_set_frame_overlap")
 
+    def set_nyquist_ahead(self, enable: bool) -> None:
+        check(lib().ocean_generator_set_nyquist_ahead(self._h, 1 if enable else 0),
+              "ocean_generator_set_nyquist_ahead")
+
+    def nyquist_ahead(self) -> bool:
+        return bool(lib().ocean_generator_nyquist_ahead(self._h))
+
+    def nyquist_time(self):
+        ms, cnt = ctypes.c_double(), ctypes.c_int64()
+        check(lib().ocean_generator_nyquist_time(self._h, ctypes.byref(ms), ctypes.byref(cnt)),
+              "ocean_generator_nyquist_time")
+        return ms.value, cnt.value
+
     def frame_bytes(self):
         out = (ctypes.c_double * 2)()
         check(lib().ocean_generator_frame_bytes(self._h, out), "ocean_generator_frame_bytes")
```
